# ylsung/vl-merging

Measured on AMD Instinct MI355X. Metric: VL samples/sec (fwd+bwd) base_vl 384^2 at 1/2/4/8 GPUs; merge GB/s vs HBM peak, higher is better.
Workload: dtype bf16

## Files before the change

include/vlm_hip.h:

```cpp
#ifndef VLM_HIP_H
#define VLM_HIP_H
#include <stddef.h>
#include <stdint.h>

#ifdef __cplusplus
extern "C" {
#endif

#define VLM_OK 0
#define VLM_ERR_ARG (-1)
#define VLM_ERR_LAUNCH (-2)
#define VLM_ERR_WORKSPACE (-3)
#define VLM_ERR_UNSUPPORTED (-4)

#define VLM_ABI_VERSION 10
int vlm_abi_version(void);
int vlm_device_cus(void);
int vlm_set_cu_budget(int cus);
int vlm_debug_occupy(int workgroups, int threads, int lds_bytes, int microseconds, void* stream);

#define VLM_MERGE_LERP 0
#define VLM_MERGE_TASKVEC 1
#define VLM_MERGE_MEAN 2
#define VLM_MERGE_MAX_SRC 4

typedef struct {
  void* dst;
  const void* base;
  const void* src[VLM_MERGE_MAX_SRC];
  float ratio[VLM_MERGE_MAX_SRC];
  int32_t n_src;
  int32_t mode;
  uint64_t n_elem;
} vlm_merge_job_t;

size_t vlm_merge_plan_bytes(int n_jobs, uint64_t total_elems);
int vlm_merge_plan_upload(const vlm_merge_job_t* jobs_host, int n_jobs, void* workspace, size_t workspace_bytes,
                          void* stream);
int vlm_merge_run(const void* workspace, void* stream);

typedef struct {
  void* dst;
  const void* base;
  const void* src[VLM_MERGE_MAX_SRC];
  uint64_t k[VLM_MERGE_MAX_SRC];
  uint64_t n_elem;
  int32_t n_src;
  float lam;
} vlm_ties_job_t;

typedef struct {
  uint64_t n_jobs, n_units, n_chunks;
  uint64_t jobs_off;
  uint64_t chunks_off;
  uint64_t unit0_off;
  uint64_t units_off;
  uint64_t state_off;
  uint64_t counters_off;
  uint64_t hist_off;
} vlm_ties_header_t;
typedef struct {
  uint32_t key;
  uint32_t reserved;
  uint64_t rank;
} vlm_ties_state_t;
#define VLM_TIES_COUNTERS (VLM_MERGE_MAX_SRC + 2)

size_t vlm_ties_plan_bytes(int n_jobs, uint64_t total_elems);
int vlm_ties_plan_upload(const vlm_ties_job_t* jobs_host, int n_jobs, void* workspace, size_t workspace_bytes, void* stream);
int vlm_ties_run(void* workspace, void* stream);

#define VLM_ACT_NONE 0
#define VLM_ACT_GELU 1
#define VLM_ACT_GELU_BWD 2
#define VLM_ACT_GELU_DERIV 3
#define VLM_ACT_MUL_AUX 4

typedef struct {
  const float* bias;
  const float* col_scale;
  const float* row_scale;
  const float* residual;
  int64_t ld_res;
  void* aux;
  int64_t ld_aux;
  int32_t act;
  float alpha;
  int32_t accumulate;
  int32_t reserved;
  float* col_sum;
  float* col_sum_ws;
  float* splitk_ws;
  uint64_t splitk_ws_bytes;
} vlm_epilogue_t;

int vlm_gemm_bf16(int ta, int tb, int M, int N, int K, const void* A, int lda, const void* B, int ldb, void* C,
                  int ldc, int c_is_f32, const vlm_epilogue_t* epi, void* stream);
#define VLM_GEMM_MAX_GROUPS 4
typedef struct {
  int32_t row0, rows;
  const void* B;
  int32_t ldb;
  int32_t reserved;
  const float* bias;
  float* col_sum;
  float* col_sum_ws;
} vlm_gemm_group_t;
int vlm_gemm_bf16_grouped(int n_groups, const vlm_gemm_group_t* groups, int N, int K, const void* A, int lda, void* C,
                          int ldc, int c_is_f32, const vlm_epilogue_t* epi, void* stream);
typedef struct {
  int32_t row0, rows;
  float* C;
  int32_t accumulate;
  int32_t reserved;
} vlm_wgrad_group_t;
int vlm_gemm_wgrad_grouped(int n_groups, const vlm_wgrad_group_t* groups, int M, int N, const void* A, int lda,
                           const void* B, int ldb, int ldc, float* splitk_ws, uint64_t splitk_ws_bytes, void* stream);
int vlm_gemm_set_big_tile_mode(int mode);

int vlm_layernorm_fwd(const float* x, int ldx, int M, int D, const float* gamma, const float* beta, float eps,
                      void* y, int ldy, int y_is_f32, float* stats, void* stream);
#define VLM_ROW_WS_BYTES(D) ((size_t)1536 * 2 * (size_t)(D) * sizeof(float))
int vlm_layernorm_bwd(const void* dy, int lddy, int dy_is_f32, const float* x, int ldx, const float* stats,
                      const float* gamma, int M, int D, const float* dres, int lddres, float* dx, int lddx,
                      float* dgamma, float* dbeta, float* workspace, size_t workspace_bytes, int* deferred_blocks,
                      void* stream);
typedef struct {
  const void* y;
  int32_t ldy;
  const float* gamma;
  const float* row_scale;
  void* dy;
  int32_t lddy;
  float* dgamma;
  float* dbias;
  float* workspace;
  size_t workspace_bytes;
} vlm_layerscale_t;
int vlm_layernorm_bwd_scale(const void* dy, int lddy, int dy_is_f32, const float* x, int ldx, const float* stats,
                            const float* gamma, int M, int D, const float* dres, int lddres, float* dx, int lddx,
                            float* dgamma, float* dbeta, float* workspace, size_t workspace_bytes,
                            const vlm_layerscale_t* scale, int* deferred_blocks, void* stream);
#define VLM_MAX_FOLD_JOBS 16
typedef struct {
  const float* partials;
  int32_t nblocks;
  int32_t D;
  float* out0;
  float* out1;
} vlm_fold_job_t;
int vlm_colreduce_batch(const vlm_fold_job_t* jobs_host, int n_jobs, void* stream);
int vlm_layerscale_bwd(const float* dx, int lddx, const void* y_bf16, int ldy, const float* gamma,
                       const float* row_scale, int M, int D, void* dy_bf16, int lddy, float* dgamma, float* dbias,
                       float* workspace, size_t workspace_bytes, int* deferred_blocks, void* stream);
#define VLM_MAX_LAYERSCALE_JOBS 32
typedef struct {
  const float* weight;
  const float* gamma;
  const float* bias;
  void* shadow;
  float* bias_out;
  float* raw_w;
  float* raw_b;
  float* dweight;
  float* dbias;
  float* dgamma;
  int32_t N, K;
} vlm_layerscale_job_t;
int vlm_layerscale_fold(const vlm_layerscale_job_t* jobs_host, int n_jobs, void* stream);
int vlm_layerscale_finish(const vlm_layerscale_job_t* jobs_host, int n_jobs, void* stream);
int vlm_colsum_bf16(const void* a, int lda, int M, int N, float* out, void* stream);

int vlm_cross_entropy_fwd(const void* logits_bf16, int ld, int rows, int V, const int64_t* labels, int64_t ignore_index,
                          float* loss_rows, float* lse, void* stream);
int vlm_cross_entropy_bwd(const void* logits_bf16, int ld, int rows, int V, const int64_t* labels, int64_t ignore_index,
                          const float* lse, const float* scale_dev, void* dlogits_bf16, int ld_d, void* stream);

int vlm_l2norm_fwd(const void* x, int x_is_bf16, int ld, int rows, int D, float* y, float* inv_norm, void* stream);
int vlm_l2norm_bwd(const float* g, const float* y, const float* inv_norm, int rows, int D, void* dx, int dx_is_bf16, int ld, void* stream);
size_t vlm_contrastive_ws_floats(int n);
int vlm_contrastive(const float* all_img, const float* all_txt, int n, int B, int D, const float* log_scale, float* logits, float* out3,
                    float* d_img, float* d_txt, float* ws, void* stream);
int vlm_small_cross_entropy(const void* logits, int is_bf16, int ld, int rows, int V, const int64_t* labels, float* loss, float* dlogits,
                            void* stream);
int vlm_cross_entropy_reduce(const float* loss_rows, const int64_t* labels, int rows, int V, int64_t ignore_index, float* out2, void* stream);
int vlm_scale_by_scalar(const float* const* in, float* const* out, const int* n, int count, const float* scalar_dev, void* stream);

int vlm_text_rows_fwd(const int64_t* ids, int n, const float* word, int ld_word, const float* add0, const float* gamma, const float* beta,
                      float eps, const float* u, float p, float scale, const float* add1, float* out, int ld_out, float* stats, int D,
                      void* stream);
size_t vlm_text_rows_bwd_ws_floats(int D);
int vlm_text_rows_bwd(const float* g, int ld_g, const int64_t* ids, int n, const float* word, int ld_word, const float* add0,
                      const float* gamma, const float* stats, const float* u, float p, float scale, int D, float* d_word,
                      int64_t padding_idx, float* d_add1, float* d_beta, float* d_gamma, float* d_add0, float* ws, void* stream);
int vlm_image_rows_prep(const float* conv_bias, const float* type_row, const float* cls, int D, float* out2, void* stream);
int vlm_image_lead_rows(float* x, int ld_x, int B, int rows, int D, const float* lead, void* stream);
size_t vlm_image_rows_bwd_ws_floats(int D);
int vlm_image_rows_bwd(const float* g, int ld_g, int B, int rows, int D, void* g16, float* d_bias, float* d_type_row, float* d_cls, float* ws,
                       void* stream);
int vlm_tanh_fwd(const void* x_bf16, int ld_x, int M, int N, float* y, void* stream);
int vlm_act_bwd(const void* g, int g_is_f32, int ld_g, const void* saved, int ld_saved, int mode, int M, int N, int Np, void* dy_bf16,
                void* stream);
int vlm_colsum_small(const void* a_bf16, int lda, int M, int N, float* out, void* stream);
int vlm_sample_negatives(const float* sim_a, int a_row_stride, int a_col_stride, const float* sim_b, int b_row_stride, int b_col_stride, int B,
                         int n, const float* u, int64_t* idx, void* stream);
int vlm_weighted_sum(const float* const* terms, const float* weights, int count, float* out, void* stream);

typedef struct {
  const void* g;
  int g_is_f32;
  int ld;
  int first_row, row_step, count;
} vlm_scatter_src_t;
int vlm_scatter_rows(void* dx, int dx_is_f32, int ld_dx, int R, int D, const vlm_scatter_src_t* src, int n_src, void* stream);

int vlm_adamw_step(float* p, float* g, float* m, float* v, void* p_bf16, uint64_t n, float lr, float beta1,
                   float beta2, float eps, float weight_decay, float step_size, float grad_scale, int zero_grad,
                   void* stream);
int vlm_cast_f32_bf16(const float* src, void* dst_bf16, uint64_t n, void* stream);
int vlm_embedding_bwd(const float* gy, int ld, const int64_t* ids, int64_t n, int D, int64_t padding_idx, float* dW, int ld_w,
                      int64_t vocab, void* stream);
typedef struct {
  uint64_t src;
  uint64_t dst;
  int32_t rows, cols;
  int32_t tile_row, tile_col;
} vlm_transpose_tile_t;
int vlm_transpose_bf16_tiles(const vlm_transpose_tile_t* tiles_dev, int n_tiles, void* stream);

int vlm_droppath_rows(const float* u, float keep, int B, int n0, int n1, int base0, int base1, float* out, void* stream);
int vlm_droppath_sites(const float* u0, const float* u1, const float* keep, int n_sites, int B, int n0, int n1, int base0,
                       int base1, int rows, float* out, void* stream);
int vlm_patch_im2col(const float* image, void* patches_bf16, int B, int H, int W, int P, int lead_rows, void* stream);
int vlm_accumulate_f32_f64(const float* src, double* dst_f64, uint64_t n, void* stream);
int vlm_gram_f64(const void* x, int ldx, int M, int D, int x_is_f32, double* gram, void* stream);
int vlm_gemm_f64(int ta, int tb, int M, int N, int K, double alpha, const void* A, int lda, int a_is_f32, const double* B,
                 int ldb, double beta, double* C, int ldc, void* stream);
int vlm_scale_gram_f64(const double* src, double* dst, int n, double alpha, int accumulate, void* stream);
int vlm_potrf_block_f64(double* A, int lda, int j0, int nb, int* status, void* stream);
int vlm_trsm_block_f64(const double* L, int ldl, int l0, int nb, int trans, double* B, int ldb, int rows, int c0, void* stream);
int vlm_cholesky_f64(double* A, int n, int* status, void* stream);
int vlm_solve_spd_right_f64(const double* chol, int n, double* rhs, int ld, int rows, void* stream);
int vlm_gemm_f64_batched(int ta, int tb, int M, int N, int K, double alpha, const void* const* A_list, int lda, int a_is_f32,
                         const double* const* B_list, int ldb, double beta, double* const* C_list, int ldc, int count, void* stream);
int vlm_cholesky_f64_batched(double* const* A_list, int count, int n, int* status, void* stream);
int vlm_solve_spd_right_f64_batched(double* const* chol_list, int n, double* const* rhs_list, int ld, int rows, int count, void* stream);

#define VLM_ATTN_JOINT 0
#define VLM_ATTN_SEPARATE 1

typedef struct {
  const void* qkv;
  int32_t ld_qkv;
  int32_t H;
  int32_t total_rows;
  int32_t R;
  const float* bias_t;
  const int16_t* rel_index;
  const int16_t* rel_index_t;
  int32_t ld_index;
  int32_t index_rows;
  int32_t ld_index_t;
  int32_t index_t_rows;
  int32_t head_row0;
  int32_t mode;
  const uint8_t* keep0;
  const uint8_t* keep1;
  int32_t B, n0, n1, base0, base1, pos1;
  float scale;
  int32_t reserved;
  const void* bias_dense;
  const void* bias_dense_t;
  int32_t dense_tiles;
  int32_t reserved2;
} vlm_attn_desc_t;

size_t vlm_bias_dense_bytes(int n0, int n1, int pos1, int mode);
int vlm_bias_dense(const float* bias_t, int n_cols, int R, const int16_t* index, int ld_index, int n0, int n1, int pos1,
                   int mode, int k_major, void* out_f16, void* stream);

int vlm_attention_fwd(const vlm_attn_desc_t* d, void* out_bf16, int ld_out, float* lse, void* stream);
typedef struct {
  float* dq[2];
  float* dv[2];
} vlm_attn_colsum_t;

size_t vlm_attention_bwd_ws_floats(const vlm_attn_desc_t* d, int with_dbias);
int vlm_attention_bwd(const vlm_attn_desc_t* d, const void* out_bf16, int ld_out, const void* dout_bf16, int ld_dout,
                      const float* lse, float* delta_ws, size_t ws_floats, void* dqkv_bf16, int ld_dqkv, float* dbias_t,
                      const vlm_attn_colsum_t* colsum, void* stream);

#ifdef __cplusplus
}
#endif
#endif
```

vl-merging_amd/_lib.py:

```python
import ctypes
import os

_HERE = os.path.dirname(os.path.abspath(__file__))
LIB_PATH = os.environ.get("VLM_LIB_PATH") or os.path.join(_HERE, "lib", "libvlm_hip.so")
_lib = None

c_void_p = ctypes.c_void_p
c_int = ctypes.c_int
c_float = ctypes.c_float
c_size_t = ctypes.c_size_t
c_u64 = ctypes.c_uint64

MERGE_LERP, MERGE_TASKVEC, MERGE_MEAN = 0, 1, 2
MERGE_MAX_SRC = 4


class MergeJob(ctypes.Structure):
    _fields_ = [
        ("dst", c_void_p),
        ("base", c_void_p),
        ("src", c_void_p * MERGE_MAX_SRC),
        ("ratio", c_float * MERGE_MAX_SRC),
        ("n_src", ctypes.c_int32),
        ("mode", ctypes.c_int32),
        ("n_elem", c_u64),
    ]


TIES_COUNTERS = MERGE_MAX_SRC + 2


class TiesJob(ctypes.Structure):
    _fields_ = [
        ("dst", c_void_p),
        ("base", c_void_p),
        ("src", c_void_p * MERGE_MAX_SRC),
        ("k", c_u64 * MERGE_MAX_SRC),
        ("n_elem", c_u64),
        ("n_src", ctypes.c_int32),
        ("lam", c_float),
    ]


class TiesHeader(ctypes.Structure):
    _fields_ = [(n, c_u64) for n in ("n_jobs", "n_units", "n_chunks", "jobs_off", "chunks_off", "unit0_off", "units_off",
                                     "state_off", "counters_off", "hist_off")]


class TiesState(ctypes.Structure):
    _fields_ = [("key", ctypes.c_uint32), ("reserved", ctypes.c_uint32), ("rank", c_u64)]


class ScatterSrc(ctypes.Structure):
    _fields_ = [("g", c_void_p), ("g_is_f32", ctypes.c_int32), ("ld", ctypes.c_int32), ("first_row", ctypes.c_int32),
                ("row_step", ctypes.c_int32), ("count", ctypes.c_int32)]


class Epilogue(ctypes.Structure):
    _fields_ = [
        ("bias", c_void_p), ("col_scale", c_void_p), ("row_scale", c_void_p), ("residual", c_void_p),
        ("ld_res", ctypes.c_int64), ("aux", c_void_p), ("ld_aux", ctypes.c_int64), ("act", ctypes.c_int32),
        ("alpha", c_float), ("accumulate", ctypes.c_int32), ("reserved", ctypes.c_int32), ("col_sum", c_void_p),
        ("col_sum_ws", c_void_p), ("splitk_ws", c_void_p), ("splitk_ws_bytes", ctypes.c_uint64),
    ]


GEMM_MAX_GROUPS = 4


class GemmGroup(ctypes.Structure):
    _fields_ = [("row0", ctypes.c_int32), ("rows", ctypes.c_int32), ("B", c_void_p), ("ldb", ctypes.c_int32),
                ("reserved", ctypes.c_int32), ("bias", c_void_p), ("col_sum", c_void_p), ("col_sum_ws", c_void_p)]


class WgradGroup(ctypes.Structure):
    _fields_ = [("row0", ctypes.c_int32), ("rows", ctypes.c_int32), ("C", c_void_p), ("accumulate", ctypes.c_int32),
                ("reserved", ctypes.c_int32)]


class FoldJob(ctypes.Structure):
    _fields_ = [("partials", c_void_p), ("nblocks", ctypes.c_int32), ("D", ctypes.c_int32), ("out0", c_void_p),
                ("out1", c_void_p)]


class LayerScale(ctypes.Structure):
    _fields_ = [("y", c_void_p), ("ldy", ctypes.c_int32), ("gamma", c_void_p), ("row_scale", c_void_p), ("dy", c_void_p),
                ("lddy", ctypes.c_int32), ("dgamma", c_void_p), ("dbias", c_void_p), ("workspace", c_void_p),
                ("workspace_bytes", c_size_t)]


class AttnColsum(ctypes.Structure):
    _fields_ = [("dq", c_void_p * 2), ("dv", c_void_p * 2)]


ACT_NONE, ACT_GELU, ACT_GELU_BWD, ACT_GELU_DERIV, ACT_MUL_AUX = 0, 1, 2, 3, 4
ATTN_JOINT, ATTN_SEPARATE = 0, 1


class AttnDesc(ctypes.Structure):
    _fields_ = [
        ("qkv", c_void_p), ("ld_qkv", ctypes.c_int32), ("H", ctypes.c_int32), ("total_rows", ctypes.c_int32),
        ("R", ctypes.c_int32), ("bias_t", c_void_p), ("rel_index", c_void_p), ("rel_index_t", c_void_p),
        ("ld_index", ctypes.c_int32), ("index_rows", ctypes.c_int32), ("ld_index_t", ctypes.c_int32),
        ("index_t_rows", ctypes.c_int32), ("head_row0", ctypes.c_int32), ("mode", ctypes.c_int32),
        ("keep0", c_void_p), ("keep1", c_void_p),
        ("B", ctypes.c_int32), ("n0", ctypes.c_int32), ("n1", ctypes.c_int32), ("base0", ctypes.c_int32),
        ("base1", ctypes.c_int32), ("pos1", ctypes.c_int32), ("scale", c_float), ("reserved", ctypes.c_int32),
        ("bias_dense", c_void_p), ("bias_dense_t", c_void_p), ("dense_tiles", ctypes.c_int32), ("reserved2", ctypes.c_int32),
    ]


class LayerScaleJob(ctypes.Structure):
    _fields_ = [("weight", c_void_p), ("gamma", c_void_p), ("bias", c_void_p), ("shadow", c_void_p), ("bias_out", c_void_p),
                ("raw_w", c_void_p), ("raw_b", c_void_p), ("dweight", c_void_p), ("dbias", c_void_p), ("dgamma", c_void_p),
                ("N", ctypes.c_int32), ("K", ctypes.c_int32)]


MAX_LAYERSCALE_JOBS = 32


class VlmError(RuntimeError):
    pass


_ERR = {-1: "VLM_ERR_ARG", -2: "VLM_ERR_LAUNCH", -3: "VLM_ERR_WORKSPACE", -4: "VLM_ERR_UNSUPPORTED"}

SIGNATURES = {
    "vlm_abi_version": (c_int, []),
    "vlm_device_cus": (c_int, []),
    "vlm_set_cu_budget": (c_int, [c_int]),
    "vlm_debug_occupy": (c_int, [c_int, c_int, c_int, c_int, c_void_p]),
    "vlm_layerscale_fold": (c_int, [ctypes.POINTER(LayerScaleJob), c_int, c_void_p]),
    "vlm_layerscale_finish": (c_int, [ctypes.POINTER(LayerScaleJob), c_int, c_void_p]),
    "vlm_merge_plan_bytes": (c_size_t, [c_int, c_u64]),
    "vlm_merge_plan_upload": (c_int, [ctypes.POINTER(MergeJob), c_int, c_void_p, c_size_t, c_void_p]),
    "vlm_merge_run": (c_int, [c_void_p, c_void_p]),
    "vlm_ties_plan_bytes": (c_size_t, [c_int, c_u64]),
    "vlm_ties_plan_upload": (c_int, [ctypes.POINTER(TiesJob), c_int, c_void_p, c_size_t, c_void_p]),
    "vlm_ties_run": (c_int, [c_void_p, c_void_p]),
    "vlm_gemm_bf16": (c_int, [c_int, c_int, c_int, c_int, c_int, c_void_p, c_int, c_void_p, c_int, c_void_p, c_int,
                              c_int, ctypes.POINTER(Epilogue), c_void_p]),
    "vlm_gemm_bf16_grouped": (c_int, [c_int, ctypes.POINTER(GemmGroup), c_int, c_int, c_void_p, c_int, c_void_p, c_int, c_int,
                                      ctypes.POINTER(Epilogue), c_void_p]),
    "vlm_gemm_wgrad_grouped": (c_int, [c_int, ctypes.POINTER(WgradGroup), c_int, c_int, c_void_p, c_int, c_void_p, c_int, c_int,
                                       c_void_p, c_u64, c_void_p]),
    "vlm_attention_fwd": (c_int, [ctypes.POINTER(AttnDesc), c_void_p, c_int, c_void_p, c_void_p]),
    "vlm_attention_bwd_ws_floats": (c_size_t, [ctypes.POINTER(AttnDesc), c_int]),
    "vlm_attention_bwd": (c_int, [ctypes.POINTER(AttnDesc), c_void_p, c_int, c_void_p, c_int, c_void_p, c_void_p, c_size_t,
                                  c_void_p, c_int, c_void_p, c_void_p, c_void_p]),
    "vlm_layernorm_fwd": (c_int, [c_void_p, c_int, c_int, c_int, c_void_p, c_void_p, c_float, c_void_p, c_int, c_int,
                                  c_void_p, c_void_p]),
    "vlm_layernorm_bwd": (c_int, [c_void_p, c_int, c_int, c_void_p, c_int, c_void_p, c_void_p, c_int, c_int, c_void_p,
                                  c_int, c_void_p, c_int, c_void_p, c_void_p, c_void_p, c_size_t,
                                  ctypes.POINTER(c_int), c_void_p]),
    "vlm_layernorm_bwd_scale": (c_int, [c_void_p, c_int, c_int, c_void_p, c_int, c_void_p, c_void_p, c_int, c_int, c_void_p,
                                        c_int, c_void_p, c_int, c_void_p, c_void_p, c_void_p, c_size_t,
                                        ctypes.POINTER(LayerScale), ctypes.POINTER(c_int), c_void_p]),
    "vlm_layerscale_bwd": (c_int, [c_void_p, c_int, c_void_p, c_int, c_void_p, c_void_p, c_int, c_int, c_void_p, c_int,
                                   c_void_p, c_void_p, c_void_p, c_size_t, ctypes.POINTER(c_int), c_void_p]),
    "vlm_colreduce_batch": (c_int, [ctypes.POINTER(FoldJob), c_int, c_void_p]),
    "vlm_gemm_set_big_tile_mode": (c_int, [c_int]),
    "vlm_colsum_bf16": (c_int, [c_void_p, c_int, c_int, c_int, c_void_p, c_void_p]),
    "vlm_adamw_step": (c_int, [c_void_p, c_void_p, c_void_p, c_void_p, c_void_p, c_u64, c_float, c_float, c_float,
                               c_float, c_float, c_float, c_float, c_int, c_void_p]),
    "vlm_accumulate_f32_f64": (c_int, [c_void_p, c_void_p, c_u64, c_void_p]),
    "vlm_gram_f64": (c_int, [c_void_p, c_int, c_int, c_int, c_int, c_void_p, c_void_p]),
    "vlm_gemm_f64": (c_int, [c_int, c_int, c_int, c_int, c_int, ctypes.c_double, c_void_p, c_int, c_int, c_void_p, c_int,
                             ctypes.c_double, c_void_p, c_int, c_void_p]),
    "vlm_scale_gram_f64": (c_int, [c_void_p, c_void_p, c_int, ctypes.c_double, c_int, c_void_p]),
    "vlm_potrf_block_f64": (c_int, [c_void_p, c_int, c_int, c_int, c_void_p, c_void_p]),
    "vlm_trsm_block_f64": (c_int, [c_void_p, c_int, c_int, c_int, c_int, c_void_p, c_int, c_int, c_int, c_void_p]),
    "vlm_cholesky_f64": (c_int, [c_void_p, c_int, c_void_p, c_void_p]),
    "vlm_solve_spd_right_f64": (c_int, [c_void_p, c_int, c_void_p, c_int, c_int, c_void_p]),
    "vlm_gemm_f64_batched": (c_int, [c_int, c_int, c_int, c_int, c_int, ctypes.c_double, ctypes.POINTER(c_void_p), c_int, c_int,
                                     ctypes.POINTER(c_void_p), c_int, ctypes.c_double, ctypes.POINTER(c_void_p), c_int, c_int, c_void_p]),
    "vlm_cholesky_f64_batched": (c_int, [ctypes.POINTER(c_void_p), c_int, c_int, c_void_p, c_void_p]),
    "vlm_solve_spd_right_f64_batched": (c_int, [ctypes.POINTER(c_void_p), c_int, ctypes.POINTER(c_void_p), c_int, c_int, c_int, c_void_p]),
    "vlm_cross_entropy_fwd": (c_int, [c_void_p, c_int, c_int, c_int, c_void_p, ctypes.c_int64, c_void_p, c_void_p, c_void_p]),
    "vlm_cross_entropy_bwd": (c_int, [c_void_p, c_int, c_int, c_int, c_void_p, ctypes.c_int64, c_void_p, c_void_p, c_void_p, c_int,
                                      c_void_p]),
    "vlm_l2norm_fwd": (c_int, [c_void_p, c_int, c_int, c_int, c_int, c_void_p, c_void_p, c_void_p]),
    "vlm_l2norm_bwd": (c_int, [c_void_p, c_void_p, c_void_p, c_int, c_int, c_void_p, c_int, c_int, c_void_p]),
    "vlm_contrastive_ws_floats": (c_size_t, [c_int]),
    "vlm_contrastive": (c_int, [c_void_p, c_void_p, c_int, c_int, c_int, c_void_p, c_void_p, c_void_p, c_void_p, c_void_p, c_void_p,
                                c_void_p]),
    "vlm_small_cross_entropy": (c_int, [c_void_p, c_int, c_int, c_int, c_int, c_void_p, c_void_p, c_void_p, c_void_p]),
    "vlm_cross_entropy_reduce": (c_int, [c_void_p, c_void_p, c_int, c_int, ctypes.c_int64, c_void_p, c_void_p]),
    "vlm_scale_by_scalar": (c_int, [ctypes.POINTER(c_void_p), ctypes.POINTER(c_void_p), ctypes.POINTER(c_int), c_int, c_void_p, c_void_p]),
    "vlm_text_rows_fwd": (c_int, [c_void_p, c_int, c_void_p, c_int, c_void_p, c_void_p, c_void_p, c_float, c_void_p, c_float, c_float,
                                  c_void_p, c_void_p, c_int, c_void_p, c_int, c_void_p]),
    "vlm_text_rows_bwd_ws_floats": (c_size_t, [c_int]),
    "vlm_text_rows_bwd": (c_int, [c_void_p, c_int, c_void_p, c_int, c_void_p, c_int, c_void_p, c_void_p, c_void_p, c_void_p, c_float, c_float,
                                  c_int, c_void_p, ctypes.c_int64, c_void_p, c_void_p, c_void_p, c_void_p, c_void_p, c_void_p]),
    "vlm_image_rows_prep": (c_int, [c_void_p, c_void_p, c_void_p, c_int, c_void_p, c_void_p]),
    "vlm_image_lead_rows": (c_int, [c_void_p, c_int, c_int, c_int, c_int, c_void_p, c_void_p]),
    "vlm_image_rows_bwd_ws_floats": (c_size_t, [c_int]),
    "vlm_image_rows_bwd": (c_int, [c_void_p, c_int, c_int, c_int, c_int, c_void_p, c_void_p, c_void_p, c_void_p, c_void_p, c_void_p]),
    "vlm_tanh_fwd": (c_int, [c_void_p, c_int, c_int, c_int, c_void_p, c_void_p]),
    "vlm_act_bwd": (c_int, [c_void_p, c_int, c_int, c_void_p, c_int, c_int, c_int, c_int, c_int, c_void_p, c_void_p]),
    "vlm_colsum_small": (c_int, [c_void_p, c_int, c_int, c_int, c_void_p, c_void_p]),
    "vlm_sample_negatives": (c_int, [c_void_p, c_int, c_int, c_void_p, c_int, c_int, c_int, c_int, c_void_p, c_void_p, c_void_p]),
    "vlm_weighted_sum": (c_int, [ctypes.POINTER(c_void_p), ctypes.POINTER(c_float), c_int, c_void_p, c_void_p]),
    "vlm_scatter_rows": (c_int, [c_void_p, c_int, c_int, c_int, c_int, c_void_p, c_int, c_void_p]),
    "vlm_cast_f32_bf16": (c_int, [c_void_p, c_void_p, c_u64, c_void_p]),
    "vlm_embedding_bwd": (c_int, [c_void_p, c_int, c_void_p, ctypes.c_int64, c_int, ctypes.c_int64, c_void_p, c_int,
                                  ctypes.c_int64, c_void_p]),
    "vlm_bias_dense_bytes": (c_size_t, [c_int, c_int, c_int, c_int]),
    "vlm_bias_dense": (c_int, [c_void_p, c_int, c_int, c_void_p, c_int, c_int, c_int, c_int, c_int, c_int, c_void_p,
                               c_void_p]),
    "vlm_transpose_bf16_tiles": (c_int, [c_void_p, c_int, c_void_p]),
    "vlm_droppath_sites": (c_int, [c_void_p, c_void_p, c_void_p, c_int, c_int, c_int, c_int, c_int, c_int, c_int, c_void_p,
                                   c_void_p]),
    "vlm_droppath_rows": (c_int, [c_void_p, c_float, c_int, c_int, c_int, c_int, c_int, c_void_p, c_void_p]),
    "vlm_patch_im2col": (c_int, [c_void_p, c_void_p, c_int, c_int, c_int, c_int, c_int, c_void_p]),
}


def get_lib():
    global _lib
    if _lib is None:
        if not os.path.exists(LIB_PATH):
            raise VlmError(
                f"{LIB_PATH} is missing: build it with `python -c 'import __graft_entry__ as g; g.build()'` "
                "(hipcc --offload-arch=gfx950).  There is no CPU fallback for the hot path.")
        import torch
        lib = ctypes.CDLL(LIB_PATH)
        for name, (res, args) in SIGNATURES.items():
            fn = getattr(lib, name)
            fn.restype = res
            fn.argtypes = args
        _lib = lib
    return _lib


def check(rc, what):
    if rc != 0:
        raise VlmError(f"{what} failed: {_ERR.get(rc, rc)}")


def stream_ptr():
    import torch
    return c_void_p(torch.cuda.current_stream().cuda_stream)


def ptr(t):
    return c_void_p(t.data_ptr()) if t is not None else c_void_p(0)


def require_cuda(*tensors):
    for t in tensors:
        if t is not None and not t.is_cuda:
            raise VlmError("vl_merging_amd ops run on the GPU only (tensor on %s); there is no CPU path" % t.device)
```

vl-merging_amd/csrc/gemm.hip:

```cpp
#include "vlm_common.h"
#include "vlm_diag.h"
#include <atomic>

#define GEMM_BM 128
#define GEMM_BN 128
#define GEMM_BK 64
#define GEMM_THREADS 256
#define GEMM_TILE_BYTES (GEMM_BM * GEMM_BK * 2)

typedef __attribute__((address_space(3))) s16x4 lds_s16x4;

__device__ __forceinline__ float gelu_cdf(float x, float& ez2) {
  const float t = __builtin_amdgcn_rcpf(fmaf(0.3275911f * 0.70710678118654752440f, fabsf(x), 1.0f));
  ez2 = __builtin_amdgcn_exp2f((x * x) * (-0.5f * 1.4426950408889634f));
  float poly = fmaf(t, 0.5f * 1.061405429f, 0.5f * -1.453152027f);
  poly = fmaf(t, poly, 0.5f * 1.421413741f);
  poly = fmaf(t, poly, 0.5f * -0.284496736f);
  poly = fmaf(t, poly, 0.5f * 0.254829592f);
  const float e = fmaf(-(poly * t), ez2, 0.5f);
  return 0.5f + copysignf(e, x);
}
__device__ __forceinline__ float gelu_erf(float x) {
  float ez2;
  return x * gelu_cdf(x, ez2);
}
__device__ __forceinline__ float gelu_erf_grad(float x) {
  float ez2;
  const float cdf = gelu_cdf(x, ez2);
  return fmaf(x * 0.39894228040143267794f, ez2, cdf);
}
__device__ __forceinline__ float gelu_erf_both(float x, float& deriv) {
  float ez2;
  const float cdf = gelu_cdf(x, ez2);
  deriv = fmaf(x * 0.39894228040143267794f, ez2, cdf);
  return x * cdf;
}
__device__ __forceinline__ float act_bwd_factor(int act, float saved) {
  return act == VLM_ACT_MUL_AUX ? saved : gelu_erf_grad(saved);
}

template <bool KSTRIDED>
__device__ __forceinline__ void stage_load(u32x4 (&r)[4], __amdgpu_buffer_rsrc_t rsrc, uint32_t row0, uint32_t k0,
                                           uint32_t ld, int tid) {
#pragma unroll
  for (int u = 0; u < 4; ++u) {
    const uint32_t p = tid + 256 * u;
    uint32_t off;
    if (!KSTRIDED) {
      const uint32_t row = p >> 3, chunk = p & 7;
      off = ((row0 + row) * ld + k0 + chunk * 8) * 2;
    } else {
      const uint32_t krow = p >> 4, c16 = p & 15;
      off = ((k0 + krow) * ld + row0 + c16 * 8) * 2;
    }
    r[u] = __builtin_amdgcn_raw_buffer_load_b128(rsrc, off, 0, 0);
  }
}

template <bool KSTRIDED>
__device__ __forceinline__ void stage_store(const u32x4 (&r)[4], unsigned char* lds, int tid) {
#pragma unroll
  for (int u = 0; u < 4; ++u) {
    const uint32_t p = tid + 256 * u;
    uint32_t byte;
    if (!KSTRIDED) {
      const uint32_t row = p >> 3, chunk = p & 7;
      byte = row * 128 + ((chunk ^ (row & 7)) << 4);
    } else {
      const uint32_t krow = p >> 4, c16 = p & 15;
      const uint32_t c32 = (c16 >> 1) ^ (krow & 3) ^ (((krow >> 3) & 1) << 2);
      byte = krow * 256 + c32 * 32 + (c16 & 1) * 16;
    }
    *reinterpret_cast<u32x4*>(lds + byte) = r[u];
  }
}

typedef __attribute__((address_space(3))) void lds_void;
__device__ __forceinline__ void stage_dma(__amdgpu_buffer_rsrc_t rsrc, unsigned char* tile, uint32_t row0, uint32_t k0,
                                          uint32_t ld, int wave, int lane) {
#pragma unroll
  for (int u = 0; u < 4; ++u) {
    const int j = wave + 4 * u;
    const uint32_t row = j * 8 + (lane >> 3), chunk = (lane & 7) ^ (row & 7);
    const uint32_t off = ((row0 + row) * ld + k0 + chunk * 8) * 2;
    __builtin_amdgcn_raw_ptr_buffer_load_lds(rsrc, (lds_void*)(tile + j * 1024), 16, off, 0, 0, 0);
  }
}

template <bool KSTRIDED>
__device__ __forceinline__ bf16x8 frag_load(const unsigned char* lds, int xblk , int ksub,
                                            int lane) {
  if (!KSTRIDED) {
    const uint32_t row = xblk * 16 + (lane & 15);
    const uint32_t chunk = ksub * 4 + (lane >> 4);
    const uint32_t byte = row * 128 + ((chunk ^ (row & 7)) << 4);
    return *reinterpret_cast<const bf16x8*>(lds + byte);
  } else {
    const uint32_t g = lane >> 4, q = (lane & 15) >> 2, p = lane & 3;
    const uint32_t row = ksub * 32 + 8 * g + q;
    const uint32_t c32 = ((uint32_t)xblk ^ q ^ ((g & 1) << 2));
    const uint32_t byte = row * 256 + c32 * 32 + 8 * p;
    s16x4 lo = __builtin_amdgcn_ds_read_tr16_b64_v4i16((lds_s16x4*)(lds + byte));
    s16x4 hi = __builtin_amdgcn_ds_read_tr16_b64_v4i16((lds_s16x4*)(lds + byte + 4 * 256));
    s16x8 v = {lo[0], lo[1], lo[2], lo[3], hi[0], hi[1], hi[2], hi[3]};
    return __builtin_bit_cast(bf16x8, v);
  }
}

struct gemm_group_t {
  const void* B;
  const float* bias;
  float* col_sum;
  float* col_sum_ws;
  int ldb, row0, row_end, tile0;
};

struct gemmT_group_t {
  int row0, row_end, item0, kps, slice0;
};

struct gemm_params_t {
  const void* A;
  const void* B;
  void* C;
  int M, N, K;
  int lda, ldb, ldc;
  vlm_epilogue_t epi;
  int tiles_m, tiles_n;
  int group_m;
  int splits, ksteps_per_split;
  int n_groups;
  gemm_group_t grp[VLM_GEMM_MAX_GROUPS];
  gemmT_group_t grpT[VLM_GEMM_MAX_GROUPS];
  VLM_DIAG_GEMM_FIELD
};

__device__ __forceinline__ void lane16_swap(float& x, float& y) {
  asm volatile("s_nop 1\n\tv_permlane16_swap_b32 %0, %1" : "+v"(x), "+v"(y));
}

template <bool OUT_F32, bool LEAN = false>
__device__ __forceinline__ int gemm_epilogue(const gemm_params_t& p, const f32x4 (&acc)[4][4], int mw0, int nw0, int lane,
                                             float* red = nullptr, int red_off = 0) {
  const vlm_epilogue_t& e = p.epi;
  const bool vec_ok = ((p.ldc & 3) == 0) && (!e.aux || (e.ld_aux & 3) == 0) && (!e.residual || (e.ld_res & 3) == 0);
  const bool vec8_ok = vec_ok && (OUT_F32 || (p.ldc & 7) == 0) && (!e.aux || ((e.ld_aux & 7) == 0 && ((uintptr_t)e.aux & 15) == 0)) &&
                       (!e.residual || ((uintptr_t)e.residual & 15) == 0) && (!e.bias || ((uintptr_t)e.bias & 15) == 0) &&
                       (!e.col_scale || ((uintptr_t)e.col_scale & 15) == 0);
  if (vec8_ok && mw0 + 64 <= p.M && nw0 + 64 <= p.N) {
    const bool has_res = e.residual != nullptr, bwd = e.act == VLM_ACT_GELU_BWD || e.act == VLM_ACT_MUL_AUX, accum = OUT_F32 && e.accumulate;
    const int g = lane >> 4;
    const int nl = nw0 + (g & 1) * 16 + (g >> 1) * 8;
    float bia[2][8], gam[2][8], csum[2][8];
#pragma unroll
    for (int jp = 0; jp < 2; ++jp)
#pragma unroll
      for (int r = 0; r < 8; ++r) csum[jp][r] = 0.f;
#define EPI_LOAD_COL_VECTORS()                                                                                          \
  _Pragma("unroll") for (int jp = 0; jp < 2; ++jp) _Pragma("unroll") for (int q = 0; q < 2; ++q) {                    \
    const f32x4 b4 = e.bias ? *reinterpret_cast<const f32x4*>(e.bias + nl + jp * 32 + q * 4) : (f32x4){0.f, 0.f, 0.f, 0.f}; \
    const f32x4 g4 =                                                                                                    \
        e.col_scale ? *reinterpret_cast<const f32x4*>(e.col_scale + nl + jp * 32 + q * 4) : (f32x4){1.f, 1.f, 1.f, 1.f}; \
    _Pragma("unroll") for (int r = 0; r < 4; ++r) {                                                                     \
      bia[jp][q * 4 + r] = b4[r];                                                                                       \
      gam[jp][q * 4 + r] = g4[r];                                                                                       \
    }                                                                                                                   \
  }
    if (!LEAN) { EPI_LOAD_COL_VECTORS() }
#pragma unroll
    for (int hf = 0; hf < 4; ++hf) {
      f32x4 rsd[1][2][2], old[1][2][2];
      bf16x8 hx[1][2];
      float rs[1];
      if (LEAN) { EPI_LOAD_COL_VECTORS() }
#pragma unroll
      for (int ii = 0; ii < 1; ++ii) {
        const size_t m = mw0 + (hf + ii) * 16 + (lane & 15);
        rs[ii] = e.row_scale ? e.row_scale[m] : 1.0f;
#pragma unroll
        for (int jp = 0; jp < 2; ++jp) {
          const int n = nl + jp * 32;
          if (has_res) {
            rsd[ii][jp][0] = *reinterpret_cast<const f32x4*>(e.residual + m * e.ld_res + n);
            rsd[ii][jp][1] = *reinterpret_cast<const f32x4*>(e.residual + m * e.ld_res + n + 4);
          }
          if (bwd) hx[ii][jp] = *reinterpret_cast<const bf16x8*>(reinterpret_cast<const bf16_t*>(e.aux) + m * e.ld_aux + n);
          if (accum) {
            old[ii][jp][0] = *reinterpret_cast<const f32x4*>(reinterpret_cast<const float*>(p.C) + m * p.ldc + n);
            old[ii][jp][1] = *reinterpret_cast<const f32x4*>(reinterpret_cast<const float*>(p.C) + m * p.ldc + n + 4);
          }
        }
      }
#pragma unroll
      for (int ii = 0; ii < 1; ++ii) {
        const size_t m = mw0 + (hf + ii) * 16 + (lane & 15);
#pragma unroll
        for (int jp = 0; jp < 2; ++jp) {
          const int n = nl + jp * 32;
          float v[8];
#pragma unroll
          for (int r = 0; r < 4; ++r) {
            float x = acc[hf + ii][2 * jp][r] * e.alpha, y = acc[hf + ii][2 * jp + 1][r] * e.alpha;
            lane16_swap(x, y);
            v[r] = x;
            v[4 + r] = y;
          }
#pragma unroll
          for (int r = 0; r < 8; ++r) v[r] += bia[jp][r];
          if (bwd) {
#pragma unroll
            for (int r = 0; r < 8; ++r) v[r] *= act_bwd_factor(e.act, (float)hx[ii][jp][r]);
          } else if (e.act == VLM_ACT_GELU_DERIV) {
            bf16x8 h;
#pragma unroll
            for (int r = 0; r < 8; ++r) {
              float dg;
              v[r] = gelu_erf_both(v[r], dg);
              h[r] = (bf16_t)dg;
            }
            *reinterpret_cast<bf16x8*>(reinterpret_cast<bf16_t*>(e.aux) + m * e.ld_aux + n) = h;
          } else {
            if (e.aux) {
              bf16x8 h;
#pragma unroll
              for (int r = 0; r < 8; ++r) h[r] = (bf16_t)v[r];
              *reinterpret_cast<bf16x8*>(reinterpret_cast<bf16_t*>(e.aux) + m * e.ld_aux + n) = h;
            }
            if (e.act == VLM_ACT_GELU) {
#pragma unroll
              for (int r = 0; r < 8; ++r) v[r] = gelu_erf(v[r]);
            }
          }
          if (e.col_scale) {
#pragma unroll
            for (int r = 0; r < 8; ++r) v[r] *= gam[jp][r];
          }
          if (e.row_scale) {
#pragma unroll
            for (int r = 0; r < 8; ++r) v[r] *= rs[ii];
          }
          if (has_res) {
#pragma unroll
            for (int r = 0; r < 8; ++r) v[r] += rsd[ii][jp][r >> 2][r & 3];
          }
          if (OUT_F32 && accum) {
#pragma unroll
            for (int r = 0; r < 8; ++r) v[r] += old[ii][jp][r >> 2][r & 3];
          }
          if (!LEAN && e.col_sum) {
#pragma unroll
            for (int r = 0; r < 8; ++r) csum[jp][r] += v[r];
          }
          if (OUT_F32) {
            float* c = reinterpret_cast<float*>(p.C) + m * p.ldc + n;
            *reinterpret_cast<f32x4*>(c) = (f32x4){v[0], v[1], v[2], v[3]};
            *reinterpret_cast<f32x4*>(c + 4) = (f32x4){v[4], v[5], v[6], v[7]};
          } else {
            bf16x8 o;
#pragma unroll
            for (int r = 0; r < 8; ++r) o[r] = (bf16_t)v[r];
            *reinterpret_cast<bf16x8*>(reinterpret_cast<bf16_t*>(p.C) + m * p.ldc + n) = o;
          }
        }
      }
    }
    if (!LEAN && e.col_sum) {
#pragma unroll
      for (int jp = 0; jp < 2; ++jp)
#pragma unroll
        for (int r = 0; r < 8; ++r) {
          float t = csum[jp][r];
          t += dpp_f32<0x128>(t);
          t += dpp_f32<0x124>(t);
          t += dpp_f32<0x122>(t);
          t += dpp_f32<0x121>(t);
          if ((lane & 15) == 0) {
            if (red) red[red_off + (g & 1) * 16 + (g >> 1) * 8 + jp * 32 + r] = t;
            else atomicAdd(e.col_sum + nl + jp * 32 + r, t);
          }
        }
      return -1;
    }
    return 8 * (OUT_F32 ? 2 : 1) + ((e.aux && !bwd) ? 8 : 0);
  }
#pragma unroll
  for (int i = 0; i < 4; ++i) {
    const int m = mw0 + i * 16 + (lane & 15);
    if (m >= p.M) continue;
    const float rs = e.row_scale ? e.row_scale[m] : 1.0f;
#pragma unroll
    for (int j = 0; j < 4; ++j) {
      const int n = nw0 + j * 16 + (lane >> 4) * 4;
      if (n >= p.N) continue;
      const bool full = vec_ok && (n + 3 < p.N);
      float v[4];
#pragma unroll
      for (int r = 0; r < 4; ++r) v[r] = acc[i][j][r] * e.alpha;
      if (full) {
        if (e.bias) {
          const f32x4 b = *reinterpret_cast<const f32x4*>(e.bias + n);
#pragma unroll
          for (int r = 0; r < 4; ++r) v[r] += b[r];
        }
        if (e.act == VLM_ACT_GELU_BWD || e.act == VLM_ACT_MUL_AUX) {
          const bf16x4 h = *reinterpret_cast<const bf16x4*>(reinterpret_cast<const bf16_t*>(e.aux) + (size_t)m * e.ld_aux + n);
#pragma unroll
          for (int r = 0; r < 4; ++r) v[r] *= act_bwd_factor(e.act, (float)h[r]);
        } else if (e.act == VLM_ACT_GELU_DERIV) {
          bf16x4 h;
#pragma unroll
          for (int r = 0; r < 4; ++r) {
            float dg;
            v[r] = gelu_erf_both(v[r], dg);
            h[r] = (bf16_t)dg;
          }
          *reinterpret_cast<bf16x4*>(reinterpret_cast<bf16_t*>(e.aux) + (size_t)m * e.ld_aux + n) = h;
        } else {
          if (e.aux) {
            bf16x4 h;
#pragma unroll
            for (int r = 0; r < 4; ++r) h[r] = (bf16_t)v[r];
            *reinterpret_cast<bf16x4*>(reinterpret_cast<bf16_t*>(e.aux) + (size_t)m * e.ld_aux + n) = h;
          }
          if (e.act == VLM_ACT_GELU) {
#pragma unroll
            for (int r = 0; r < 4; ++r) v[r] = gelu_erf(v[r]);
          }
        }
        if (e.col_scale) {
          const f32x4 g = *reinterpret_cast<const f32x4*>(e.col_scale + n);
#pragma unroll
          for (int r = 0; r < 4; ++r) v[r] *= g[r];
        }
        if (e.row_scale) {
#pragma unroll
          for (int r = 0; r < 4; ++r) v[r] *= rs;
        }
        if (e.residual) {
          const f32x4 x = *reinterpret_cast<const f32x4*>(e.residual + (size_t)m * e.ld_res + n);
#pragma unroll
          for (int r = 0; r < 4; ++r) v[r] += x[r];
        }
        if (OUT_F32) {
          float* c = reinterpret_cast<float*>(p.C) + (size_t)m * p.ldc + n;
          f32x4 o = {v[0], v[1], v[2], v[3]};
          if (e.accumulate) {
            const f32x4 old = *reinterpret_cast<const f32x4*>(c);
            o += old;
          }
          if (e.col_sum) {
#pragma unroll
            for (int r = 0; r < 4; ++r) atomicAdd(e.col_sum + n + r, o[r]);
          }
          *reinterpret_cast<f32x4*>(c) = o;
        } else {
          if (e.col_sum) {
#pragma unroll
            for (int r = 0; r < 4; ++r) atomicAdd(e.col_sum + n + r, v[r]);
          }
          bf16x4 o;
#pragma unroll
          for (int r = 0; r < 4; ++r) o[r] = (bf16_t)v[r];
          *reinterpret_cast<bf16x4*>(reinterpret_cast<bf16_t*>(p.C) + (size_t)m * p.ldc + n) = o;
        }
      } else {
        for (int r = 0; r < 4 && n + r < p.N; ++r) {
          float x = v[r];
          if (e.bias) x += e.bias[n + r];
          if (e.act == VLM_ACT_GELU_BWD || e.act == VLM_ACT_MUL_AUX) {
            x *= act_bwd_factor(e.act, (float)reinterpret_cast<const bf16_t*>(e.aux)[(size_t)m * e.ld_aux + n + r]);
          } else if (e.act == VLM_ACT_GELU_DERIV) {
            float dg;
            x = gelu_erf_both(x, dg);
            reinterpret_cast<bf16_t*>(e.aux)[(size_t)m * e.ld_aux + n + r] = (bf16_t)dg;
          } else {
            if (e.aux) reinterpret_cast<bf16_t*>(e.aux)[(size_t)m * e.ld_aux + n + r] = (bf16_t)x;
            if (e.act == VLM_ACT_GELU) x = gelu_erf(x);
          }
          if (e.col_scale) x *= e.col_scale[n + r];
          if (e.row_scale) x *= rs;
          if (e.residual) x += e.residual[(size_t)m * e.ld_res + n + r];
          if (OUT_F32 && e.accumulate) x += reinterpret_cast<const float*>(p.C)[(size_t)m * p.ldc + n + r];
          if (e.col_sum) atomicAdd(e.col_sum + n + r, x);
          if (OUT_F32) {
            reinterpret_cast<float*>(p.C)[(size_t)m * p.ldc + n + r] = x;
          } else {
            reinterpret_cast<bf16_t*>(p.C)[(size_t)m * p.ldc + n + r] = (bf16_t)x;
          }
        }
      }
    }
  }
  return -1;
}

template <bool TA, bool TB, bool OUT_F32, bool SPLITK>
__global__ __launch_bounds__(GEMM_THREADS, 2) void vlm_gemm_kernel(const gemm_params_t p) {
  constexpr bool DMA_A = !TA && !SPLITK, DMA_B = !TB && !SPLITK;
  extern __shared__ __attribute__((aligned(16))) unsigned char smem[];
  const int tid = threadIdx.x;
  const int lane = tid & 63;
  const int wave = tid >> 6;
  const int wm = wave >> 1, wn = wave & 1;
  GEMM_STAMP(0)

  const uint32_t ntile = p.tiles_m * p.tiles_n;
  uint32_t tile, split = 0;
  if (SPLITK) {
    tile = blockIdx.x % ntile;
    split = blockIdx.x / ntile;
  } else {
    const uint32_t nblk = gridDim.x;
    const uint32_t bid = blockIdx.x;
    const uint32_t q8 = nblk >> 3, r8 = nblk & 7, xcd = bid & 7;
    tile = (xcd < r8 ? xcd * (q8 + 1) : r8 * (q8 + 1) + (xcd - r8) * q8) + (bid >> 3);
  }
  uint32_t tm, tn;
  {
    const uint32_t gm = (uint32_t)p.group_m, gsz = gm * p.tiles_n, grp = tile / gsz, first = grp * gm;
    const uint32_t rows = min(gm, (uint32_t)p.tiles_m - first), in = tile - grp * gsz;
    tm = first + in % rows;
    tn = in / rows;
  }
  const uint32_t m0 = tm * GEMM_BM, n0 = tn * GEMM_BN;

  const uint64_t a_rows = TA ? (uint64_t)p.K : (uint64_t)p.M;
  const uint64_t b_rows = TB ? (uint64_t)p.K : (uint64_t)p.N;
  const __amdgpu_buffer_rsrc_t ra =
      __builtin_amdgcn_make_buffer_rsrc(const_cast<void*>(p.A), 0, (int)(a_rows * p.lda * 2), 0x00020000);
  const __amdgpu_buffer_rsrc_t rb =
      __builtin_amdgcn_make_buffer_rsrc(const_cast<void*>(p.B), 0, (int)(b_rows * p.ldb * 2), 0x00020000);

#define LDS_A(s) (smem + (s) * 2 * GEMM_TILE_BYTES)
#define LDS_B(s) (smem + (s) * 2 * GEMM_TILE_BYTES + GEMM_TILE_BYTES)

  f32x4 acc[4][4];
// ... 202 lines not shown
#pragma unroll
          for (int r = 0; r < 8; ++r) v[r] *= gelu_erf_grad((float)in.hx[t][r]);
        }
      } else if (AUX == 1 && e.act == VLM_ACT_GELU_DERIV) {
        bf16x8 h;
#pragma unroll
        for (int r = 0; r < 8; ++r) {
          float dg;
          v[r] = gelu_erf_both(v[r], dg);
          h[r] = (bf16_t)dg;
        }
        __builtin_amdgcn_raw_buffer_store_b128(__builtin_bit_cast(u32x4, h), r_aux, (m * (uint32_t)e.ld_aux + n) * 2, 0, EPIL_AUX_STORE_AUX);
      } else {
        if (AUX == 1) {
          bf16x8 h;
#pragma unroll
          for (int r = 0; r < 8; ++r) h[r] = (bf16_t)v[r];
          __builtin_amdgcn_raw_buffer_store_b128(__builtin_bit_cast(u32x4, h), r_aux, (m * (uint32_t)e.ld_aux + n) * 2, 0, EPIL_AUX_STORE_AUX);
        }
        if (e.act == VLM_ACT_GELU) {
#pragma unroll
          for (int r = 0; r < 8; ++r) v[r] = gelu_erf(v[r]);
        }
      }
      if (RES) {
#pragma unroll
        for (int r = 0; r < 8; ++r) v[r] *= gam[r];
        if (e.row_scale) {
#pragma unroll
          for (int r = 0; r < 8; ++r) v[r] *= in.rs[t];
        }
#pragma unroll
        for (int r = 0; r < 8; ++r) v[r] += in.rsd[t][r >> 2][r & 3];
      }
      if (AUX == 2) {
        if (m < (uint32_t)p.M) {
#pragma unroll
          for (int r = 0; r < 8; ++r) csum[r] += v[r];
        }
      }
      if (OUT_F32) {
        const uint32_t co = (m * (uint32_t)p.ldc + n) * 4;
        __builtin_amdgcn_raw_buffer_store_b128(__builtin_bit_cast(u32x4, (f32x4){v[0], v[1], v[2], v[3]}), r_c, co, 0, STORE_AUX);
        __builtin_amdgcn_raw_buffer_store_b128(__builtin_bit_cast(u32x4, (f32x4){v[4], v[5], v[6], v[7]}), r_c, co + 16, 0, STORE_AUX);
      } else {
        bf16x8 o;
#pragma unroll
        for (int r = 0; r < 8; ++r) o[r] = (bf16_t)v[r];
        __builtin_amdgcn_raw_buffer_store_b128(__builtin_bit_cast(u32x4, o), r_c, (m * (uint32_t)p.ldc + n) * 2, 0, STORE_AUX);
      }
    }
  }

  __device__ __forceinline__ void finish(int lane, float* ws_row) {
    const vlm_epilogue_t& e = p.epi;
    if (AUX != 2 || !e.col_sum) return;
#pragma unroll
    for (int r = 0; r < 8; ++r) {
      if (LPR == 8) csum[r] += __shfl_xor(csum[r], 8);
      csum[r] += __shfl_xor(csum[r], 16);
      csum[r] += __shfl_xor(csum[r], 32);
    }
    if (lane < LPR) {
      if (ws_row) {
        *reinterpret_cast<f32x4*>(ws_row + n) = (f32x4){csum[0], csum[1], csum[2], csum[3]};
        *reinterpret_cast<f32x4*>(ws_row + n + 4) = (f32x4){csum[4], csum[5], csum[6], csum[7]};
      } else {
#pragma unroll
        for (int r = 0; r < 8; ++r) atomicAdd(e.col_sum + n + r, csum[r]);
      }
    }
  }
};

#define EPIL_DUMP_ROW(A0, A1, II, OFF)                                                           \
  _Pragma("unroll") for (int j = 0; j < 4; ++j) {                                                \
    *reinterpret_cast<f32x4*>(wr + (OFF) + 64 * j) = A0[II][j];                                  \
    *reinterpret_cast<f32x4*>(wr + (OFF) + 64 * (4 + j)) = A1[II][j];                            \
  }
#define BIG_EPILOGUE_LOOP_DEEP(AHEAD)                                                                             \
  unsigned char* wr = wl + (lane & 15) * EPIL_PITCH + (lane >> 4) * 16;                                            \
  epil_in_t in8[8];                                                                                                \
  _Pragma("unroll") for (int b8 = 0; b8 < (AHEAD); ++b8) ep.load_inputs(in8[b8], b8);                              \
  _Pragma("unroll") for (int q = 0; q < 4; ++q) {                                                                  \
    switch (q) {                                                                                                   \
      case 0: EPIL_DUMP_ROW(acc00, acc01, 0, 0) EPIL_DUMP_ROW(acc00, acc01, 1, 16 * EPIL_PITCH) break;             \
      case 1: EPIL_DUMP_ROW(acc00, acc01, 2, 0) EPIL_DUMP_ROW(acc00, acc01, 3, 16 * EPIL_PITCH) break;             \
      case 2: EPIL_DUMP_ROW(acc10, acc11, 0, 0) EPIL_DUMP_ROW(acc10, acc11, 1, 16 * EPIL_PITCH) break;             \
      default: EPIL_DUMP_ROW(acc10, acc11, 2, 0) EPIL_DUMP_ROW(acc10, acc11, 3, 16 * EPIL_PITCH) break;            \
    }                                                                                                              \
    ep.process(in8[2 * q], 2 * q, 0);                                                                              \
    if (2 * q + (AHEAD) < 8) ep.load_inputs(in8[2 * q + (AHEAD)], 2 * q + (AHEAD));                                \
    ep.process(in8[2 * q + 1], 2 * q + 1, 16 * EPIL_PITCH);                                                        \
    if (2 * q + 1 + (AHEAD) < 8) ep.load_inputs(in8[2 * q + 1 + (AHEAD)], 2 * q + 1 + (AHEAD));                    \
  }
#define BIG_EPILOGUE_LOOP()                                                                                       \
  unsigned char* wr = wl + (lane & 15) * EPIL_PITCH + (lane >> 4) * 16;                                            \
  ep.load_inputs(inB, 1);                                                                                          \
  _Pragma("unroll 1") for (int q = 0; q < 4; ++q) {                                                                \
    switch (q) {                                                                                                   \
      case 0: EPIL_DUMP_ROW(acc00, acc01, 0, 0) EPIL_DUMP_ROW(acc00, acc01, 1, 16 * EPIL_PITCH) break;             \
      case 1: EPIL_DUMP_ROW(acc00, acc01, 2, 0) EPIL_DUMP_ROW(acc00, acc01, 3, 16 * EPIL_PITCH) break;             \
      case 2: EPIL_DUMP_ROW(acc10, acc11, 0, 0) EPIL_DUMP_ROW(acc10, acc11, 1, 16 * EPIL_PITCH) break;             \
      default: EPIL_DUMP_ROW(acc10, acc11, 2, 0) EPIL_DUMP_ROW(acc10, acc11, 3, 16 * EPIL_PITCH) break;            \
    }                                                                                                              \
    ep.process(inA, 2 * q, 0);                                                                                     \
    ep.load_inputs(inA, q < 3 ? 2 * q + 2 : 7);                                                                    \
    ep.process(inB, 2 * q + 1, 16 * EPIL_PITCH);                                                                   \
    ep.load_inputs(inB, q < 3 ? 2 * q + 3 : 7);                                                                    \
  }

template <bool OUT_F32, bool RES, int AUX, bool GROUPED = false>
__global__ __launch_bounds__(GEMM_THREADS, 1) void vlm_gemm_big_kernel(const gemm_params_t p_in) {
  __shared__ __attribute__((aligned(1024))) unsigned char sA0[BIG_OP_BYTES], sA1[BIG_OP_BYTES], sB0[BIG_OP_BYTES], sB1[BIG_OP_BYTES];
  __shared__ __attribute__((aligned(16))) unsigned char epl[4 * EPIL_WAVE_BYTES];
  const int tid = threadIdx.x;
  const int lane = tid & 63;
  const int wave = __builtin_amdgcn_readfirstlane(tid >> 6);
  const int wm = wave >> 1, wn = wave & 1;

  const uint32_t nblk = gridDim.x, bid = blockIdx.x;
  const uint32_t q8 = nblk >> 3, r8 = nblk & 7, xcd = bid & 7;
  const uint32_t tile = (xcd < r8 ? xcd * (q8 + 1) : r8 * (q8 + 1) + (xcd - r8) * q8) + (bid >> 3);
  uint32_t tm, tn;
  {
    const uint32_t gm = (uint32_t)p_in.group_m, gsz = gm * p_in.tiles_n, grp = tile / gsz, first = grp * gm;
    const uint32_t rows = min(gm, (uint32_t)p_in.tiles_m - first), in = tile - grp * gsz;
    tm = first + in % rows;
    tn = in / rows;
  }
  gemm_params_t p_grp;
  uint32_t m0 = tm * BIG_BM, tm_ws = tm;
  if constexpr (GROUPED) {
    p_grp = p_in;
    int g = 0;
#pragma unroll
    for (int i = 1; i < VLM_GEMM_MAX_GROUPS; ++i)
      if (i < p_in.n_groups && tm >= (uint32_t)p_in.grp[i].tile0) g = i;
    const gemm_group_t G = p_in.grp[g];
    tm_ws = tm - (uint32_t)G.tile0;
    m0 = (uint32_t)G.row0 + tm_ws * BIG_BM;
    p_grp.M = G.row_end;
    p_grp.B = G.B;
    p_grp.ldb = G.ldb;
    p_grp.epi.bias = G.bias;
    p_grp.epi.col_sum = G.col_sum;
    p_grp.epi.col_sum_ws = G.col_sum_ws;
  }
  const gemm_params_t& p = GROUPED ? p_grp : p_in;
  GEMM_STAMP(0)
  const uint32_t n0 = tn * BIG_BN;
  const __amdgpu_buffer_rsrc_t ra =
      __builtin_amdgcn_make_buffer_rsrc(const_cast<void*>(p.A), 0, (int)((uint64_t)p.M * p.lda * 2), 0x00020000);
  const __amdgpu_buffer_rsrc_t rb =
      __builtin_amdgcn_make_buffer_rsrc(const_cast<void*>(p.B), 0, (int)((uint64_t)p.N * p.ldb * 2), 0x00020000);

  uint32_t offa[4], offb[4];
  {
    const uint32_t chunk = (lane & 3) ^ big_swz(lane >> 4);
#pragma unroll
    for (int u = 0; u < 4; ++u) {
      const uint32_t row = (wave + 4 * u) * 16 + (lane >> 2);
      offa[u] = ((m0 + row) * (uint32_t)p.lda + chunk * 8) * 2;
      offb[u] = ((n0 + row) * (uint32_t)p.ldb + chunk * 8) * 2;
    }
  }
  const uint32_t rd_slot = ((uint32_t)(lane >> 4) ^ big_swz((lane & 15) >> 2)) * 16 + (lane & 15) * 64;
  const uint32_t rda = wm * 128 * 64 + rd_slot, rdb = wn * 128 * 64 + rd_slot;

  f32x4 acc00[4][4], acc01[4][4], acc10[4][4], acc11[4][4];
#pragma unroll
  for (int i = 0; i < 4; ++i)
#pragma unroll
    for (int j = 0; j < 4; ++j) {
      acc00[i][j] = (f32x4){0.f, 0.f, 0.f, 0.f};
      acc01[i][j] = (f32x4){0.f, 0.f, 0.f, 0.f};
      acc10[i][j] = (f32x4){0.f, 0.f, 0.f, 0.f};
      acc11[i][j] = (f32x4){0.f, 0.f, 0.f, 0.f};
    }

#define BIG_PIN_ACC()                                                                                   \
  _Pragma("unroll") for (int i = 0; i < 4; ++i) _Pragma("unroll") for (int j = 0; j < 4; ++j) {         \
    asm volatile("" : "+a"(acc00[i][j]), "+a"(acc01[i][j]), "+a"(acc10[i][j]), "+a"(acc11[i][j]));      \
  }
  constexpr bool DEEP = AUX == 2 && !RES;
  constexpr int AHEAD = 6;
  if constexpr (DEEP) { BIG_PIN_ACC() }

  const int nk = p.K / BIG_BK;
  const uint32_t mw0 = m0 + wm * 128, nw0 = n0 + wn * 128;
  unsigned char* const wl = epl + wave * EPIL_WAVE_BYTES;
#define EPIL_SETUP()                                       \
  big_epilogue_t<OUT_F32, RES, AUX> ep(p, wl, mw0, nw0, lane); \
  epil_in_t inA, inB;                                      \
  ep.load_inputs(inA, 0);
  bf16x8 fa0[8], fb0[8], fa1[8], fb1[8];

#define BIG_READ(FA, FB, SA, SB)                                                         \
  _Pragma("unroll") for (int i = 0; i < 8; ++i) {                                        \
    FA[i] = *reinterpret_cast<const bf16x8*>((SA) + rda + i * 1024);                     \
    FB[i] = *reinterpret_cast<const bf16x8*>((SB) + rdb + i * 1024);                     \
  }
#define BIG_MFMA_Q(ACC, FA, FB, I0, J0)                                                                                \
  _Pragma("unroll") for (int i = 0; i < 4; ++i) _Pragma("unroll") for (int j = 0; j < 4; ++j)                         \
      ACC[i][j] = __builtin_amdgcn_mfma_f32_16x16x32_bf16(FB[(J0) + j], FA[(I0) + i], ACC[i][j], 0, 0, 0);
#define BIG_MFMA(FA, FB)        \
  BIG_MFMA_Q(acc00, FA, FB, 0, 0) \
  BIG_MFMA_Q(acc01, FA, FB, 0, 4) \
  BIG_MFMA_Q(acc11, FA, FB, 4, 4) \
  BIG_MFMA_Q(acc10, FA, FB, 4, 0)
  uint32_t wr_off[4];
  {
    const uint32_t slot = (lane & 3) ^ big_swz(lane >> 4);
#pragma unroll
    for (int u = 0; u < 4; ++u) wr_off[u] = ((wave + 4 * u) * 16 + (lane >> 2)) * 64 + slot * 16;
  }
  {
    const uint32_t unswz = (((lane & 3) ^ big_swz(lane >> 4)) - (lane & 3)) * 16;
#pragma unroll
    for (int u = 0; u < 4; ++u) { offa[u] -= unswz; offb[u] -= unswz; }
  }
  u32x4 ra0[4], rb0[4], ra1[4], rb1[4];
#define BIG_GLOAD(RA_, RB_, S)                                                                        \
  _Pragma("unroll") for (int u = 0; u < 4; ++u) {                                                     \
    RA_[u] = __builtin_amdgcn_raw_buffer_load_b128(ra, offa[u], (S) * (BIG_BK * 2), 0);               \
    RB_[u] = __builtin_amdgcn_raw_buffer_load_b128(rb, offb[u], (S) * (BIG_BK * 2), 0);               \
  }
#define BIG_LWRITE(RA_, RB_, SA, SB)                                                                  \
  _Pragma("unroll") for (int u = 0; u < 4; ++u) {                                                     \
    *reinterpret_cast<u32x4*>((SA) + wr_off[u]) = RA_[u];                                             \
    *reinterpret_cast<u32x4*>((SB) + wr_off[u]) = RB_[u];                                             \
  }
#define BIG_STEP(K, GL, WR, RD, FCA, FCB, FNA, FNB, RSA, RSB, BUFA_W, BUFB_W, BUFA_R, BUFB_R)   \
  {                                                                                      \
    if (RD) {                                                                            \
      asm volatile("s_waitcnt lgkmcnt(0)" ::: "memory");                                 \
      __builtin_amdgcn_s_barrier();                                                      \
    }                                                                                    \
    __builtin_amdgcn_sched_barrier(0);                                                   \
    if (WR) { BIG_LWRITE(RSA, RSB, BUFA_W, BUFB_W) }                                     \
    if (GL) { BIG_GLOAD(RSA, RSB, (K) + 4) }                                             \
    if (RD) { BIG_READ(FNA, FNB, BUFA_R, BUFB_R) }                                       \
    BIG_MFMA(FCA, FCB)                                                                   \
    _Pragma("unroll") for (int g = 0; g < 16; ++g) {                                     \
      __builtin_amdgcn_sched_group_barrier(0x008, 2, 0);                                 \
      __builtin_amdgcn_sched_group_barrier(0x100, 1, 0);                                 \
    }                                                                                    \
    _Pragma("unroll") for (int g = 0; g < 8; ++g) {                                      \
      __builtin_amdgcn_sched_group_barrier(0x008, 2, 0);                                 \
      __builtin_amdgcn_sched_group_barrier(0x200, 1, 0);                                 \
      __builtin_amdgcn_sched_group_barrier(0x008, 2, 0);                                 \
      __builtin_amdgcn_sched_group_barrier(0x020, 1, 0);                                 \
    }                                                                                    \
    __builtin_amdgcn_sched_barrier(0);                                                   \
  }

  BIG_GLOAD(ra0, rb0, 0)
  BIG_GLOAD(ra1, rb1, 1)
  BIG_LWRITE(ra0, rb0, sA0, sB0)
  BIG_GLOAD(ra0, rb0, 2)
  BIG_LWRITE(ra1, rb1, sA1, sB1)
  BIG_GLOAD(ra1, rb1, 3)
  asm volatile("s_waitcnt lgkmcnt(0)" ::: "memory");
  __builtin_amdgcn_s_barrier();
  BIG_READ(fa0, fb0, sA0, sB0)
  GEMM_STAMP(1)

  int kt = 0;
  for (; kt < nk - 4; kt += 2) {
    BIG_STEP(kt + 0, 1, 1, 1, fa0, fb0, fa1, fb1, ra0, rb0, sA0, sB0, sA1, sB1)
    BIG_STEP(kt + 1, 1, 1, 1, fa1, fb1, fa0, fb0, ra1, rb1, sA1, sB1, sA0, sB0)
  }
#define BIG_TAIL_STEPS()                                                               \
  BIG_STEP(kt + 0, 0, 1, 1, fa0, fb0, fa1, fb1, ra0, rb0, sA0, sB0, sA1, sB1)          \
  BIG_STEP(kt + 1, 0, 1, 1, fa1, fb1, fa0, fb0, ra1, rb1, sA1, sB1, sA0, sB0)          \
  BIG_STEP(kt + 2, 0, 0, 1, fa0, fb0, fa1, fb1, ra0, rb0, sA0, sB0, sA1, sB1)          \
  BIG_STEP(kt + 3, 0, 0, 0, fa1, fb1, fa0, fb0, ra1, rb1, sA1, sB1, sA0, sB0)
  if constexpr (DEEP) {
    BIG_TAIL_STEPS()
    GEMM_STAMP(2)
    big_epilogue_t<OUT_F32, RES, AUX> ep(p, wl, mw0, nw0, lane);
    float* ws_row = (p.epi.col_sum_ws && mw0 + 128 <= (uint32_t)p.M) ? p.epi.col_sum_ws + ((size_t)(tm_ws * 2 + wm) * 2) * p.N : nullptr;
    BIG_EPILOGUE_LOOP_DEEP(AHEAD)
    ep.finish(lane, ws_row);
  } else {
    EPIL_SETUP()
    BIG_TAIL_STEPS()
    GEMM_STAMP(2)
    float* ws_row = (p.epi.col_sum_ws && mw0 + 128 <= (uint32_t)p.M) ? p.epi.col_sum_ws + ((size_t)(tm_ws * 2 + wm) * 2) * p.N : nullptr;
    BIG_EPILOGUE_LOOP()
    ep.finish(lane, ws_row);
  }
  GEMM_STAMP_END()
}

template <bool GROUPED = false>
__global__ __launch_bounds__(GEMM_THREADS, 1) void vlm_gemm_bigT_kernel(const gemm_params_t p) {
  __shared__ __attribute__((aligned(1024))) unsigned char sA0[BIG_OP_BYTES], sA1[BIG_OP_BYTES], sB0[BIG_OP_BYTES], sB1[BIG_OP_BYTES];
  __shared__ __attribute__((aligned(16))) unsigned char epl[4 * EPIL_WAVE_BYTES];
  const int tid = threadIdx.x;
  const int lane = tid & 63;
  const int wave = __builtin_amdgcn_readfirstlane(tid >> 6);
  const int wm = wave >> 1, wn = wave & 1;
  const uint32_t ntile = p.tiles_m * p.tiles_n;
  const uint32_t q8 = gridDim.x >> 3, r8 = gridDim.x & 7, xcd = blockIdx.x & 7;
  uint32_t item = (xcd < r8 ? xcd * (q8 + 1) : r8 * (q8 + 1) + (xcd - r8) * q8) + (blockIdx.x >> 3);
  uint32_t k_base = 0, k_end = (uint32_t)p.K, slice0 = 0;
  int nk = p.ksteps_per_split;
  if constexpr (GROUPED) {
    int g = 0;
#pragma unroll
    for (int i = 1; i < VLM_GEMM_MAX_GROUPS; ++i)
      if (i < p.n_groups && item >= (uint32_t)p.grpT[i].item0) g = i;
    const gemmT_group_t G = p.grpT[g];
    item -= (uint32_t)G.item0;
    k_base = (uint32_t)G.row0;
    k_end = (uint32_t)G.row_end;
    nk = G.kps;
    slice0 = (uint32_t)G.slice0;
  }
  const uint32_t split = item / ntile, tile = item - split * ntile;
  const uint32_t tm = tile / p.tiles_n, tn = tile - tm * p.tiles_n;
  const uint32_t m0 = tm * BIG_BM, n0 = tn * BIG_BN;
  const uint32_t k_first = k_base + split * (uint32_t)nk * BIG_BK;
  const __amdgpu_buffer_rsrc_t ra =
      __builtin_amdgcn_make_buffer_rsrc(const_cast<void*>(p.A), 0, (int)((uint64_t)k_end * p.lda * 2), 0x00020000);
  const __amdgpu_buffer_rsrc_t rb =
      __builtin_amdgcn_make_buffer_rsrc(const_cast<void*>(p.B), 0, (int)((uint64_t)k_end * p.ldb * 2), 0x00020000);

  uint32_t offa[4], offb[4], wr_off[4];
#pragma unroll
  for (int u = 0; u < 4; ++u) {
    const uint32_t row = 2 * (wave + 4 * u) + (lane >> 5), c16 = lane & 31;
    offa[u] = ((k_first + row) * (uint32_t)p.lda + m0 + c16 * 8) * 2;
    offb[u] = ((k_first + row) * (uint32_t)p.ldb + n0 + c16 * 8) * 2;
    wr_off[u] = row * 512 + (((c16 >> 1) ^ ((row & 3) | (((row >> 3) & 1) << 2))) << 5) + (c16 & 1) * 16;
  }
  uint32_t rda[8], rdb[8];
  {
    const uint32_t g = lane >> 4, q = (lane & 15) >> 2, pp = lane & 3, sw = q | ((g & 1) << 2);
#pragma unroll
    for (int i = 0; i < 8; ++i) {
      rda[i] = (8 * g + q) * 512 + wm * 256 + ((i ^ sw) << 5) + 8 * pp;
      rdb[i] = (8 * g + q) * 512 + wn * 256 + ((i ^ sw) << 5) + 8 * pp;
    }
  }
  f32x4 acc00[4][4], acc01[4][4], acc10[4][4], acc11[4][4];
#pragma unroll
  for (int i = 0; i < 4; ++i)
#pragma unroll
    for (int j = 0; j < 4; ++j) {
      acc00[i][j] = (f32x4){0.f, 0.f, 0.f, 0.f};
      acc01[i][j] = (f32x4){0.f, 0.f, 0.f, 0.f};
      acc10[i][j] = (f32x4){0.f, 0.f, 0.f, 0.f};
      acc11[i][j] = (f32x4){0.f, 0.f, 0.f, 0.f};
    }
  const uint32_t stepa = BIG_BK * (uint32_t)p.lda * 2, stepb = BIG_BK * (uint32_t)p.ldb * 2;
  bf16x8 fa0[8], fb0[8], fa1[8], fb1[8];
  u32x4 ra0[4], rb0[4], ra1[4], rb1[4];
#define BIGT_TR(PTR) __builtin_amdgcn_ds_read_tr16_b64_v4i16((lds_s16x4*)(PTR))
#define BIGT_READ(FA, FB, SA, SB)                                                                    \
  _Pragma("unroll") for (int i = 0; i < 8; ++i) {                                                    \
    const s16x4 al = BIGT_TR((SA) + rda[i]), ah = BIGT_TR((SA) + rda[i] + 4 * 512);                  \
    const s16x4 bl = BIGT_TR((SB) + rdb[i]), bh = BIGT_TR((SB) + rdb[i] + 4 * 512);                  \
    FA[i] = __builtin_bit_cast(bf16x8, (s16x8){al[0], al[1], al[2], al[3], ah[0], ah[1], ah[2], ah[3]}); \
    FB[i] = __builtin_bit_cast(bf16x8, (s16x8){bl[0], bl[1], bl[2], bl[3], bh[0], bh[1], bh[2], bh[3]}); \
  }
#define BIGT_GLOAD(RA_, RB_, S)                                                                      \
  _Pragma("unroll") for (int u = 0; u < 4; ++u) {                                                    \
    RA_[u] = __builtin_amdgcn_raw_buffer_load_b128(ra, offa[u], (S) * stepa, 0);                     \
    RB_[u] = __builtin_amdgcn_raw_buffer_load_b128(rb, offb[u], (S) * stepb, 0);                     \
  }
#define BIGT_LWRITE(RA_, RB_, SA, SB)                                                                \
  _Pragma("unroll") for (int u = 0; u < 4; ++u) {                                                    \
    *reinterpret_cast<u32x4*>((SA) + wr_off[u]) = RA_[u];                                            \
    *reinterpret_cast<u32x4*>((SB) + wr_off[u]) = RB_[u];                                            \
  }
#define BIGT_STEP(K, GL, WR, RD, FCA, FCB, FNA, FNB, RSA, RSB, BUFA_W, BUFB_W, BUFA_R, BUFB_R)      \
  {                                                                                      \
    if (RD) {                                                                            \
      asm volatile("s_waitcnt lgkmcnt(0)" ::: "memory");                                 \
      __builtin_amdgcn_s_barrier();                                                      \
    }                                                                                    \
    __builtin_amdgcn_sched_barrier(0);                                                   \
    if (WR) { BIGT_LWRITE(RSA, RSB, BUFA_W, BUFB_W) }                                    \
    if (GL) { BIGT_GLOAD(RSA, RSB, (K) + 4) }                                            \
    if (RD) { BIGT_READ(FNA, FNB, BUFA_R, BUFB_R) }                                      \
    BIG_MFMA(FCA, FCB)                                                                   \
    _Pragma("unroll") for (int g = 0; g < 32; ++g) {                                     \
      __builtin_amdgcn_sched_group_barrier(0x008, 1, 0);                                 \
      __builtin_amdgcn_sched_group_barrier(0x100, 1, 0);                                 \
    }                                                                                    \
    _Pragma("unroll") for (int g = 0; g < 8; ++g) {                                      \
      __builtin_amdgcn_sched_group_barrier(0x008, 2, 0);                                 \
      __builtin_amdgcn_sched_group_barrier(0x200, 1, 0);                                 \
      __builtin_amdgcn_sched_group_barrier(0x008, 2, 0);                                 \
      __builtin_amdgcn_sched_group_barrier(0x020, 1, 0);                                 \
    }                                                                                    \
    __builtin_amdgcn_sched_barrier(0);                                                   \
  }
  BIGT_GLOAD(ra0, rb0, 0)
  BIGT_GLOAD(ra1, rb1, 1)
  BIGT_LWRITE(ra0, rb0, sA0, sB0)
  BIGT_GLOAD(ra0, rb0, 2)
  BIGT_LWRITE(ra1, rb1, sA1, sB1)
  BIGT_GLOAD(ra1, rb1, 3)
  asm volatile("s_waitcnt lgkmcnt(0)" ::: "memory");
  __builtin_amdgcn_s_barrier();
  BIGT_READ(fa0, fb0, sA0, sB0)
  int kt = 0;
  for (; kt < nk - 4; kt += 2) {
    BIGT_STEP(kt + 0, 1, 1, 1, fa0, fb0, fa1, fb1, ra0, rb0, sA0, sB0, sA1, sB1)
    BIGT_STEP(kt + 1, 1, 1, 1, fa1, fb1, fa0, fb0, ra1, rb1, sA1, sB1, sA0, sB0)
  }
  BIGT_STEP(kt + 0, 0, 1, 1, fa0, fb0, fa1, fb1, ra0, rb0, sA0, sB0, sA1, sB1)
  BIGT_STEP(kt + 1, 0, 1, 1, fa1, fb1, fa0, fb0, ra1, rb1, sA1, sB1, sA0, sB0)
  BIGT_STEP(kt + 2, 0, 0, 1, fa0, fb0, fa1, fb1, ra0, rb0, sA0, sB0, sA1, sB1)
  BIGT_STEP(kt + 3, 0, 0, 0, fa1, fb1, fa0, fb0, ra1, rb1, sA1, sB1, sA0, sB0)

  gemm_params_t pl = p;
  pl.C = reinterpret_cast<float*>(p.C) + (size_t)(slice0 + split) * p.M * p.N;
  pl.ldc = p.N;
  const uint32_t mw0 = m0 + wm * 128, nw0 = n0 + wn * 128;
  unsigned char* const wl = epl + wave * EPIL_WAVE_BYTES;
  big_epilogue_t<true, false, 0, 128, 0, true> ep(pl, wl, mw0, nw0, lane);
  epil_in_t inA, inB;
  ep.load_inputs(inA, 0);
  BIG_EPILOGUE_LOOP()
}

__global__ __launch_bounds__(256) void splitk_reduce_kernel(const float* __restrict__ ws, int splits, int M, int N, float* __restrict__ C,
                                                            int ldc, int accumulate) {
  const size_t i = (size_t)blockIdx.x * 256 + threadIdx.x, per = (size_t)M * N / 4;
  if (i >= per) return;
  const size_t e = i * 4, m = e / N, n = e - m * N;
  f32x4 t = accumulate ? *reinterpret_cast<const f32x4*>(C + m * ldc + n) : (f32x4){0.f, 0.f, 0.f, 0.f};
  for (int s = 0; s < splits; ++s) t += *reinterpret_cast<const f32x4*>(ws + (size_t)s * M * N + e);
  *reinterpret_cast<f32x4*>(C + m * ldc + n) = t;
}

struct splitk_groups_t {
  float* C[VLM_GEMM_MAX_GROUPS];
  int slice0[VLM_GEMM_MAX_GROUPS], splits[VLM_GEMM_MAX_GROUPS], accumulate[VLM_GEMM_MAX_GROUPS];
};
__global__ __launch_bounds__(256) void splitk_reduce_grouped_kernel(const float* __restrict__ ws, const splitk_groups_t g, int M, int N, int ldc) {
  const size_t i = (size_t)blockIdx.x * 256 + threadIdx.x, per = (size_t)M * N / 4;
  if (i >= per) return;
  const int gi = blockIdx.y;
  float* const C = g.C[gi];
  const size_t e = i * 4, m = e / N, n = e - m * N;
  f32x4 t = g.accumulate[gi] ? *reinterpret_cast<const f32x4*>(C + m * ldc + n) : (f32x4){0.f, 0.f, 0.f, 0.f};
  for (int s = 0; s < g.splits[gi]; ++s) t += *reinterpret_cast<const f32x4*>(ws + (size_t)(g.slice0[gi] + s) * M * N + e);
  *reinterpret_cast<f32x4*>(C + m * ldc + n) = t;
}

static int plan_cus() {
  const int cus = vlm_device_cus();
  return cus > 0 ? cus : 256;
}

static bool epi_vec8(const vlm_epilogue_t* e, int ldc, int c_is_f32) {
  const bool v4 = ((ldc & 3) == 0) && (!e->aux || (e->ld_aux & 3) == 0) && (!e->residual || (e->ld_res & 3) == 0);
  return v4 && (c_is_f32 || (ldc & 7) == 0) && (!e->aux || ((e->ld_aux & 7) == 0 && ((uintptr_t)e->aux & 15) == 0)) &&
         (!e->residual || ((uintptr_t)e->residual & 15) == 0) && (!e->bias || ((uintptr_t)e->bias & 15) == 0) &&
         (!e->col_scale || ((uintptr_t)e->col_scale & 15) == 0);
}

static bool epi_off32(const vlm_epilogue_t* e, int M, int lda, int ldc) {
  return (uint64_t)M * ldc * 4 < (1ull << 31) && (!e->residual || (uint64_t)M * e->ld_res * 4 < (1ull << 31)) &&
         (!e->aux || (uint64_t)M * e->ld_aux * 2 < (1ull << 31)) && (uint64_t)M * lda * 2 < (1ull << 31);
}

static int launch_gemm_bigT(gemm_params_t p, const vlm_epilogue_t* epi, hipStream_t stream) {
  if (!epi->splitk_ws || (p.N % BIG_BN) || (p.ldc % 4)) return 1;
  if ((uint64_t)p.M * p.N * 4 >= (1ull << 31)) return 1;
  p.tiles_m = (p.M + BIG_BM - 1) / BIG_BM;
  p.tiles_n = (p.N + BIG_BN - 1) / BIG_BN;
  const int ntile = p.tiles_m * p.tiles_n, nk = (p.K + BIG_BK - 1) / BIG_BK;
  int splits = plan_cus() / ntile;
  if (splits < 1) splits = 1;
  if (splits > nk / 16) splits = nk / 16;
  if (splits < 1) return 1;
  int kps = (nk + splits - 1) / splits;
  kps += kps & 1;
  if (kps < 4) kps = 4;
  splits = (nk + kps - 1) / kps;
  if ((size_t)splits * p.M * p.N * 4 > (size_t)epi->splitk_ws_bytes) return 1;
  p.ksteps_per_split = kps;
  p.splits = splits;
  float* const out = reinterpret_cast<float*>(p.C);
  const int ldc = p.ldc;
  p.C = epi->splitk_ws;
  hipLaunchKernelGGL(vlm_gemm_bigT_kernel<false>, dim3(ntile * splits), dim3(GEMM_THREADS), 0, stream, p);
  VLM_CHECK_LAUNCH();
  const size_t per = (size_t)p.M * p.N / 4;
  hipLaunchKernelGGL(splitk_reduce_kernel, dim3((unsigned)((per + 255) / 256)), dim3(256), 0, stream,
                     reinterpret_cast<const float*>(epi->splitk_ws), splits, p.M, p.N, out, ldc, epi->accumulate);
  VLM_CHECK_LAUNCH();
  return VLM_OK;
}

template <bool OUT_F32, bool RES, int AUX, bool GROUPED = false>
static int launch_gemm_big(gemm_params_t p, hipStream_t stream) {
  if (!GROUPED) p.tiles_m = (p.M + BIG_BM - 1) / BIG_BM;
  p.tiles_n = (p.N + BIG_BN - 1) / BIG_BN;
  p.group_m = p.tiles_n >= 6 ? 4 : 1;
  GEMM_STAMP_ARM(p)
  hipLaunchKernelGGL((vlm_gemm_big_kernel<OUT_F32, RES, AUX, GROUPED>), dim3(p.tiles_m * p.tiles_n), dim3(GEMM_THREADS), 0, stream, p);
  VLM_CHECK_LAUNCH();
  return VLM_OK;
}

template <bool GROUPED = false>
static int launch_gemm_big_variant(const gemm_params_t& p, bool c_is_f32, hipStream_t s) {
  const vlm_epilogue_t& e = p.epi;
  const bool res = e.residual != nullptr;
  const int aux = e.aux ? ((e.act == VLM_ACT_GELU_BWD || e.act == VLM_ACT_MUL_AUX) ? 2 : 1) : 0;
  if (e.row_scale && !res) return 1;
  {
    bool any_cs = e.col_sum != nullptr;
    if (GROUPED)
      for (int g = 0; g < p.n_groups; ++g) any_cs = any_cs || p.grp[g].col_sum != nullptr;
    if (e.alpha != 1.0f || (e.col_scale && !res) || (any_cs && aux != 2)) return 1;
  }
  if (!c_is_f32 && !res) {
    if (aux == 0) return launch_gemm_big<false, false, 0, GROUPED>(p, s);
    if (aux == 1) return launch_gemm_big<false, false, 1, GROUPED>(p, s);
    return launch_gemm_big<false, false, 2, GROUPED>(p, s);
  }
  if (c_is_f32 && aux != 2) {
    if (res && aux) return launch_gemm_big<true, true, 1, GROUPED>(p, s);
    if (res) return launch_gemm_big<true, true, 0, GROUPED>(p, s);
    if (GROUPED) return 1;
    if (aux == 0) return launch_gemm_big<true, false, 0>(p, s);
  }
  return 1;
}

static std::atomic<int> g_big_mode{1};
static int gemm_big_mode() { return g_big_mode.load(std::memory_order_relaxed); }
extern "C" int vlm_gemm_set_big_tile_mode(int mode) {
  if (mode < -1 || mode > 2) return VLM_ERR_ARG;
  g_big_mode.store(mode < 0 ? 1 : mode, std::memory_order_relaxed);
  return VLM_OK;
}


extern "C" int vlm_gemm_bf16(int ta, int tb, int M, int N, int K, const void* A, int lda, const void* B, int ldb,
                             void* C, int ldc, int c_is_f32, const vlm_epilogue_t* epi, void* stream) {
  if (M < 0 || N < 0 || K < 0 || !C) return VLM_ERR_ARG;
  if (M == 0 || N == 0) return VLM_OK;
  if (!A || !B || !epi) return VLM_ERR_ARG;
  if ((lda & 7) || (ldb & 7) || ((uintptr_t)A & 15) || ((uintptr_t)B & 15)) return VLM_ERR_ARG;
  if ((!ta || !tb) && (K % GEMM_BK)) return VLM_ERR_UNSUPPORTED;
  if (((ldc & 3) == 0) && ((uintptr_t)C & 15)) return VLM_ERR_ARG;
  if (epi->accumulate && !c_is_f32) return VLM_ERR_ARG;
  if ((epi->act == VLM_ACT_GELU_BWD || epi->act == VLM_ACT_MUL_AUX || epi->act == VLM_ACT_GELU_DERIV) && !epi->aux) return VLM_ERR_ARG;
  if (epi->act < VLM_ACT_NONE || epi->act > VLM_ACT_MUL_AUX) return VLM_ERR_ARG;
  if (epi->col_sum_ws && (!epi->col_sum || (N % GEMM_BN) != 0 || ta)) return VLM_ERR_ARG;
  const uint64_t a_bytes = (uint64_t)(ta ? K : M) * lda * 2, b_bytes = (uint64_t)(tb ? K : N) * ldb * 2;
  if (a_bytes >= (1ull << 31) || b_bytes >= (1ull << 31)) return VLM_ERR_UNSUPPORTED;
  gemm_params_t p;
  p.A = A; p.B = B; p.C = C;
  p.M = M; p.N = N; p.K = K;
  p.lda = lda; p.ldb = ldb; p.ldc = ldc;
  p.epi = *epi;
  p.epi.reserved = epi_vec8(epi, ldc, c_is_f32) ? 1 : 0;
  if (epi->col_sum_ws && !p.epi.reserved) return VLM_ERR_ARG;
  p.tiles_m = (M + GEMM_BM - 1) / GEMM_BM;
  p.tiles_n = (N + GEMM_BN - 1) / GEMM_BN;
  p.splits = 1;
  p.ksteps_per_split = 0;
  p.n_groups = 0;
  p.group_m = p.tiles_n >= 12 ? 8 : 1;
  GEMM_STAMP_ARM(p)
  hipStream_t s = (hipStream_t)stream;
  const int ntile = p.tiles_m * p.tiles_n, nk = (K + GEMM_BK - 1) / GEMM_BK;
  const bool plain_acc = epi->accumulate && c_is_f32 && !epi->bias && !epi->col_scale && !epi->row_scale &&
                         !epi->residual && !epi->aux && !epi->col_sum && epi->act == VLM_ACT_NONE;
  if (gemm_big_mode() > 0 && ta && tb && c_is_f32 && !epi->bias && !epi->col_scale && !epi->row_scale && !epi->residual &&
      !epi->aux && !epi->col_sum && epi->act == VLM_ACT_NONE && K >= 2048) {
    const int rc = launch_gemm_bigT(p, epi, s);
    if (rc <= 0) return rc;
  }
  if (tb && plain_acc && ntile < 512 && nk >= 32) {
    int splits = 2 * plan_cus() / ntile;
    if (splits < 1) splits = 1;
    if (splits > nk / 8) splits = nk / 8;
    if (splits > 1) {
      p.ksteps_per_split = (nk + splits - 1) / splits;
      p.splits = (nk + p.ksteps_per_split - 1) / p.ksteps_per_split;
      p.group_m = p.tiles_n >= 12 ? 1 : 4;
      if (ta) return launch_gemm<true, true, true, true>(p, s);
      return launch_gemm<false, true, true, true>(p, s);
    }
  }
  if (!ta && !tb && (K % (4 * BIG_BK)) == 0 && gemm_big_mode() > 0) {
    const long big_tiles = (long)((M + BIG_BM - 1) / BIG_BM) * ((N + BIG_BN - 1) / BIG_BN);
    const bool ws_ok = (N % BIG_BN) == 0 && p.epi.reserved == 1 && epi_off32(epi, M, lda, ldc) && !epi->accumulate;
    if (ws_ok && (gemm_big_mode() >= 2 || 2 * big_tiles >= plan_cus())) {
      const int rc = launch_gemm_big_variant<>(p, c_is_f32 != 0, s);
      if (rc <= 0) return rc;
    }
  }
#ifdef GEMM_ONLY_BIG
  return VLM_ERR_UNSUPPORTED;
#endif
  const int key = (ta ? 4 : 0) | (tb ? 2 : 0) | (c_is_f32 ? 1 : 0);
  switch (key) {
    case 0: return launch_gemm<false, false, false, false>(p, s);
    case 1: return launch_gemm<false, false, true, false>(p, s);
    case 2: return launch_gemm<false, true, false, false>(p, s);
    case 3: return launch_gemm<false, true, true, false>(p, s);
    case 4: return launch_gemm<true, false, false, false>(p, s);
    case 5: return launch_gemm<true, false, true, false>(p, s);
    case 6: return launch_gemm<true, true, false, false>(p, s);
    default: return launch_gemm<true, true, true, false>(p, s);
  }
}

extern "C" int vlm_gemm_bf16_grouped(int n_groups, const vlm_gemm_group_t* groups, int N, int K, const void* A, int lda, void* C,
                                     int ldc, int c_is_f32, const vlm_epilogue_t* epi, void* stream) {
  if (n_groups < 1 || n_groups > VLM_GEMM_MAX_GROUPS || !groups || N < 0 || K < 0 || !C || !epi) return VLM_ERR_ARG;
  if (epi->bias || epi->col_sum || epi->col_sum_ws || epi->splitk_ws) return VLM_ERR_ARG;
  int prev_end = 0;
  for (int g = 0; g < n_groups; ++g) {
    const vlm_gemm_group_t& G = groups[g];
    if (G.row0 < prev_end || G.rows < 0 || !G.B || (G.col_sum_ws && !G.col_sum)) return VLM_ERR_ARG;
    prev_end = G.row0 + G.rows;
  }
  const int M_total = prev_end;
  if (M_total == 0 || N == 0) return VLM_OK;
  if (!A) return VLM_ERR_ARG;
  hipStream_t s = (hipStream_t)stream;
  bool big = gemm_big_mode() > 0 && (K % (4 * BIG_BK)) == 0 && (N % BIG_BN) == 0 && !epi->accumulate && (lda & 7) == 0 &&
             ((uintptr_t)A & 15) == 0 && ((uintptr_t)C & 15) == 0 && epi_vec8(epi, ldc, c_is_f32) && epi_off32(epi, M_total, lda, ldc);
  gemm_params_t p;
  p.A = A; p.B = nullptr; p.C = C;
  p.M = M_total; p.N = N; p.K = K;
  p.lda = lda; p.ldb = 0; p.ldc = ldc;
  p.epi = *epi;
  p.epi.reserved = 1;
  p.splits = 1;
  p.ksteps_per_split = 0;
  p.n_groups = 0;
  int tiles = 0;
  for (int g = 0; g < n_groups && big; ++g) {
    const vlm_gemm_group_t& G = groups[g];
    if (G.rows == 0) continue;
    if ((G.ldb & 7) || ((uintptr_t)G.B & 15) || (uint64_t)N * G.ldb * 2 >= (1ull << 31) || (G.bias && ((uintptr_t)G.bias & 15))) big = false;
    gemm_group_t& D = p.grp[p.n_groups++];
    D.B = G.B; D.bias = G.bias; D.col_sum = G.col_sum; D.col_sum_ws = G.col_sum_ws;
    D.ldb = G.ldb; D.row0 = G.row0; D.row_end = G.row0 + G.rows; D.tile0 = tiles;
    tiles += (G.rows + BIG_BM - 1) / BIG_BM;
  }
  if (big && p.n_groups >= 1) {
    p.tiles_m = tiles;
    if (gemm_big_mode() >= 2 || 2l * tiles * (N / BIG_BN) >= plan_cus()) {
      const int rc = launch_gemm_big_variant<true>(p, c_is_f32 != 0, s);
      if (rc <= 0) return rc;
    }
  }
  for (int g = 0; g < n_groups; ++g) {
    const vlm_gemm_group_t& G = groups[g];
    if (G.rows == 0) continue;
    vlm_epilogue_t e = *epi;
    const size_t r0 = (size_t)G.row0;
    e.bias = G.bias; e.col_sum = G.col_sum; e.col_sum_ws = G.col_sum_ws;
    if (e.residual) e.residual += r0 * e.ld_res;
    if (e.aux) e.aux = reinterpret_cast<unsigned char*>(e.aux) + r0 * e.ld_aux * 2;
    if (e.row_scale) e.row_scale += r0;
    const int rc = vlm_gemm_bf16(0, 0, G.rows, N, K, reinterpret_cast<const unsigned char*>(A) + r0 * lda * 2, lda, G.B, G.ldb,
                                 reinterpret_cast<unsigned char*>(C) + r0 * ldc * (c_is_f32 ? 4 : 2), ldc, c_is_f32, &e, stream);
    if (rc) return rc;
  }
  return VLM_OK;
}

extern "C" int vlm_gemm_wgrad_grouped(int n_groups, const vlm_wgrad_group_t* groups, int M, int N, const void* A, int lda,
                                      const void* B, int ldb, int ldc, float* splitk_ws, uint64_t splitk_ws_bytes, void* stream) {
  if (n_groups < 1 || n_groups > VLM_GEMM_MAX_GROUPS || !groups || M < 0 || N < 0) return VLM_ERR_ARG;
  int prev_end = 0;
  for (int g = 0; g < n_groups; ++g) {
    if (groups[g].row0 < prev_end || groups[g].rows < 0 || !groups[g].C) return VLM_ERR_ARG;
    prev_end = groups[g].row0 + groups[g].rows;
  }
  if (M == 0 || N == 0) return VLM_OK;
  if (!A || !B || (lda & 7) || (ldb & 7) || ((uintptr_t)A & 15) || ((uintptr_t)B & 15)) return VLM_ERR_ARG;
  hipStream_t s = (hipStream_t)stream;
  for (int g = 0; g < n_groups; ++g)
    if (groups[g].rows == 0 && !groups[g].accumulate &&
        hipMemset2DAsync(groups[g].C, (size_t)ldc * 4, 0, (size_t)N * 4, M, s) != hipSuccess)
      return VLM_ERR_LAUNCH;
  const int K_total = prev_end;
  bool big = gemm_big_mode() > 0 && splitk_ws && (N % BIG_BN) == 0 && (ldc % 4) == 0 && (uint64_t)M * N * 4 < (1ull << 31) &&
             (uint64_t)K_total * lda * 2 < (1ull << 31) && (uint64_t)K_total * ldb * 2 < (1ull << 31);
  gemm_params_t p;
  p.A = A; p.B = B; p.C = splitk_ws;
  p.M = M; p.N = N; p.K = K_total;
  p.lda = lda; p.ldb = ldb; p.ldc = N;
  p.epi = vlm_epilogue_t{};
  p.epi.alpha = 1.0f;
  p.epi.reserved = 1;
  p.tiles_m = (M + BIG_BM - 1) / BIG_BM;
  p.tiles_n = (N + BIG_BN - 1) / BIG_BN;
  p.group_m = 1;
  p.splits = 1;
  p.ksteps_per_split = 0;
  p.n_groups = 0;
  splitk_groups_t rg{};
  if (big) {
    const int ntile = p.tiles_m * p.tiles_n;
    const int cus = plan_cus();
    long total_steps = 0;
    int live = 0;
    for (int g = 0; g < n_groups; ++g)
      if (groups[g].rows > 0) { total_steps += (groups[g].rows + BIG_BK - 1) / BIG_BK; ++live; }
    if (live == 0) return VLM_OK;
    if ((long)live * ntile > cus) big = false;
    long target = (total_steps * ntile + cus - 1) / cus;
    if (target < 16) target = 16;
    for (; big; target += 2) {
      long items = 0;
      for (int g = 0; g < n_groups; ++g)
        if (groups[g].rows > 0) items += (((groups[g].rows + BIG_BK - 1) / BIG_BK + target - 1) / target) * ntile;
      if (items <= cus) break;
    }
    int item0 = 0, slice0 = 0;
    for (int g = 0; g < n_groups && big; ++g) {
      const vlm_wgrad_group_t& G = groups[g];
      if (G.rows == 0) continue;
      if ((uintptr_t)G.C & 15) { big = false; break; }
      const int nk = (G.rows + BIG_BK - 1) / BIG_BK;
      int splits = (int)((nk + target - 1) / target);
      int kps = (nk + splits - 1) / splits;
      kps += kps & 1;
      if (kps < 4) kps = 4;
      splits = (nk + kps - 1) / kps;
      const int i = p.n_groups++;
      p.grpT[i] = gemmT_group_t{G.row0, G.row0 + G.rows, item0, kps, slice0};
      rg.C[i] = G.C; rg.slice0[i] = slice0; rg.splits[i] = splits; rg.accumulate[i] = G.accumulate;
      item0 += splits * ntile;
      slice0 += splits;
    }
    if (big && (size_t)slice0 * M * N * 4 > (size_t)splitk_ws_bytes) big = false;
    if (big) {
      hipLaunchKernelGGL(vlm_gemm_bigT_kernel<true>, dim3(item0), dim3(GEMM_THREADS), 0, s, p);
      VLM_CHECK_LAUNCH();
      const size_t per = (size_t)M * N / 4;
      hipLaunchKernelGGL(splitk_reduce_grouped_kernel, dim3((unsigned)((per + 255) / 256), p.n_groups), dim3(256), 0, s,
                         reinterpret_cast<const float*>(splitk_ws), rg, M, N, ldc);
      VLM_CHECK_LAUNCH();
      return VLM_OK;
    }
  }
  for (int g = 0; g < n_groups; ++g) {
    const vlm_wgrad_group_t& G = groups[g];
    if (G.rows == 0) continue;
    vlm_epilogue_t e{};
    e.alpha = 1.0f;
    e.accumulate = G.accumulate;
    e.splitk_ws = splitk_ws;
    e.splitk_ws_bytes = splitk_ws_bytes;
    const size_t r0 = (size_t)G.row0;
    const int rc = vlm_gemm_bf16(1, 1, M, N, G.rows, reinterpret_cast<const unsigned char*>(A) + r0 * lda * 2, lda,
                                 reinterpret_cast<const unsigned char*>(B) + r0 * ldb * 2, ldb, G.C, ldc, 1, &e, stream);
    if (rc) return rc;
  }
  return VLM_OK;
}
```

vl-merging_amd/engine.py:

```python
import itertools
import math
import os
import weakref
from typing import List, Optional

import torch

from . import _lib as L
from . import ops

BF16, F32 = torch.bfloat16, torch.float32
ALIGN = 64


def _touch_hook(p):
    p._vlm_flat.touched.add(p._vlm_name)


def touch(*params):
    for p in params:
        if p is not None:
            f = getattr(p, "_vlm_flat", None)
            if f is not None:
                f.touched.add(p._vlm_name)


def _touch_expert(e):
    touch(e.n1w, e.n1b, e.qkvw, e.qb, e.vb, e.projw, e.projb, e.n2w, e.n2b, e.fc1w, e.fc1b, e.fc2w, e.fc2b)


_FLAT_SERIAL = itertools.count()


class FlatParams:

    def __init__(self, module: torch.nn.Module, order_key=None):
        named = [(n, p) for n, p in module.named_parameters()]
        if order_key is not None:
            named.sort(key=lambda np_: order_key(np_[0]))
        self.names = [n for n, _ in named]
        self.params = [p for _, p in named]
        self.offsets = {}
        self.extent = {}
        off = 0
        for i, (n, p) in enumerate(named):
            self.offsets[n] = (off, p.numel())
            ext = (p.numel() + ALIGN - 1) // ALIGN * ALIGN
            nxt = named[i + 1] if i + 1 < len(named) else None
            if (n.endswith(".q_bias") and nxt is not None and nxt[0] == n[:-len("q_bias")] + "v_bias"
                    and p.numel() % ALIGN == 0 and nxt[1].numel() == p.numel()):
                ext = 2 * p.numel()
                p._vlm_qkv_bias_span = 3 * p.numel()
            self.extent[n] = ext
            off += ext
        self.numel = off
        self.touched = set()
        self.serial = next(_FLAT_SERIAL)
        self.dense_cache = {}
        dev = self.params[0].device
        pad = 64 * 4096
        self.flat_p = torch.zeros(off + pad, device=dev, dtype=F32)
        self.flat_g = torch.zeros(off + pad, device=dev, dtype=F32)
        self.flat_b = torch.zeros(off + pad, device=dev, dtype=BF16) if dev.type == "cuda" else None
        for n, p in named:
            o, k = self.offsets[n]
            self.flat_p[o:o + k].view_as(p).copy_(p.data)
            p.data = self.flat_p[o:o + k].view_as(p)
            p.grad = self.flat_g[o:o + k].view_as(p)
            p._vlm_name = n
            p._vlm_flat = self
            p.register_post_accumulate_grad_hook(_touch_hook)
            p._vlm_bf16 = self.flat_b[o:o + k].view_as(p) if self.flat_b is not None else None
            span = getattr(p, "_vlm_qkv_bias_span", 0)
            p._vlm_qkv_bias = self.flat_p[o:o + span] if span else None
        self.dirty = True
        self.version = 0

    def refresh_shadow(self):
        if self.flat_b is None:
            raise L.VlmError("the bf16 shadow lives on the GPU; move the model to cuda before flattening")
        ops.cast_bf16(self.flat_p[:self.numel], self.flat_b[:self.numel])
        self.refresh_transposed()
        self.dirty = False
        self.version += 1

    def enable_transposed(self, predicate):
        if self.flat_b is None:
            return
        self.flat_bt = torch.zeros_like(self.flat_b)
        pairs = []
        for n, p in zip(self.names, self.params):
            if p.dim() == 2 and predicate(n):
                o, k = self.offsets[n]
                p._vlm_bf16_t = self.flat_bt[o:o + k].view(p.shape[1], p.shape[0])
                pairs.append((p._vlm_bf16, p._vlm_bf16_t))
        self._tr_table, self._tr_tiles = ops.transpose_table(pairs) if pairs else (None, 0)

    def refresh_transposed(self):
        self.refresh_folded()
        if getattr(self, "_tr_tiles", 0):
            ops.transpose_tiles(self._tr_table, self._tr_tiles)

    def enable_layerscale_fold(self, entries):
        if self.flat_b is None or not entries:
            return
        seen, total = set(), 0
        uniq = []
        for layer, w, b, g in entries:
            if id(w) in seen:
                continue
            seen.add(id(w))
            uniq.append((layer, w, b, g))
            total += (w.numel() + ALIGN - 1) // ALIGN * ALIGN + 2 * ((w.shape[0] + ALIGN - 1) // ALIGN * ALIGN)
        buf = torch.zeros(total, device=self.flat_p.device, dtype=F32)
        off = 0
        self._ls_jobs = {}

        def take(n, shape):
            nonlocal off
            t = buf[off:off + n].view(shape)
            off += (n + ALIGN - 1) // ALIGN * ALIGN
            return t

        for layer, w, b, g in uniq:
            w._vlm_raw = take(w.numel(), w.shape)
            raw_b = take(w.shape[0], (w.shape[0],))
            folded_b = take(w.shape[0], (w.shape[0],))
            if b is not None:
                b._vlm_raw, b._vlm_folded = raw_b, folded_b
            w._vlm_ls_gamma = g
            self._ls_jobs.setdefault(layer, []).append(dict(
                weight=w.data, gamma=g.data, bias=b.data if b is not None else None, shadow=w._vlm_bf16,
                bias_out=folded_b if b is not None else None, raw_w=w._vlm_raw, raw_b=raw_b if b is not None else None,
                dweight=w.grad, dbias=b.grad if b is not None else None, dgamma=g.grad))
        self._ls_buf = buf
        self.ls_pending = set()

    def shadow_reference(self):
        ref = self.flat_p[:self.numel].to(BF16)
        for jobs in getattr(self, "_ls_jobs", {}).values():
            for j in jobs:
                w = j["weight"]
                o = (w.data_ptr() - self.flat_p.data_ptr()) // 4
                ref[o:o + w.numel()] = (j["gamma"][:, None] * w).to(BF16).reshape(-1)
        return ref

    def refresh_folded(self):
        jobs = getattr(self, "_ls_jobs", None)
        if jobs:
            ops.layerscale_fold([j for layer in sorted(jobs) for j in jobs[layer]])

    def finish_layerscale(self, layer=None):
        pend = getattr(self, "ls_pending", None)
        if not pend:
            return
        layers = sorted(pend) if layer is None else ([layer] if layer in pend else [])
        if not layers:
            return
        jobs = [j for i in layers for j in self._ls_jobs.get(i, ())]
        side = wgrad_stream()
        if side is None:
            ops.layerscale_finish(jobs)
        else:
            side.wait_stream(torch.cuda.current_stream())
            with torch.cuda.stream(side):
                ops.layerscale_finish(jobs)
            if not _WGRAD["pending"]:
                torch.cuda.current_stream().wait_stream(side)
        for i in layers:
            pend.discard(i)

    def zero_grad(self):
        self.flat_g.zero_()
        if getattr(self, "ls_pending", None) or getattr(self, "_ls_armed", False):
            for jobs in getattr(self, "_ls_jobs", {}).values():
                for j in jobs:
                    j["raw_w"].zero_()
                    if j["raw_b"] is not None:
                        j["raw_b"].zero_()
            self.ls_pending.clear()
            self._ls_armed = False

    def slice_of(self, names):
        lo = min(self.offsets[n][0] for n in names)
        hi = max(self.offsets[n][0] + self.extent[n] for n in names)
        return lo, hi


_WGRAD = {"stream": None, "enabled": os.environ.get("VLM_WGRAD_STREAM", "1") != "0", "pending": False}


def wgrad_stream():
    if not _WGRAD["enabled"]:
        return None
    if _WGRAD["stream"] is None:
        _WGRAD["stream"] = torch.cuda.Stream()
    return _WGRAD["stream"]


def sync_wgrad():
    if _WGRAD["stream"] is not None:
        torch.cuda.current_stream().wait_stream(_WGRAD["stream"])
    _WGRAD["pending"] = False


def _arm_wgrad_join():
    if not _WGRAD["pending"]:
        _WGRAD["pending"] = True
        torch.autograd.Variable._execution_engine.queue_callback(sync_wgrad)


class _Side:

    def __init__(self, *tensors):
        self.s = wgrad_stream()
        self.tensors = tensors
        self.ctx = None

    def __enter__(self):
        if self.s is None:
            return self
        self.s.wait_stream(torch.cuda.current_stream())
        for t in self.tensors:
            t.record_stream(self.s)
        _arm_wgrad_join()
        self.ctx = torch.cuda.stream(self.s)
        self.ctx.__enter__()
        return self

    def __exit__(self, *a):
        if self.ctx is not None:
            self.ctx.__exit__(*a)
        return False


def wT16(p):
    s = getattr(p, "_vlm_bf16_t", None)
    if s is None:
        raise L.VlmError("weight has no transposed bf16 shadow: call model.setup_engine() on a CUDA model first")
    return s


def _gemm_rows(a, groups, out, *, act=L.ACT_NONE, aux=None, col_scale=None, row_scale=None, residual=None, col_sum_fold=None):
    if len(groups) > 1:
        return ops.gemm_grouped(a, groups, out, act=act, aux=aux, col_scale=col_scale, row_scale=row_scale,
                                residual=residual, col_sum_fold=col_sum_fold)
    (r0, r1, w, bias, col_sum), = groups

    def rows(t):
        return t[r0:r1] if t is not None else None

    return ops.gemm(a[r0:r1], w, out[r0:r1], bias=bias, act=act, aux=rows(aux), col_scale=col_scale,
                    row_scale=rows(row_scale), residual=rows(residual), col_sum=col_sum, col_sum_fold=col_sum_fold)


def _wgrad_rows(dy, x, groups):
    if len(groups) > 1:
        return ops.gemm_wgrad_grouped(dy, x, groups)
    (r0, r1, dw), = groups
    return ops.gemm(dy[r0:r1], x[r0:r1], dw, ta=True, tb=True, accumulate=True)


def w16(p):
    s = getattr(p, "_vlm_bf16", None)
    if s is None:
        raise L.VlmError("parameter has no bf16 shadow: call model.setup_engine() on a CUDA model first")
    return s


class RelPos:

    def __init__(self, bias_t, index16, index16_t, holder, cache_tag=None, cache=None):
        self.bias_t = bias_t
        self.index = index16
        self.index_t = index16_t
        self.holder = holder
        self._dense = {}
        self.cache_tag = cache_tag
        self.cache = cache

    def dense_for(self, seq, mode):
        key = (seq.n0, seq.n1, seq.pos1, mode)
        d = self._dense.get(key)
        if d is None:
            ck = self.cache_tag + key if self.cache_tag is not None and self.cache is not None else None
            cache = self.cache
            d = cache.get(ck) if ck is not None else None
            if d is None:
                with torch.no_grad():
                    d = ops.bias_dense(self.bias_t.detach(), self.index, seq, mode)
                _DENSE_STATS["built"] += 1
                if ck is not None:
                    for k in [k for k in cache if k[:2] != ck[:2]]:
                        del cache[k]
                    while len(cache) >= 8:
                        del cache[next(iter(cache))]
                    cache[ck] = d
            else:
                _DENSE_STATS["hits"] += 1
            self._dense[key] = d
        return d

    @property
    def dbias_t(self):
        return self.holder["dbias_t"]


_ZERO = {}


def _zero_scalar(dev):
    z = _ZERO.get(str(dev))
    if z is None:
        z = _ZERO[str(dev)] = torch.zeros((), device=dev, dtype=F32)
    return z


class _TableT(torch.autograd.Function):

    @staticmethod
    def forward(ctx, table, holder):
        ctx.holder, ctx.table = holder, table
        flat = getattr(table, "_vlm_flat", None)
        if flat is None or flat.dirty:
            return table.detach().t().contiguous()
        key = (flat.version, table._version, table.data_ptr())
        ent = getattr(flat, "table_t", None)
        if ent is None or ent[0] != key:
            ent = flat.table_t = (key, table.detach().t().contiguous())
        return ent[1].view_as(ent[1])

    @staticmethod
    def backward(ctx, g):
        acc = ctx.holder.pop("dbias_t", None)
        ctx.holder.pop("routed", None)
        table = ctx.table
        z = _ZERO.get(str(g.device))
        placeholder = z is not None and g.data_ptr() == z.data_ptr()
        if acc is None:
            return (None if placeholder else g.t()), None
        if getattr(table, "_vlm_flat", None) is not None and table.requires_grad and table.grad is not None:
            touch(table)
            table.grad.add_(acc.t() if placeholder else (acc + g).t())
            return None, None
        return (acc if placeholder else acc + g).t(), None


_DENSE_STATS = {"built": 0, "hits": 0}


def make_relpos(table, index16, index16_t, index_tag=None):
    holder = {}
    bias_t = _TableT.apply(table, holder)
    if torch.is_grad_enabled() and table.requires_grad:
        holder["dbias_t"] = torch.zeros_like(bias_t)
    flat = getattr(table, "_vlm_flat", None)
    ok = flat is not None and not flat.dirty and index_tag is not None
    tag = (flat.version, table._version, index_tag) if ok else None
    return RelPos(bias_t, index16, index16_t, holder, tag, flat.dense_cache if ok else None)


_KEEPS_CACHE = {}


class PassCtx:

    def __init__(self, seq: ops.Seq, num_heads: int, relpos: Optional[RelPos], keep0=None, keep1=None):
        self.seq = seq
        self.H = num_heads
        self.relpos = relpos
        self.keep0 = keep0
        self.keep1 = keep1
        self.gram = None
        self._row2sample = None
        self._dp_pool, self._dp_next = None, 0
        self._dp_sites, self._dp_all, self._dp_call = None, None, 0
        self.independent_segments = False
        self.uniform_source = None

    def row2sample(self, device):
        if self._row2sample is None:
            s = self.seq
            a = torch.arange(s.B, device=device).repeat_interleave(s.n0)
            b = torch.arange(s.B, device=device).repeat_interleave(s.n1)
            self._row2sample = torch.cat([a, b])
        return self._row2sample

    def plan_drop_path(self, probs):
        self._dp_sites = [float(p) for p in probs]

    def drop_path_rows(self, prob, training, device):
        if not training or prob <= 0.0:
            self._dp_call += 1
            return None
        s = self.seq
        rows = max(s.base0 + s.B * s.n0, s.base1 + s.B * s.n1)
        i = self._dp_call
        self._dp_call += 1
        if self._dp_sites is not None and i < len(self._dp_sites) and abs(self._dp_sites[i] - prob) < 1e-12:
            if self._dp_all is None:
                S = len(self._dp_sites)
                key = (tuple(self._dp_sites), str(device))
                keeps = _KEEPS_CACHE.get(key)
                if keeps is None:
                    keeps = _KEEPS_CACHE[key] = torch.tensor([1.0 - p if p > 0.0 else 1.0 for p in self._dp_sites],
                                                             dtype=F32).to(device)
                streams = 2 if (self.independent_segments and s.n0 and s.n1) else 1
                if self.uniform_source is not None:
                    u = self.uniform_source(self, S, streams).to(device=device, dtype=F32).contiguous()
                    assert u.shape == (streams, S, s.B), (u.shape, streams, S, s.B)
                else:
                    u = torch.rand(streams, S, s.B, device=device, dtype=F32)
                self._dp_all = ops.droppath_sites(u[0], u[1] if u.shape[0] == 2 else None, keeps, s,
                                                  torch.empty(S, rows, device=device, dtype=F32))
            return self._dp_all[i]
        if self._dp_pool is None or self._dp_next + 2 > self._dp_pool.shape[0]:
            self._dp_pool = torch.rand(64, s.B, device=device, dtype=F32)
            self._dp_next = 0
        u = self._dp_pool[self._dp_next]
        self._dp_next += 1
        out = torch.empty(rows, device=device, dtype=F32)
        if self.independent_segments and s.n0 and s.n1:
            u1 = self._dp_pool[self._dp_next]
            self._dp_next += 1
            ops.droppath_rows(u, 1.0 - prob, ops.Seq(s.B, s.n0, 0, base0=s.base0, base1=s.base1), out)
            return ops.droppath_rows(u1, 1.0 - prob, ops.Seq(s.B, 0, s.n1, base0=s.base0, base1=s.base1), out)
        return ops.droppath_rows(u, 1.0 - prob, s, out)


class ExpertWeights:

    __slots__ = ("n1w", "n1b", "qkvw", "qb", "vb", "projw", "projb", "n2w", "n2b", "fc1w", "fc1b", "fc2w", "fc2b",
                 "gram_names")


class GramCapture:

    def __init__(self):
        self.grams = {}

    def add(self, name, x):
        if name is None or x.shape[0] == 0:
            return
        D = x.shape[1]
        g = self.grams.get(name)
        if g is None:
            g = self.grams[name] = torch.zeros(D, D, device=x.device, dtype=torch.float64)
        ops.gram_accumulate(x if x.stride(1) == 1 else x.contiguous(), g)

    def all_reduce(self, group=None):
        import torch.distributed as dist
        if not (dist.is_available() and dist.is_initialized()) or dist.get_world_size(group) == 1:
            return self
        mine = {k: int(v.shape[0]) for k, v in self.grams.items()}
        every = [None] * dist.get_world_size(group)
        dist.all_gather_object(every, mine, group=group)
        dev = next(iter(self.grams.values())).device if self.grams else torch.device("cuda", torch.cuda.current_device())
        for d in every:
            for k, D in d.items():
                if k not in self.grams:
                    self.grams[k] = torch.zeros(D, D, device=dev, dtype=torch.float64)
        for k in sorted(self.grams):
            dist.all_reduce(self.grams[k], group=group)
        return self

    def state_dict(self):
        return {k: v.cpu() for k, v in self.grams.items()}


_DENSE_BIAS = True


def _segment_bias_grads(ranges, seq):
    qb, vb = [None, None], [None, None]
    for sgm, (base, n) in enumerate(((seq.base0, seq.n0), (seq.base1, seq.n1))):
        if n == 0:
            continue
        lo, hi = base, base + seq.B * n
        owner = [e for r0, r1, e in ranges if r0 <= lo and hi <= r1]
        if len(owner) != 1:
            return None, None, False
        if owner[0].qb is not None:
            qb[sgm], vb[sgm] = owner[0].qb.grad, owner[0].vb.grad
    return qb, vb, True


class BlockPlan:

    def __init__(self, ranges, mode, gamma1, gamma2, layer, drop_prob, eps):
        self.ranges = ranges
        self.mode = mode
        self.gamma1, self.gamma2 = gamma1, gamma2
        self.layer = layer
        self.drop_prob = drop_prob
        self.eps = eps


def _qkv_bias(e):
    if e.qb is None:
        return None
    view = getattr(e.qb, "_vlm_qkv_bias", None)
    if view is not None:
        return view
    return torch.cat((e.qb.detach(), torch.zeros_like(e.vb), e.vb.detach()))


_FOLD_LS = os.environ.get("VLM_FOLD_LAYERSCALE", "1") != "0"


def _folded(ranges):
    return _FOLD_LS and all(getattr(e.projw, "_vlm_raw", None) is not None and getattr(e.fc2w, "_vlm_raw", None) is not None
                            for _, _, e in ranges)


def _fb(b):
    return b._vlm_folded if b is not None else None


def _rb(b):
    return b._vlm_raw if b is not None else None


def _arm_layerscale_finish(flat):
    if getattr(flat, "_ls_armed", False):
        return
    flat._ls_armed = True

    def done():
        flat._ls_armed = False
        flat.finish_layerscale()
        sync_wgrad()

    torch.autograd.Variable._execution_engine.queue_callback(done)


def _ln2_bwd_scale1(dln, x1, st2, e, dx1, dx2, y1, g1, rs1, dy1, fold):
    sgamma, dsgamma, dsbias = (None, None, _rb(e.projb)) if y1 is None else (g1, g1.grad, e.projb.grad)
    if x1.shape[1] <= 768:
        ops.layernorm_bwd_scale(dln, x1, st2, e.n2w, dx1, dx2, e.n2w.grad, e.n2b.grad, y=y1, sgamma=sgamma, row_scale=rs1,
                                sdy=dy1, dsgamma=dsgamma, dsbias=dsbias, fold=fold)
    else:
        ops.layernorm_bwd(dln, x1, st2, e.n2w, dx1, dres=dx2, dgamma=e.n2w.grad, dbeta=e.n2b.grad, fold=fold)
        ops.layerscale_bwd(dx1, y1, sgamma, rs1, dy1, dsgamma, dsbias, fold=fold)


class _BlockFn(torch.autograd.Function):

    @staticmethod
    def forward(ctx, x, bias_t, plan: BlockPlan, pc: PassCtx, training: bool, hook):
        M, D = x.shape
        dev = x.device
        H = pc.H
        Fdim = plan.ranges[0][2].fc1w.shape[0]
        x = x.contiguous()
        ln1 = torch.empty(M, D, device=dev, dtype=BF16)
        st1 = torch.empty(M, 2, device=dev, dtype=F32)
        qkv = torch.empty(M, 3 * D, device=dev, dtype=BF16)
        rs1 = pc.drop_path_rows(plan.drop_prob, training, dev)
        rs2 = pc.drop_path_rows(plan.drop_prob, training, dev)
        rg = plan.ranges
        for r0, r1, e in rg:
            ops.layernorm_fwd(x[r0:r1], e.n1w, e.n1b, plan.eps, ln1[r0:r1], st1[r0:r1])
        _gemm_rows(ln1, [(r0, r1, w16(e.qkvw), _qkv_bias(e), None) for r0, r1, e in rg], qkv)
        o = torch.empty(M, D, device=dev, dtype=BF16)
        lse = torch.empty(H, M, device=dev, dtype=F32)
        rp = pc.relpos
        ops.attention_fwd(qkv, o, lse, pc.seq, H, bias_t=bias_t, head_row0=plan.layer * H,
                          rel_index=rp.index if rp is not None else None,
                          rel_index_t=rp.index_t if rp is not None else None, keep0=pc.keep0, keep1=pc.keep1,
                          mode=plan.mode, bias_dense=rp.dense_for(pc.seq, plan.mode) if rp is not None else None)
        x1 = torch.empty(M, D, device=dev, dtype=F32)
        folded = _folded(plan.ranges)
        y1 = torch.empty(M, D, device=dev, dtype=BF16) if not folded else None
        ln2 = torch.empty(M, D, device=dev, dtype=BF16)
        st2 = torch.empty(M, 2, device=dev, dtype=F32)
        h = torch.empty(M, Fdim, device=dev, dtype=BF16)
        a = torch.empty(M, Fdim, device=dev, dtype=BF16)
        x2 = torch.empty(M, D, device=dev, dtype=F32)
        y2 = torch.empty(M, D, device=dev, dtype=BF16) if not folded else None
        cs1, cs2 = (None, None) if folded else (plan.gamma1, plan.gamma2)
        pb = (lambda e: _fb(e.projb)) if folded else (lambda e: e.projb)
        fb2 = (lambda e: _fb(e.fc2b)) if folded else (lambda e: e.fc2b)
        _gemm_rows(o, [(r0, r1, w16(e.projw), pb(e), None) for r0, r1, e in rg], x1, col_scale=cs1, row_scale=rs1,
                   residual=x, aux=y1)
        for r0, r1, e in rg:
            ops.layernorm_fwd(x1[r0:r1], e.n2w, e.n2b, plan.eps, ln2[r0:r1], st2[r0:r1])
        _gemm_rows(ln2, [(r0, r1, w16(e.fc1w), e.fc1b, None) for r0, r1, e in rg], a, act=L.ACT_GELU_DERIV, aux=h)
        _gemm_rows(a, [(r0, r1, w16(e.fc2w), fb2(e), None) for r0, r1, e in rg], x2, col_scale=cs2, row_scale=rs2,
                   residual=x1, aux=y2)
        if pc.gram is not None:
            for r0, r1, e in plan.ranges:
                gn = e.gram_names
                if gn.get("qkv") or gn.get("fc1"):
                    t32 = torch.empty(r1 - r0, D, device=dev, dtype=F32)
                    st = torch.empty(r1 - r0, 2, device=dev, dtype=F32)
                    if gn.get("qkv"):
                        ops.layernorm_fwd(x[r0:r1], e.n1w, e.n1b, plan.eps, t32, st)
                        pc.gram.add(gn.get("qkv"), t32)
                    if gn.get("fc1"):
                        ops.layernorm_fwd(x1[r0:r1], e.n2w, e.n2b, plan.eps, t32, st)
                        pc.gram.add(gn.get("fc1"), t32)
                pc.gram.add(gn.get("proj"), o[r0:r1])
                pc.gram.add(gn.get("fc2"), a[r0:r1])
        ctx.plan, ctx.pc, ctx.hook = plan, pc, hook
        ctx.has_bias = bias_t is not None
        ctx.folded = folded
        ctx.save_for_backward(x, st1, ln1, qkv, o, lse, y1 if y1 is not None else x.new_empty(0), x1, st2, ln2, h, a,
                              y2 if y2 is not None else x.new_empty(0),
                              rs1 if rs1 is not None else x.new_empty(0), rs2 if rs2 is not None else x.new_empty(0),
                              bias_t if bias_t is not None else x.new_empty(0))
        return x2

    @staticmethod
    def backward(ctx, dx2):
        plan, pc = ctx.plan, ctx.pc
        x, st1, ln1, qkv, o, lse, y1, x1, st2, ln2, h, a, y2, rs1, rs2, bias_t = ctx.saved_tensors
        rs1 = rs1 if rs1.numel() else None
        rs2 = rs2 if rs2.numel() else None
        bias_t = bias_t if ctx.has_bias else None
        M, D = x.shape
        dev = x.device
        H = pc.H
        Fdim = h.shape[1]
        dx2 = dx2.contiguous()
        g1, g2 = plan.gamma1, plan.gamma2
        folded = ctx.folded
        if folded:
            y1 = y2 = None
            flat = plan.ranges[0][2].projw._vlm_flat
            _arm_layerscale_finish(flat)
        wg = (lambda w: w._vlm_raw) if folded else (lambda w: w.grad)
        touch(g1, g2)
        for _, _, e in plan.ranges:
            _touch_expert(e)
        dy2 = torch.empty(M, D, device=dev, dtype=BF16)
        dy1 = torch.empty(M, D, device=dev, dtype=BF16)
        dh = torch.empty(M, Fdim, device=dev, dtype=BF16)
        dln = torch.empty(M, D, device=dev, dtype=BF16)
        dx1 = torch.empty(M, D, device=dev, dtype=F32)
        fold = ops.FoldBatch(dev, D)
        rg = plan.ranges
        do = torch.empty(M, D, device=dev, dtype=BF16)
        for r0, r1, e in rg:
            rr = slice(r0, r1)
            if folded:
                ops.layerscale_bwd(dx2[rr], None, None, rs2[rr] if rs2 is not None else None, dy2[rr], None, _rb(e.fc2b), fold=fold)
            else:
                ops.layerscale_bwd(dx2[rr], y2[rr], g2, rs2[rr] if rs2 is not None else None, dy2[rr], g2.grad, e.fc2b.grad,
                                   fold=fold)
        _gemm_rows(dy2, [(r0, r1, wT16(e.fc2w), None, e.fc1b.grad) for r0, r1, e in rg], dh, act=L.ACT_MUL_AUX, aux=h,
                   col_sum_fold=fold)
        with _Side(dy2, a, dh, ln2):
            _wgrad_rows(dy2, a, [(r0, r1, wg(e.fc2w)) for r0, r1, e in rg])
            _wgrad_rows(dh, ln2, [(r0, r1, e.fc1w.grad) for r0, r1, e in rg])
        _gemm_rows(dh, [(r0, r1, wT16(e.fc1w), None, None) for r0, r1, e in rg], dln)
        for r0, r1, e in rg:
            rr = slice(r0, r1)
            _ln2_bwd_scale1(dln[rr], x1[rr], st2[rr], e, dx1[rr], dx2[rr], y1[rr] if y1 is not None else None, g1,
                            rs1[rr] if rs1 is not None else None, dy1[rr], fold)
        _gemm_rows(dy1, [(r0, r1, wT16(e.projw), None, None) for r0, r1, e in rg], do)
        with _Side(dy1, o):
            _wgrad_rows(dy1, o, [(r0, r1, wg(e.projw)) for r0, r1, e in rg])
        dqkv = torch.empty(M, 3 * D, device=dev, dtype=BF16)
        dln1 = torch.empty(M, D, device=dev, dtype=BF16)
        rp = pc.relpos
        qb_grads, vb_grads, fused_qv = _segment_bias_grads(rg, pc.seq)
        ops.attention_bwd(qkv, o, do, lse, dqkv, pc.seq, H, bias_t=bias_t, head_row0=plan.layer * H,
                          rel_index=rp.index if rp is not None else None,
                          rel_index_t=rp.index_t if rp is not None else None, keep0=pc.keep0, keep1=pc.keep1,
                          mode=plan.mode, dbias_t=rp.holder.get("dbias_t") if rp is not None else None,
                          dq_colsum=qb_grads, dv_colsum=vb_grads,
                          bias_dense=rp.dense_for(pc.seq, plan.mode) if rp is not None else None)
        dx = torch.empty(M, D, device=dev, dtype=F32)
        for r0, r1, e in rg:
            if e.qb is not None and not fused_qv:
                ops.colsum(dqkv[r0:r1, :D], e.qb.grad)
                ops.colsum(dqkv[r0:r1, 2 * D:], e.vb.grad)
        with _Side(dqkv, ln1):
            _wgrad_rows(dqkv, ln1, [(r0, r1, e.qkvw.grad) for r0, r1, e in rg])
        _gemm_rows(dqkv, [(r0, r1, wT16(e.qkvw), None, None) for r0, r1, e in rg], dln1)
        for r0, r1, e in rg:
            rr = slice(r0, r1)
            ops.layernorm_bwd(dln1[rr], x[rr], st1[rr], e.n1w, dx[rr], dres=dx1[rr], dgamma=e.n1w.grad, dbeta=e.n1b.grad,
                              fold=fold)
        fold.flush()
        if folded:
            flat.ls_pending.add(plan.layer)
        if ctx.hook is not None:
            ctx.hook(plan.layer)
        dbias = None
        if bias_t is not None and ctx.needs_input_grad[1] and rp is not None and not rp.holder.get("routed"):
            rp.holder["routed"] = True
            dbias = _zero_scalar(dev).expand_as(bias_t)
        return dx, dbias, None, None, None, None


def run_block(x, plan: BlockPlan, pc: PassCtx, training: bool, hook=None):
    bias_t = pc.relpos.bias_t if pc.relpos is not None else None
    return _BlockFn.apply(x, bias_t, plan, pc, training, hook)


class _LinearFn(torch.autograd.Function):

    @staticmethod
    def forward(ctx, x, weight, bias, act):
        x2 = x.reshape(-1, x.shape[-1])
        if x2.dtype != BF16:
            x2 = x2.to(BF16)
        if x2.stride(1) != 1 or (x2.shape[0] > 1 and x2.stride(0) < x2.shape[1]):
            x2 = x2.contiguous()
        M, K = x2.shape
        N = weight.shape[0]
        Np = (N + 63) // 64 * 64
        gelu = act == "gelu"
        buf = torch.empty(M, Np, device=x.device, dtype=BF16)
        pre = torch.empty(M, Np, device=x.device, dtype=BF16) if gelu else None
        ops.gemm(x2, w16(weight), buf[:, :N], bias=bias, act=L.ACT_GELU if gelu else L.ACT_NONE,
                 aux=pre[:, :N] if gelu else None)
        y = ops.tanh_fwd(buf[:, :N]) if act == "tanh" else None
        ctx.save_for_backward(x2, pre if gelu else (y if y is not None else x2.new_empty(0)))
        ctx.weight, ctx.bias, ctx.act, ctx.shape, ctx.N, ctx.Np = weight, bias, act, x.shape, N, Np
        return (y if y is not None else buf[:, :N]).view(*x.shape[:-1], N)

    @staticmethod
    def backward(ctx, gy):
        x2, saved = ctx.saved_tensors
        weight, bias, N, Np, act = ctx.weight, ctx.bias, ctx.N, ctx.Np, ctx.act
        M, K = x2.shape
        gy2 = gy.reshape(M, N)
        if gy2.dtype not in (BF16, F32):
            gy2 = gy2.float()
        if gy2.stride(1) != 1:
            gy2 = gy2.contiguous()
        if (act is None and gy2.dtype == BF16 and gy2.stride() == (Np, 1) and gy2.storage_offset() == 0
                and _is_padded_grad(gy2, M, Np)):
            dy = torch.as_strided(gy2, (M, Np), (Np, 1))
        elif act is None and Np == N and gy2.dtype == BF16:
            dy = gy2
        else:
            mode = {"gelu": ops.ACT_BWD_GELU, "tanh": ops.ACT_BWD_TANH, None: ops.ACT_BWD_NONE}[act]
            dy = ops.act_bwd(gy2, saved[:, :N] if act is not None else None, mode, Np)
        touch(weight if weight.requires_grad else None, bias if bias is not None and bias.requires_grad else None)
        if bias is not None and bias.requires_grad:
            if N % 8 == 0:
                ops.colsum(dy[:, :N], bias.grad)
            elif N <= 64:
                ops.colsum_small(dy[:, :N], bias.grad)
            elif bias.grad.is_contiguous():
                N8 = N // 8 * 8
                ops.colsum(dy[:, :N8], bias.grad[:N8])
                ops.colsum_small(dy[:, N8:N], bias.grad[N8:])
            else:
                bias.grad.add_(dy[:, :N].float().sum(0))
        if weight.requires_grad:
            ops.gemm(dy[:, :N], x2, weight.grad, ta=True, tb=True, accumulate=True)
        dx = None
        if ctx.needs_input_grad[0]:
            wpad = w16(weight) if Np == N else torch.as_strided(w16(weight), (Np, K), (K, 1))
            if Np >= 8192 and ((M + 127) // 128) * ((K + 127) // 128) <= 128:
                dx32 = torch.zeros(M, K, device=x2.device, dtype=F32)
                ops.gemm(dy, wpad, dx32, tb=True, accumulate=True)
                dx = dx32.to(BF16)
            else:
                dx = torch.empty(M, K, device=x2.device, dtype=BF16)
                ops.gemm(dy, wpad, dx, tb=True)
            dx = dx.view(ctx.shape)
        return dx, None, None, None


def linear(x, weight, bias=None, gelu=False, act=None):
    return _LinearFn.apply(x, weight, bias, "gelu" if gelu else act)


class _L2NormFn(torch.autograd.Function):

    @staticmethod
    def forward(ctx, x):
        x2 = x.reshape(-1, x.shape[-1])
        if x2.stride(-1) != 1:
            x2 = x2.contiguous()
        y, inv = ops.l2norm_fwd(x2)
        ctx.save_for_backward(y, inv)
        ctx.dtype, ctx.shape = x.dtype, x.shape
        return y.view(x.shape)

    @staticmethod
    def backward(ctx, g):
        y, inv = ctx.saved_tensors
        g2 = g.reshape(y.shape)
        if g2.dtype != F32 or not g2.is_contiguous():
            g2 = g2.float().contiguous()
        return ops.l2norm_bwd(g2, y, inv, ctx.dtype).view(ctx.shape)


_FUSED_LOSS = os.environ.get("VLM_FUSED_LOSS", "1") != "0"


def l2_normalize(x):
    if not _FUSED_LOSS or not x.is_cuda or x.dtype not in (BF16, F32):
        x = x.float()
        return x / x.norm(dim=-1, keepdim=True)
    return _L2NormFn.apply(x)


class _ContrastiveFn(torch.autograd.Function):

    @staticmethod
    def forward(ctx, img, txt, log_scale, others_img, others_txt):
        B = img.shape[0]
        all_img = img if others_img is None else torch.cat([img, others_img])
        all_txt = txt if others_txt is None else torch.cat([txt, others_txt])
        ls = log_scale.detach().reshape(1).float()
        out3, logits, d_img, d_txt = ops.contrastive(all_img.contiguous(), all_txt.contiguous(), B, ls)
        ctx.save_for_backward(out3, d_img, d_txt)
        ctx.ls_shape = log_scale.shape
        ctx.mark_non_differentiable(logits)
        ctx.set_materialize_grads(False)
        return out3[0], logits, out3[2]

    @staticmethod
    def backward(ctx, g_loss, _g_logits, g_scale):
        out3, d_img, d_txt = ctx.saved_tensors
        if g_loss is None:
            g_loss = torch.zeros((), device=out3.device, dtype=F32)
        gi, gt, gs = ops.scale_by_scalar([d_img, d_txt, out3[1:2]], g_loss.reshape(1).float())
        gs = gs.view(ctx.ls_shape)
        if g_scale is not None:
            gs = gs + (g_scale * out3[2]).view(ctx.ls_shape)
        return gi, gt, gs, None, None


def contrastive_loss(img, txt, log_scale, others_img=None, others_txt=None):
    return _ContrastiveFn.apply(img, txt, log_scale, others_img, others_txt)


_WVEC = {}


class _WeightedSumFn(torch.autograd.Function):

    @staticmethod
    def forward(ctx, weights, *terms):
        ctx.weights, ctx.dev = weights, terms[0].device
        return ops.weighted_sum([t.detach().reshape(1) for t in terms], weights)

    @staticmethod
    def backward(ctx, g):
        w = ctx.weights
        if all(x == 1.0 for x in w):
            return (None,) + (g,) * len(w)
        key = (w, str(ctx.dev))
        wv = _WVEC.get(key)
        if wv is None:
            if len(_WVEC) > 64:
                _WVEC.clear()
            wv = _WVEC[key] = torch.tensor(w, dtype=F32).to(ctx.dev)
        gw = g * wv
        return (None,) + tuple(gw[k] for k in range(len(w)))


def weighted_sum(terms, weights=None):
    terms = list(terms)
    weights = tuple(float(w) for w in (weights if weights is not None else [1.0] * len(terms)))
    if (_FUSED_LOSS and 1 <= len(terms) <= 8 and all(torch.is_tensor(t) and t.is_cuda and t.dtype == F32 and t.numel() == 1 for t in terms)):
        return _WeightedSumFn.apply(weights, *terms)
    out = 0
    for t, w in zip(terms, weights):
        out = out + (t if w == 1.0 else t * w)
    return out


class _SmallCrossEntropyFn(torch.autograd.Function):

    @staticmethod
    def forward(ctx, logits, labels):
        loss, d = ops.small_cross_entropy(logits, labels)
        ctx.save_for_backward(d)
        ctx.dtype = logits.dtype
        return loss[0]

    @staticmethod
    def backward(ctx, g):
        (d,) = ctx.saved_tensors
        (gd,) = ops.scale_by_scalar([d], g.reshape(1).float())
        return (gd if ctx.dtype == F32 else gd.to(ctx.dtype)), None


def small_cross_entropy(logits, labels):
    if (_FUSED_LOSS and logits.is_cuda and logits.dim() == 2 and logits.dtype in (BF16, F32) and logits.stride(1) == 1
            and logits.shape[1] <= 64 and labels.dtype == torch.int64):
        return _SmallCrossEntropyFn.apply(logits, labels.contiguous())
    return torch.nn.functional.cross_entropy(logits.float(), labels)


_PADDED_GRADS = {}


def _is_padded_grad(g, M, Np):
    ent = _PADDED_GRADS.pop(g.data_ptr(), None)
    return ent is not None and ent[0]() is not None and ent[1:] == (M, Np)


class _CrossEntropyFn(torch.autograd.Function):

    @staticmethod
    def forward(ctx, logits, labels, ignore_index):
        loss_rows, lse = ops.cross_entropy_fwd(logits, labels, ignore_index)
        out2 = ops.cross_entropy_reduce(loss_rows, labels, logits.shape[1], ignore_index)
        ctx.save_for_backward(logits, labels, lse, out2)
        ctx.ignore_index = ignore_index
        return out2[0]

    @staticmethod
    def backward(ctx, g):
        logits, labels, lse, out2 = ctx.saved_tensors
        (scale,) = ops.scale_by_scalar([out2[1:2]], g.reshape(1).float())
        d = ops.cross_entropy_bwd(logits, labels, lse, scale, ctx.ignore_index)
        if len(_PADDED_GRADS) > 64:
            _PADDED_GRADS.clear()
        _PADDED_GRADS[d.data_ptr()] = (weakref.ref(d._base), d.shape[0], d._base.shape[1])
        return d, None, None


def cross_entropy(logits, labels, ignore_index=-100):
    if (_FUSED_LOSS and logits.is_cuda and logits.dtype == BF16 and logits.dim() == 2 and logits.stride(1) == 1 and logits.stride(0) % 8 == 0
            and logits.data_ptr() % 16 == 0 and labels.dtype == torch.int64):
        return _CrossEntropyFn.apply(logits, labels.contiguous(), ignore_index)
    return torch.nn.functional.cross_entropy(logits.float(), labels, ignore_index=ignore_index)


class _LayerNormFn(torch.autograd.Function):

    @staticmethod
    def forward(ctx, x, weight, bias, eps, out_f32):
        shape = x.shape
        x2 = x.reshape(-1, shape[-1]).float().contiguous()
        M, D = x2.shape
        y = torch.empty(M, D, device=x.device, dtype=F32 if out_f32 else BF16)
        st = torch.empty(M, 2, device=x.device, dtype=F32)
        ops.layernorm_fwd(x2, weight, bias, eps, y, st)
        ctx.save_for_backward(x2, st)
        ctx.weight, ctx.bias, ctx.shape, ctx.in_dtype = weight, bias, shape, x.dtype
        return y.view(shape)

    @staticmethod
    def backward(ctx, gy):
        x2, st = ctx.saved_tensors
        M, D = x2.shape
        g2 = gy.reshape(M, D).contiguous()
        if g2.dtype not in (BF16, F32):
            g2 = g2.float()
        dx = torch.empty(M, D, device=x2.device, dtype=F32)
        touch(ctx.weight if ctx.weight.requires_grad else None, ctx.bias if ctx.bias.requires_grad else None)
        ops.layernorm_bwd(g2, x2, st, ctx.weight, dx, dgamma=ctx.weight.grad if ctx.weight.requires_grad else None,
                          dbeta=ctx.bias.grad if ctx.bias.requires_grad else None)
        return dx.view(ctx.shape).to(ctx.in_dtype), None, None, None, None


def layer_norm(x, weight, bias, eps, out_f32=False):
    return _LayerNormFn.apply(x, weight, bias, eps, out_f32)


def _rows2d(g, D):
    g2 = g.reshape(-1, D)
    if g2.dtype not in (BF16, F32):
        g2 = g2.float()
    return g2 if g2.stride(1) == 1 else g2.contiguous()


class _FeatureViewsFn(torch.autograd.Function):

    @staticmethod
    def forward(ctx, x, B, T, I):
        ctx.set_materialize_grads(False)
        D = x.shape[1]
        nt = B * T
        ctx.geom = (x.shape[0], D, B, T, I, x.dtype)
        text = x[:nt].view(B, T, D)
        image = x[nt:].view(B, I, D)
        tcls = torch.as_strided(x, (B, D), (T * D, 1), x.storage_offset()) if T else x[:0]
        icls = torch.as_strided(x, (B, D), (I * D, 1), x.storage_offset() + nt * D) if I else x[:0]
        return text, image, tcls, icls
# ... 192 lines not shown
```

vl-merging_amd/ops.py:

```python
import ctypes

import torch

from . import _lib as L

BF16 = torch.bfloat16
F32 = torch.float32


def _ld(t):
    if t.dim() != 2 or t.stride(1) != 1:
        raise L.VlmError("expected a 2-D tensor with unit inner stride, got shape %s strides %s"
                         % (tuple(t.shape), t.stride()))
    return t.stride(0) if t.shape[0] > 1 else max(t.stride(0), t.shape[1])


def gemm(a, b, out, ta=False, tb=False, *, bias=None, act=L.ACT_NONE, aux=None, col_scale=None, row_scale=None,
         residual=None, alpha=1.0, accumulate=False, col_sum=None, col_sum_fold=None):
    L.require_cuda(a, b, out, bias, aux, col_scale, row_scale, residual, col_sum)
    if a.dtype != BF16 or b.dtype != BF16:
        raise L.VlmError("gemm operands must be bfloat16")
    M, N = out.shape
    K = a.shape[0] if ta else a.shape[1]
    if (a.shape[1] if ta else a.shape[0]) != M:
        raise L.VlmError("gemm: A rows %s do not match M=%d" % (tuple(a.shape), M))
    kb, nb = (b.shape[0], b.shape[1]) if tb else (b.shape[1], b.shape[0])
    if nb != N or kb != K:
        raise L.VlmError("gemm: B shape %s incompatible with N=%d K=%d" % (tuple(b.shape), N, K))
    e = L.Epilogue()
    e.bias = bias.data_ptr() if bias is not None else 0
    e.col_scale = col_scale.data_ptr() if col_scale is not None else 0
    e.row_scale = row_scale.data_ptr() if row_scale is not None else 0
    e.residual = residual.data_ptr() if residual is not None else 0
    e.ld_res = _ld(residual) if residual is not None else 0
    e.aux = aux.data_ptr() if aux is not None else 0
    e.ld_aux = _ld(aux) if aux is not None else 0
    e.act = act
    e.alpha = alpha
    e.accumulate = 1 if accumulate else 0
    e.col_sum = col_sum.data_ptr() if col_sum is not None else 0
    region = None
    if col_sum is not None and col_sum_fold is not None and not ta and N % 128 == 0 and M >= 128:
        region = col_sum_fold.next_region()
        if region.numel() >= (M // 128) * 2 * N:
            e.col_sum_ws = region.data_ptr()
        else:
            region = None
    if ta and tb and out.dtype == F32 and K >= 2048 and bias is None and col_sum is None:
        ws = _splitk_workspace(out.device)
        e.splitk_ws = ws.data_ptr()
        e.splitk_ws_bytes = ws.numel() * 4
    if col_sum is not None and (col_sum.numel() < N or not col_sum.is_contiguous()):
        raise L.VlmError("gemm: col_sum must be a contiguous f32 vector of at least N elements")
    for t, dt in ((bias, F32), (col_scale, F32), (row_scale, F32), (residual, F32), (aux, BF16), (col_sum, F32)):
        if t is not None and t.dtype != dt:
            raise L.VlmError("gemm epilogue tensor has dtype %s, expected %s" % (t.dtype, dt))
    if out.dtype not in (BF16, F32):
        raise L.VlmError("gemm output must be bf16 or f32")
    rc = L.get_lib().vlm_gemm_bf16(int(ta), int(tb), M, N, K, L.ptr(a), _ld(a), L.ptr(b), _ld(b), L.ptr(out), _ld(out),
                                   int(out.dtype == F32), ctypes.byref(e), L.stream_ptr())
    L.check(rc, "vlm_gemm_bf16")
    if region is not None:
        col_sum_fold.add(region, M // 128, N, col_sum, None)
    return out


def gemm_grouped(a, groups, out, *, act=L.ACT_NONE, aux=None, col_scale=None, row_scale=None, residual=None, alpha=1.0,
                 col_sum_fold=None):
    L.require_cuda(a, out, aux, col_scale, row_scale, residual)
    if a.dtype != BF16:
        raise L.VlmError("gemm operands must be bfloat16")
    if len(groups) < 1 or len(groups) > L.GEMM_MAX_GROUPS:
        raise L.VlmError("gemm_grouped: 1..%d groups" % L.GEMM_MAX_GROUPS)
    M, N = out.shape
    K = a.shape[1]
    if a.shape[0] != M:
        raise L.VlmError("gemm_grouped: A rows %s do not match M=%d" % (tuple(a.shape), M))
    e = L.Epilogue()
    e.col_scale = col_scale.data_ptr() if col_scale is not None else 0
    e.row_scale = row_scale.data_ptr() if row_scale is not None else 0
    e.residual = residual.data_ptr() if residual is not None else 0
    e.ld_res = _ld(residual) if residual is not None else 0
    e.aux = aux.data_ptr() if aux is not None else 0
    e.ld_aux = _ld(aux) if aux is not None else 0
    e.act = act
    e.alpha = alpha
    for t, dt in ((col_scale, F32), (row_scale, F32), (residual, F32), (aux, BF16)):
        if t is not None and t.dtype != dt:
            raise L.VlmError("gemm epilogue tensor has dtype %s, expected %s" % (t.dtype, dt))
    if out.dtype not in (BF16, F32):
        raise L.VlmError("gemm output must be bf16 or f32")
    arr = (L.GemmGroup * len(groups))()
    folds = []
    prev = 0
    if col_sum_fold is not None and len(col_sum_fold.jobs) + len(groups) > col_sum_fold.MAX:
        col_sum_fold.flush()
    for g, (r0, r1, w, bias, col_sum) in zip(arr, groups):
        L.require_cuda(w, bias, col_sum)
        if w.dtype != BF16 or tuple(w.shape) != (N, K) or r0 < prev or r1 < r0 or r1 > M:
            raise L.VlmError("gemm_grouped: group (%d, %d) weight %s for N=%d K=%d M=%d" % (r0, r1, tuple(w.shape), N, K, M))
        prev = r1
        for t in (bias, col_sum):
            if t is not None and (t.dtype != F32 or t.numel() < N or not t.is_contiguous()):
                raise L.VlmError("gemm_grouped: bias / col_sum must be contiguous f32 vectors of at least N elements")
        g.row0, g.rows, g.B, g.ldb = r0, r1 - r0, w.data_ptr(), _ld(w)
        g.bias = bias.data_ptr() if bias is not None else None
        g.col_sum = col_sum.data_ptr() if col_sum is not None else None
        rows = r1 - r0
        if col_sum is not None and col_sum_fold is not None and N % 128 == 0 and rows >= 128:
            region = col_sum_fold.next_region()
            if region.numel() >= (rows // 128) * 2 * N:
                g.col_sum_ws = region.data_ptr()
                col_sum_fold.add(region, rows // 128, N, col_sum, None)
                folds.append(region)
    rc = L.get_lib().vlm_gemm_bf16_grouped(len(groups), arr, N, K, L.ptr(a), _ld(a), L.ptr(out), _ld(out),
                                           int(out.dtype == F32), ctypes.byref(e), L.stream_ptr())
    L.check(rc, "vlm_gemm_bf16_grouped")
    return out


def gemm_wgrad_grouped(dy, x, groups, accumulate=True):
    L.require_cuda(dy, x)
    if dy.dtype != BF16 or x.dtype != BF16 or dy.shape[0] != x.shape[0]:
        raise L.VlmError("gemm_wgrad_grouped: bf16 dy [tokens, M] and x [tokens, N]")
    M, N = dy.shape[1], x.shape[1]
    arr = (L.WgradGroup * len(groups))()
    prev, ldc = 0, None
    for g, (r0, r1, dW) in zip(arr, groups):
        L.require_cuda(dW)
        if dW.dtype != F32 or tuple(dW.shape) != (M, N) or r0 < prev or r1 < r0 or r1 > dy.shape[0]:
            raise L.VlmError("gemm_wgrad_grouped: group (%d, %d) gradient %s for M=%d N=%d" % (r0, r1, tuple(dW.shape), M, N))
        if ldc is not None and _ld(dW) != ldc:
            raise L.VlmError("gemm_wgrad_grouped: the groups' gradients must share one leading dimension")
        ldc = _ld(dW)
        prev = r1
        g.row0, g.rows, g.C, g.accumulate = r0, r1 - r0, dW.data_ptr(), int(bool(accumulate))
    ws = _splitk_workspace(dy.device)
    rc = L.get_lib().vlm_gemm_wgrad_grouped(len(groups), arr, M, N, L.ptr(dy), _ld(dy), L.ptr(x), _ld(x), ldc, L.ptr(ws),
                                            ws.numel() * 4, L.stream_ptr())
    L.check(rc, "vlm_gemm_wgrad_grouped")


_SPLITK_WS = {}
SPLITK_WS_BYTES = 96 << 20


def _splitk_workspace(device):
    key = (device.index, torch.cuda.current_stream().cuda_stream)
    ws = _SPLITK_WS.get(key)
    if ws is None:
        ws = _SPLITK_WS[key] = torch.empty(SPLITK_WS_BYTES // 4, device=device, dtype=F32)
    return ws


def layernorm_fwd(x, gamma, beta, eps, out, stats=None):
    L.require_cuda(x, gamma, beta, out, stats)
    M, D = x.shape
    rc = L.get_lib().vlm_layernorm_fwd(L.ptr(x), _ld(x), M, D, L.ptr(gamma), L.ptr(beta), eps, L.ptr(out), _ld(out),
                                       int(out.dtype == F32), L.ptr(stats), L.stream_ptr())
    L.check(rc, "vlm_layernorm_fwd")
    return out


_ROW_WS = {}


def _row_workspace(device, D, slot=0):
    key = (device.index, torch.cuda.current_stream().cuda_stream, slot)
    n = 1536 * 2 * max(D, 1024)
    ws = _ROW_WS.get(key)
    if ws is None or ws.numel() < n:
        ws = _ROW_WS[key] = torch.empty(n, device=device, dtype=F32)
    return ws


class FoldBatch:

    MAX = 16

    def __init__(self, device, D=1024):
        self.region = 1536 * 2 * max(D, 1024)
        key = ("fold", device.index, torch.cuda.current_stream().cuda_stream)
        ws = _ROW_WS.get(key)
        if ws is None or ws.numel() < self.MAX * self.region:
            ws = _ROW_WS[key] = torch.empty(self.MAX * self.region, device=device, dtype=F32)
        self.ws = ws
        self.jobs = []
        self.taken = 0

    def next_region(self):
        return self.next_regions(1)[0]

    def next_regions(self, n):
        if self.taken + n > self.MAX:
            self.flush()
        i = self.taken
        self.taken += n
        return [self.ws[(i + k) * self.region:(i + k + 1) * self.region] for k in range(n)]

    def add(self, region, nblocks, D, out0, out1):
        if nblocks > 0:
            self.jobs.append((region, nblocks, D, out0, out1))

    def flush(self):
        self.taken = 0
        if not self.jobs:
            return
        arr = (L.FoldJob * len(self.jobs))()
        for a, (region, nblocks, D, out0, out1) in zip(arr, self.jobs):
            a.partials, a.nblocks, a.D = region.data_ptr(), nblocks, D
            a.out0 = out0.data_ptr() if out0 is not None else None
            a.out1 = out1.data_ptr() if out1 is not None else None
        L.check(L.get_lib().vlm_colreduce_batch(arr, len(self.jobs), L.stream_ptr()), "vlm_colreduce_batch")
        self.jobs = []


def layernorm_bwd(dy, x, stats, gamma, dx, dres=None, dgamma=None, dbeta=None, fold=None):
    L.require_cuda(dy, x, stats, gamma, dx, dres, dgamma, dbeta)
    M, D = x.shape
    ws = fold.next_region() if fold is not None else _row_workspace(x.device, D)
    nb = ctypes.c_int(0)
    rc = L.get_lib().vlm_layernorm_bwd(L.ptr(dy), _ld(dy), int(dy.dtype == F32), L.ptr(x), _ld(x), L.ptr(stats),
                                       L.ptr(gamma), M, D, L.ptr(dres), _ld(dres) if dres is not None else 0,
                                       L.ptr(dx), _ld(dx), L.ptr(dgamma), L.ptr(dbeta), L.ptr(ws), ws.numel() * 4,
                                       ctypes.byref(nb) if fold is not None else None, L.stream_ptr())
    L.check(rc, "vlm_layernorm_bwd")
    if fold is not None:
        fold.add(ws, nb.value, D, dgamma, dbeta)
    return dx


def layernorm_bwd_scale(dy, x, stats, gamma, dx, dres, dgamma, dbeta, *, y, sgamma, row_scale, sdy, dsgamma=None, dsbias=None,
                        fold=None):
    L.require_cuda(dy, x, stats, gamma, dx, dres, dgamma, dbeta, y, sgamma, row_scale, sdy, dsgamma, dsbias)
    M, D = x.shape
    nb = ctypes.c_int(0)
    if fold is not None:
        ws, ws2 = fold.next_regions(2)
    else:
        ws, ws2 = _row_workspace(x.device, D), _row_workspace(x.device, D, slot=1)
    sc = L.LayerScale()
    sc.y, sc.ldy, sc.gamma, sc.row_scale = L.ptr(y), _ld(y) if y is not None else 0, L.ptr(sgamma), L.ptr(row_scale)
    sc.dy, sc.lddy, sc.dgamma, sc.dbias = L.ptr(sdy), _ld(sdy), L.ptr(dsgamma), L.ptr(dsbias)
    sc.workspace, sc.workspace_bytes = L.ptr(ws2), ws2.numel() * 4
    rc = L.get_lib().vlm_layernorm_bwd_scale(L.ptr(dy), _ld(dy), int(dy.dtype == F32), L.ptr(x), _ld(x), L.ptr(stats),
                                             L.ptr(gamma), M, D, L.ptr(dres), _ld(dres) if dres is not None else 0,
                                             L.ptr(dx), _ld(dx), L.ptr(dgamma), L.ptr(dbeta), L.ptr(ws), ws.numel() * 4,
                                             ctypes.byref(sc), ctypes.byref(nb) if fold is not None else None, L.stream_ptr())
    L.check(rc, "vlm_layernorm_bwd_scale")
    if fold is not None:
        fold.add(ws, nb.value if (dgamma is not None or dbeta is not None) else 0, D, dgamma, dbeta)
        fold.add(ws2, nb.value if (dsgamma is not None or dsbias is not None) else 0, D, dsgamma, dsbias)
    return dx


def layerscale_bwd(dx, y, gamma, row_scale, dy, dgamma=None, dbias=None, fold=None):
    L.require_cuda(dx, y, gamma, row_scale, dy, dgamma, dbias)
    M, D = dx.shape
    ws = fold.next_region() if fold is not None else _row_workspace(dx.device, D)
    nb = ctypes.c_int(0)
    rc = L.get_lib().vlm_layerscale_bwd(L.ptr(dx), _ld(dx), L.ptr(y), _ld(y) if y is not None else 0, L.ptr(gamma), L.ptr(row_scale), M, D,
                                        L.ptr(dy), _ld(dy), L.ptr(dgamma), L.ptr(dbias), L.ptr(ws), ws.numel() * 4,
                                        ctypes.byref(nb) if fold is not None else None, L.stream_ptr())
    L.check(rc, "vlm_layerscale_bwd")
    if fold is not None:
        fold.add(ws, nb.value, D, dgamma, dbias)
    return dy


def embedding_bwd(gy, ids, dW, padding_idx=-1):
    L.require_cuda(gy, ids, dW)
    n, D = gy.shape
    assert gy.dtype == F32 and dW.dtype == F32 and ids.dtype == torch.int64 and ids.numel() == n and gy.stride(1) == 1
    L.check(L.get_lib().vlm_embedding_bwd(L.ptr(gy), _ld(gy), L.ptr(ids), n, D, int(padding_idx), L.ptr(dW), _ld(dW),
                                          dW.shape[0], L.stream_ptr()), "vlm_embedding_bwd")
    return dW


def cross_entropy_fwd(logits, labels, ignore_index=-100):
    L.require_cuda(logits, labels)
    rows, V = logits.shape
    if logits.dtype != BF16 or labels.dtype != torch.int64 or labels.numel() != rows or not labels.is_contiguous():
        raise L.VlmError("cross_entropy: bf16 logits [rows, V], contiguous int64 labels [rows]")
    loss_rows = torch.empty(rows, device=logits.device, dtype=F32)
    lse = torch.empty(rows, device=logits.device, dtype=F32)
    L.check(L.get_lib().vlm_cross_entropy_fwd(L.ptr(logits), _ld(logits), rows, V, L.ptr(labels), int(ignore_index), L.ptr(loss_rows),
                                              L.ptr(lse), L.stream_ptr()), "vlm_cross_entropy_fwd")
    return loss_rows, lse


def cross_entropy_bwd(logits, labels, lse, scale, ignore_index=-100):
    L.require_cuda(logits, labels, lse, scale)
    rows, V = logits.shape
    Vp = (V + 63) // 64 * 64
    buf = torch.empty(rows, Vp, device=logits.device, dtype=BF16)
    L.check(L.get_lib().vlm_cross_entropy_bwd(L.ptr(logits), _ld(logits), rows, V, L.ptr(labels), int(ignore_index), L.ptr(lse),
                                              L.ptr(scale), L.ptr(buf), Vp, L.stream_ptr()), "vlm_cross_entropy_bwd")
    return buf[:, :V]


def l2norm_fwd(x):
    L.require_cuda(x)
    rows, D = x.shape
    if x.dtype not in (BF16, F32) or x.stride(1) != 1:
        raise L.VlmError("l2norm: bf16 / fp32 [rows, D] with unit column stride")
    y = torch.empty(rows, D, device=x.device, dtype=F32)
    inv = torch.empty(rows, device=x.device, dtype=F32)
    L.check(L.get_lib().vlm_l2norm_fwd(L.ptr(x), int(x.dtype == BF16), _ld(x), rows, D, L.ptr(y), L.ptr(inv), L.stream_ptr()), "vlm_l2norm_fwd")
    return y, inv


def l2norm_bwd(g, y, inv, dtype):
    L.require_cuda(g, y, inv)
    rows, D = y.shape
    if g.dtype != F32 or not g.is_contiguous() or g.shape != y.shape:
        raise L.VlmError("l2norm_bwd: contiguous fp32 gradient of y's shape")
    dx = torch.empty(rows, D, device=y.device, dtype=dtype)
    L.check(L.get_lib().vlm_l2norm_bwd(L.ptr(g), L.ptr(y), L.ptr(inv), rows, D, L.ptr(dx), int(dtype == BF16), D, L.stream_ptr()), "vlm_l2norm_bwd")
    return dx


def contrastive(all_img, all_txt, B, log_scale):
    L.require_cuda(all_img, all_txt, log_scale)
    n, D = all_img.shape
    for t in (all_img, all_txt):
        if t.dtype != F32 or not t.is_contiguous() or t.shape != (n, D):
            raise L.VlmError("contrastive: contiguous fp32 [n, D] features")
    if log_scale.dtype != F32 or log_scale.numel() != 1:
        raise L.VlmError("contrastive: log_scale is one fp32 number")
    dev = all_img.device
    logits = torch.empty(n, n, device=dev, dtype=F32)
    out3 = torch.empty(3, device=dev, dtype=F32)
    d_img = torch.empty(B, D, device=dev, dtype=F32)
    d_txt = torch.empty(B, D, device=dev, dtype=F32)
    ws = torch.empty(max(1, L.get_lib().vlm_contrastive_ws_floats(n)), device=dev, dtype=F32)
    L.check(L.get_lib().vlm_contrastive(L.ptr(all_img), L.ptr(all_txt), n, B, D, L.ptr(log_scale), L.ptr(logits), L.ptr(out3), L.ptr(d_img),
                                        L.ptr(d_txt), L.ptr(ws), L.stream_ptr()), "vlm_contrastive")
    return out3, logits, d_img, d_txt


def small_cross_entropy(logits, labels):
    L.require_cuda(logits, labels)
    rows, V = logits.shape
    if logits.dtype not in (BF16, F32) or logits.stride(1) != 1 or labels.dtype != torch.int64 or not labels.is_contiguous() or labels.numel() != rows:
        raise L.VlmError("small_cross_entropy: bf16 / fp32 logits [rows, V], contiguous int64 labels [rows]")
    loss = torch.empty(1, device=logits.device, dtype=F32)
    d = torch.empty(rows, V, device=logits.device, dtype=F32)
    L.check(L.get_lib().vlm_small_cross_entropy(L.ptr(logits), int(logits.dtype == BF16), _ld(logits), rows, V, L.ptr(labels), L.ptr(loss),
                                                L.ptr(d), L.stream_ptr()), "vlm_small_cross_entropy")
    return loss, d


def cross_entropy_reduce(loss_rows, labels, V, ignore_index=-100):
    L.require_cuda(loss_rows, labels)
    out2 = torch.empty(2, device=loss_rows.device, dtype=F32)
    L.check(L.get_lib().vlm_cross_entropy_reduce(L.ptr(loss_rows), L.ptr(labels), loss_rows.numel(), int(V), int(ignore_index), L.ptr(out2),
                                                 L.stream_ptr()), "vlm_cross_entropy_reduce")
    return out2


def scale_by_scalar(tensors, scalar):
    L.require_cuda(scalar, *tensors)
    k = len(tensors)
    if k == 0:
        return []
    if k > 4 or any(t.dtype != F32 or not t.is_contiguous() for t in tensors) or scalar.dtype != F32:
        raise L.VlmError("scale_by_scalar: up to four contiguous fp32 tensors and an fp32 device scalar")
    outs = [torch.empty_like(t) for t in tensors]
    P = ctypes.c_void_p * k
    I = ctypes.c_int * k
    L.check(L.get_lib().vlm_scale_by_scalar(P(*[L.ptr(t) for t in tensors]), P(*[L.ptr(o) for o in outs]), I(*[t.numel() for t in tensors]), k,
                                            L.ptr(scalar), L.stream_ptr()), "vlm_scale_by_scalar")
    return outs


_FRONT_WS = {}


def _front_ws(kind, D, device):
    key = (kind, D, str(device))
    ws = _FRONT_WS.get(key)
    if ws is None:
        lib = L.get_lib()
        n = lib.vlm_text_rows_bwd_ws_floats(D) if kind == "text" else lib.vlm_image_rows_bwd_ws_floats(D)
        ws = _FRONT_WS[key] = torch.empty(max(1, n), device=device, dtype=F32)
    return ws


def _rowvec(t, D, what):
    if t is None:
        return 0
    if t.dtype != F32 or t.numel() != D or not t.is_contiguous():
        raise L.VlmError("%s: a contiguous fp32 vector of %d elements" % (what, D))
    return L.ptr(t)


def text_rows_fwd(ids, word, add0, gamma, beta, eps, out, u=None, p=0.0, scale=1.0, add1=None):
    L.require_cuda(ids, word, add0, gamma, beta, out, u, add1)
    n, D = out.shape
    if ids.dtype != torch.int64 or ids.numel() != n or not ids.is_contiguous():
        raise L.VlmError("text_rows: contiguous int64 ids, one per output row")
    if word.dtype != F32 or word.shape[1] != D or word.stride(1) != 1 or out.dtype != F32 or out.stride(1) != 1:
        raise L.VlmError("text_rows: fp32 word table [V, D] and fp32 output rows")
    if u is not None and (u.dtype != F32 or u.numel() != n * D or not u.is_contiguous()):
        raise L.VlmError("text_rows: u is a contiguous fp32 [n, D]")
    stats = torch.empty(n, 2, device=out.device, dtype=F32)
    L.check(L.get_lib().vlm_text_rows_fwd(L.ptr(ids), n, L.ptr(word), _ld(word), _rowvec(add0, D, "add0"), _rowvec(gamma, D, "gamma"),
                                          _rowvec(beta, D, "beta"), float(eps), L.ptr(u) if u is not None else 0, float(p), float(scale),
                                          _rowvec(add1, D, "add1"), L.ptr(out), _ld(out), L.ptr(stats), D, L.stream_ptr()), "vlm_text_rows_fwd")
    return stats


def text_rows_bwd(g, ids, word, add0, gamma, stats, u, p, scale, d_word, padding_idx, d_add1, d_beta, d_gamma, d_add0):
    L.require_cuda(g, ids, word, add0, gamma, stats, u, d_word, d_add1, d_beta, d_gamma, d_add0)
    n, D = g.shape
    if g.dtype != F32 or g.stride(1) != 1:
        raise L.VlmError("text_rows_bwd: fp32 gradient rows with unit column stride")
    if d_word is not None and (d_word.dtype != F32 or d_word.shape != word.shape or d_word.stride() != word.stride()):
        raise L.VlmError("text_rows_bwd: d_word has the word table's layout")
    L.check(L.get_lib().vlm_text_rows_bwd(L.ptr(g), _ld(g), L.ptr(ids), n, L.ptr(word), _ld(word), _rowvec(add0, D, "add0"),
                                          _rowvec(gamma, D, "gamma"), L.ptr(stats), L.ptr(u) if u is not None else 0, float(p), float(scale), D,
                                          L.ptr(d_word) if d_word is not None else 0, -1 if padding_idx is None else int(padding_idx),
                                          _rowvec(d_add1, D, "d_add1"), _rowvec(d_beta, D, "d_beta"), _rowvec(d_gamma, D, "d_gamma"),
                                          _rowvec(d_add0, D, "d_add0"), L.ptr(_front_ws("text", D, g.device)), L.stream_ptr()),
            "vlm_text_rows_bwd")


def image_rows_prep(conv_bias, type_row, cls):
    L.require_cuda(conv_bias, type_row, cls)
    D = cls.numel()
    out2 = torch.empty(2, D, device=cls.device, dtype=F32)
    L.check(L.get_lib().vlm_image_rows_prep(_rowvec(conv_bias, D, "conv_bias"), _rowvec(type_row, D, "type_row"), _rowvec(cls.reshape(-1), D, "cls"),
                                            D, L.ptr(out2), L.stream_ptr()), "vlm_image_rows_prep")
    return out2


def image_lead_rows(x, B, rows, lead):
    L.require_cuda(x, lead)
    D = x.shape[1]
    if x.dtype != F32 or x.stride(1) != 1 or x.shape[0] != B * rows:
        raise L.VlmError("image_lead_rows: fp32 [B * rows, D]")
    L.check(L.get_lib().vlm_image_lead_rows(L.ptr(x), _ld(x), B, rows, D, _rowvec(lead, D, "lead"), L.stream_ptr()), "vlm_image_lead_rows")


def image_rows_bwd(g, B, rows, d_bias, d_type_row, d_cls):
    L.require_cuda(g, d_bias, d_type_row, d_cls)
    n, D = g.shape
    if g.dtype != F32 or g.stride(1) != 1 or n != B * rows:
        raise L.VlmError("image_rows_bwd: fp32 [B * rows, D] gradient rows")
    g16 = torch.empty(n, D, device=g.device, dtype=BF16)
    L.check(L.get_lib().vlm_image_rows_bwd(L.ptr(g), _ld(g), B, rows, D, L.ptr(g16), _rowvec(d_bias, D, "d_bias"),
                                           _rowvec(d_type_row, D, "d_type_row"), _rowvec(d_cls.reshape(-1) if d_cls is not None else None, D, "d_cls"),
                                           L.ptr(_front_ws("image", D, g.device)), L.stream_ptr()), "vlm_image_rows_bwd")
    return g16
# ... 452 lines not shown
```

Before: 336.8.

## Batch all block weight-gradient GEMMs into one planned split-K multi-problem launch

Replaces the per-layer grouped wgrad calls (fc2, fc1, proj, qkv issued separately on a side stream) with one multi-problem wgrad launch per block. A host-side planner breaks every problem into tile groups and K-segments, balances them across CUs and XCDs, and uploads a segment table through a pinned host ring buffer. A per-tile split-K reduce kernel then folds the partials. This is meant to fill the GPU better and cut launch and reduce overhead. In exchange it adds host planning and H2D upload cost on every call and delays all wgrads until after the qkv backward.

```diff
diff --git a/include/vlm_hip.h b/include/vlm_hip.h
--- a/include/vlm_hip.h
+++ b/include/vlm_hip.h
@@ -116,6 +116,26 @@
 } vlm_wgrad_group_t;
 int vlm_gemm_wgrad_grouped(int n_groups, const vlm_wgrad_group_t* groups, int M, int N, const void* A, int lda,
                            const void* B, int ldb, int ldc, float* splitk_ws, uint64_t splitk_ws_bytes, void* stream);
+#define VLM_WGRAD_MAX_PROBLEMS (4 * VLM_GEMM_MAX_GROUPS)
+typedef struct {
+  const void* A;
+  const void* B;
+  float* C;
+  int32_t lda, ldb, ldc;
+  int32_t M, N;
+  int32_t row0, rows;
+  int32_t accumulate;
+  int32_t reserved;
+} vlm_wgrad_problem_t;
+int vlm_gemm_wgrad_multi(int n_problems, const vlm_wgrad_problem_t* problems, float* splitk_ws, uint64_t splitk_ws_bytes,
+                         void* stream);
+typedef struct {
+  int32_t problem, m0, n0;
+  int32_t k0, k1;
+  int32_t slot, part, block;
+} vlm_wgrad_segment_t;
+int vlm_gemm_wgrad_plan(int n_problems, const vlm_wgrad_problem_t* problems, int n_cu, vlm_wgrad_segment_t* segs, int max_segs,
+                        int* n_blocks, uint64_t* ws_bytes);
 int vlm_gemm_set_big_tile_mode(int mode);
 
 int vlm_layernorm_fwd(const float* x, int ldx, int M, int D, const float* gamma, const float* beta, float eps,
diff --git a/vl-merging_amd/_lib.py b/vl-merging_amd/_lib.py
--- a/vl-merging_amd/_lib.py
+++ b/vl-merging_amd/_lib.py
@@ -76,6 +76,20 @@
 class WgradGroup(ctypes.Structure):
     _fields_ = [("row0", ctypes.c_int32), ("rows", ctypes.c_int32), ("C", c_void_p), ("accumulate", ctypes.c_int32),
                 ("reserved", ctypes.c_int32)]
+
+
+WGRAD_MAX_PROBLEMS = 4 * GEMM_MAX_GROUPS
+
+
+class WgradProblem(ctypes.Structure):
+    _fields_ = [("A", c_void_p), ("B", c_void_p), ("C", c_void_p), ("lda", ctypes.c_int32), ("ldb", ctypes.c_int32),
+                ("ldc", ctypes.c_int32), ("M", ctypes.c_int32), ("N", ctypes.c_int32), ("row0", ctypes.c_int32),
+                ("rows", ctypes.c_int32), ("accumulate", ctypes.c_int32), ("reserved", ctypes.c_int32)]
+
+
+class WgradSegment(ctypes.Structure):
+    _fields_ = [("problem", ctypes.c_int32), ("m0", ctypes.c_int32), ("n0", ctypes.c_int32), ("k0", ctypes.c_int32),
+                ("k1", ctypes.c_int32), ("slot", ctypes.c_int32), ("part", ctypes.c_int32), ("block", ctypes.c_int32)]
 
 
 class FoldJob(ctypes.Structure):
@@ -144,6 +158,9 @@
                                       ctypes.POINTER(Epilogue), c_void_p]),
     "vlm_gemm_wgrad_grouped": (c_int, [c_int, ctypes.POINTER(WgradGroup), c_int, c_int, c_void_p, c_int, c_void_p, c_int, c_int,
                                        c_void_p, c_u64, c_void_p]),
+    "vlm_gemm_wgrad_multi": (c_int, [c_int, ctypes.POINTER(WgradProblem), c_void_p, c_u64, c_void_p]),
+    "vlm_gemm_wgrad_plan": (c_int, [c_int, ctypes.POINTER(WgradProblem), c_int, ctypes.POINTER(WgradSegment), c_int,
+                                    ctypes.POINTER(c_int), ctypes.POINTER(c_u64)]),
     "vlm_attention_fwd": (c_int, [ctypes.POINTER(AttnDesc), c_void_p, c_int, c_void_p, c_void_p]),
     "vlm_attention_bwd_ws_floats": (c_size_t, [ctypes.POINTER(AttnDesc), c_int]),
     "vlm_attention_bwd": (c_int, [ctypes.POINTER(AttnDesc), c_void_p, c_int, c_void_p, c_int, c_void_p, c_void_p, c_size_t,
diff --git a/vl-merging_amd/csrc/gemm.hip b/vl-merging_amd/csrc/gemm.hip
--- a/vl-merging_amd/csrc/gemm.hip
+++ b/vl-merging_amd/csrc/gemm.hip
@@ -1,6 +1,10 @@
 #include "vlm_common.h"
 #include "vlm_diag.h"
+#include <algorithm>
 #include <atomic>
+#include <cstring>
+#include <mutex>
+#include <vector>
 
 #define GEMM_BM 128
 #define GEMM_BN 128
@@ -115,8 +119,21 @@
   int ldb, row0, row_end, tile0;
 };
 
-struct gemmT_group_t {
-  int row0, row_end, item0, kps, slice0;
+struct wgrad_seg_t {
+  const void* A;
+  const void* B;
+  int lda, ldb;
+  int m0, n0;
+  int k_first, k_end;
+  int nk;
+  int slot;
+  int m_rows;
+  int pad[3];
+};
+struct wgrad_tile_t {
+  float* C;
+  int ldc, m0, n0, m_rows;
+  int slot0, n_parts, accumulate, pad;
 };
 
 struct gemm_params_t {
@@ -131,7 +148,7 @@
   int splits, ksteps_per_split;
   int n_groups;
   gemm_group_t grp[VLM_GEMM_MAX_GROUPS];
-  gemmT_group_t grpT[VLM_GEMM_MAX_GROUPS];
+  const wgrad_seg_t* segs;
   VLM_DIAG_GEMM_FIELD
 };
 
@@ -940,38 +957,44 @@
   const int lane = tid & 63;
   const int wave = __builtin_amdgcn_readfirstlane(tid >> 6);
   const int wm = wave >> 1, wn = wave & 1;
-  const uint32_t ntile = p.tiles_m * p.tiles_n;
-  const uint32_t q8 = gridDim.x >> 3, r8 = gridDim.x & 7, xcd = blockIdx.x & 7;
-  uint32_t item = (xcd < r8 ? xcd * (q8 + 1) : r8 * (q8 + 1) + (xcd - r8) * q8) + (blockIdx.x >> 3);
-  uint32_t k_base = 0, k_end = (uint32_t)p.K, slice0 = 0;
-  int nk = p.ksteps_per_split;
+  const void* gA = p.A;
+  const void* gB = p.B;
+  uint32_t lda = (uint32_t)p.lda, ldb = (uint32_t)p.ldb;
+  uint32_t m0, n0, k_first, k_end, slot;
+  int nk, m_rows = p.M;
   if constexpr (GROUPED) {
-    int g = 0;
-#pragma unroll
-    for (int i = 1; i < VLM_GEMM_MAX_GROUPS; ++i)
-      if (i < p.n_groups && item >= (uint32_t)p.grpT[i].item0) g = i;
-    const gemmT_group_t G = p.grpT[g];
-    item -= (uint32_t)G.item0;
-    k_base = (uint32_t)G.row0;
-    k_end = (uint32_t)G.row_end;
-    nk = G.kps;
-    slice0 = (uint32_t)G.slice0;
-  }
-  const uint32_t split = item / ntile, tile = item - split * ntile;
-  const uint32_t tm = tile / p.tiles_n, tn = tile - tm * p.tiles_n;
-  const uint32_t m0 = tm * BIG_BM, n0 = tn * BIG_BN;
-  const uint32_t k_first = k_base + split * (uint32_t)nk * BIG_BK;
+    const wgrad_seg_t& S = p.segs[blockIdx.x];
+    nk = S.nk;
+    if (nk == 0) return;
+    gA = S.A; gB = S.B;
+    lda = (uint32_t)S.lda; ldb = (uint32_t)S.ldb;
+    m0 = (uint32_t)S.m0; n0 = (uint32_t)S.n0;
+    k_first = (uint32_t)S.k_first; k_end = (uint32_t)S.k_end;
+    slot = (uint32_t)S.slot;
+    m_rows = S.m_rows;
+  } else {
+    const uint32_t ntile = p.tiles_m * p.tiles_n;
+    const uint32_t q8 = gridDim.x >> 3, r8 = gridDim.x & 7, xcd = blockIdx.x & 7;
+    const uint32_t item = (xcd < r8 ? xcd * (q8 + 1) : r8 * (q8 + 1) + (xcd - r8) * q8) + (blockIdx.x >> 3);
+    nk = p.ksteps_per_split;
+    slot = item / ntile;
+    const uint32_t tile = item - slot * ntile;
+    const uint32_t tm = tile / p.tiles_n, tn = tile - tm * p.tiles_n;
+    m0 = tm * BIG_BM; n0 = tn * BIG_BN;
+    k_first = slot * (uint32_t)nk * BIG_BK;
+    k_end = (uint32_t)p.K;
+  }
   const __amdgpu_buffer_rsrc_t ra =
-      __builtin_amdgcn_make_buffer_rsrc(const_cast<void*>(p.A), 0, (int)((uint64_t)k_end * p.lda * 2), 0x00020000);
+      __builtin_amdgcn_make_buffer_rsrc(const_cast<void*>(gA), 0, (int)((uint64_t)k_end * lda * 2), 0x00020000);
   const __amdgpu_buffer_rsrc_t rb =
-      __builtin_amdgcn_make_buffer_rsrc(const_cast<void*>(p.B), 0, (int)((uint64_t)k_end * p.ldb * 2), 0x00020000);
+      __builtin_amdgcn_make_buffer_rsrc(const_cast<void*>(gB), 0, (int)((uint64_t)k_end * ldb * 2), 0x00020000);
 
   uint32_t offa[4], offb[4], wr_off[4];
 #pragma unroll
   for (int u = 0; u < 4; ++u) {
     const uint32_t row = 2 * (wave + 4 * u) + (lane >> 5), c16 = lane & 31;
-    offa[u] = ((k_first + row) * (uint32_t)p.lda + m0 + c16 * 8) * 2;
-    offb[u] = ((k_first + row) * (uint32_t)p.ldb + n0 + c16 * 8) * 2;
+    offa[u] = ((k_first + row) * lda + m0 + c16 * 8) * 2;
+    offb[u] = ((k_first + row) * ldb + n0 + c16 * 8) * 2;
     wr_off[u] = row * 512 + (((c16 >> 1) ^ ((row & 3) | (((row >> 3) & 1) << 2))) << 5) + (c16 & 1) * 16;
   }
   uint32_t rda[8], rdb[8];
@@ -993,7 +1016,7 @@
       acc10[i][j] = (f32x4){0.f, 0.f, 0.f, 0.f};
       acc11[i][j] = (f32x4){0.f, 0.f, 0.f, 0.f};
     }
-  const uint32_t stepa = BIG_BK * (uint32_t)p.lda * 2, stepb = BIG_BK * (uint32_t)p.ldb * 2;
+  const uint32_t stepa = BIG_BK * lda * 2, stepb = BIG_BK * ldb * 2;
   bf16x8 fa0[8], fb0[8], fa1[8], fb1[8];
   u32x4 ra0[4], rb0[4], ra1[4], rb1[4];
 #define BIGT_TR(PTR) __builtin_amdgcn_ds_read_tr16_b64_v4i16((lds_s16x4*)(PTR))
@@ -1057,9 +1080,10 @@
   BIGT_STEP(kt + 3, 0, 0, 0, fa1, fb1, fa0, fb0, ra1, rb1, sA1, sB1, sA0, sB0)
 
   gemm_params_t pl = p;
-  pl.C = reinterpret_cast<float*>(p.C) + (size_t)(slice0 + split) * p.M * p.N;
-  pl.ldc = p.N;
-  const uint32_t mw0 = m0 + wm * 128, nw0 = n0 + wn * 128;
+  pl.C = reinterpret_cast<float*>(p.C) + (GROUPED ? (size_t)slot * (BIG_BM * BIG_BN) : (size_t)slot * p.M * p.N);
+  pl.M = m_rows;
+  pl.ldc = GROUPED ? BIG_BN : p.N;
+  const uint32_t mw0 = (GROUPED ? 0 : m0) + wm * 128, nw0 = (GROUPED ? 0 : n0) + wn * 128;
   unsigned char* const wl = epl + wave * EPIL_WAVE_BYTES;
   big_epilogue_t<true, false, 0, 128, 0, true> ep(pl, wl, mw0, nw0, lane);
   epil_in_t inA, inB;
@@ -1077,19 +1101,15 @@
   *reinterpret_cast<f32x4*>(C + m * ldc + n) = t;
 }
 
-struct splitk_groups_t {
-  float* C[VLM_GEMM_MAX_GROUPS];
-  int slice0[VLM_GEMM_MAX_GROUPS], splits[VLM_GEMM_MAX_GROUPS], accumulate[VLM_GEMM_MAX_GROUPS];
-};
-__global__ __launch_bounds__(256) void splitk_reduce_grouped_kernel(const float* __restrict__ ws, const splitk_groups_t g, int M, int N, int ldc) {
-  const size_t i = (size_t)blockIdx.x * 256 + threadIdx.x, per = (size_t)M * N / 4;
-  if (i >= per) return;
-  const int gi = blockIdx.y;
-  float* const C = g.C[gi];
-  const size_t e = i * 4, m = e / N, n = e - m * N;
-  f32x4 t = g.accumulate[gi] ? *reinterpret_cast<const f32x4*>(C + m * ldc + n) : (f32x4){0.f, 0.f, 0.f, 0.f};
-  for (int s = 0; s < g.splits[gi]; ++s) t += *reinterpret_cast<const f32x4*>(ws + (size_t)(g.slice0[gi] + s) * M * N + e);
-  *reinterpret_cast<f32x4*>(C + m * ldc + n) = t;
+__global__ __launch_bounds__(256) void splitk_reduce_tiles_kernel(const float* __restrict__ ws, const wgrad_tile_t* __restrict__ tiles) {
+  const wgrad_tile_t T = tiles[blockIdx.y];
+  const int r = blockIdx.x * 4 + (threadIdx.x >> 6), c = (threadIdx.x & 63) * 4;
+  if (r >= T.m_rows) return;
+  float* const dst = T.C + (size_t)(T.m0 + r) * T.ldc + T.n0 + c;
+  f32x4 t = T.accumulate ? *reinterpret_cast<const f32x4*>(dst) : (f32x4){0.f, 0.f, 0.f, 0.f};
+  const float* src = ws + (size_t)T.slot0 * (BIG_BM * BIG_BN) + r * BIG_BN + c;
+  for (int s = 0; s < T.n_parts; ++s) t += *reinterpret_cast<const f32x4*>(src + (size_t)s * (BIG_BM * BIG_BN));
+  *reinterpret_cast<f32x4*>(dst) = t;
 }
 
 static int plan_cus() {
@@ -1315,95 +1335,233 @@
   return VLM_OK;
 }
 
+#define WGRAD_GROUP_EDGE 3
+#define WGRAD_MIN_UNITS 4
+#define WGRAD_XCDS 8
+
+struct wgrad_plan_t {
+  std::vector<vlm_wgrad_segment_t> segs;
+  int n_blocks = 0, n_tiles = 0, n_slots = 0;
+  uint64_t table_bytes = 0, partial_off = 0, ws_bytes = 0;
+};
+
+static uint64_t wgrad_align(uint64_t x, uint64_t a) { return (x + a - 1) / a * a; }
+
+static void wgrad_make_plan(int n, const vlm_wgrad_problem_t* P, int n_cu, wgrad_plan_t& out) {
+  struct grp_t { int prob, tm0, tn0, gm, gn, units, nk, slot0, parts; };
+  struct gseg_t { int g, u0, u1, part; };
+  std::vector<grp_t> groups;
+  int G = 1;
+  long total = 0;
+  for (int i = 0; i < n; ++i) {
+    if (P[i].rows <= 0 || P[i].M <= 0 || P[i].N <= 0) continue;
+    const int tiles_m = (P[i].M + BIG_BM - 1) / BIG_BM, tiles_n = (P[i].N + BIG_BN - 1) / BIG_BN;
+    const int nk = (P[i].rows + BIG_BK - 1) / BIG_BK;
+    for (int tm0 = 0; tm0 < tiles_m; tm0 += WGRAD_GROUP_EDGE)
+      for (int tn0 = 0; tn0 < tiles_n; tn0 += WGRAD_GROUP_EDGE) {
+        const int gm = std::min(WGRAD_GROUP_EDGE, tiles_m - tm0), gn = std::min(WGRAD_GROUP_EDGE, tiles_n - tn0);
+        groups.push_back(grp_t{i, tm0, tn0, gm, gn, (nk + 1) / 2, nk, 0, 0});
+        G = std::max(G, gm * gn);
+        total += (nk + 1) / 2;
+        out.n_tiles += gm * gn;
+      }
+  }
+  if (groups.empty()) return;
+  const long shares = std::max(1, n_cu / G);
+  std::vector<gseg_t> gs;
+  long base = 0, w = 1;
+  for (size_t gi = 0; gi < groups.size(); ++gi) {
+    grp_t& g = groups[gi];
+    int prev = 0, part = 0;
+    for (; w < shares && w * total / shares < base + g.units; ++w) {
+      const int rel = (int)(w * total / shares - base);
+      if (rel - prev >= WGRAD_MIN_UNITS && g.units - rel >= WGRAD_MIN_UNITS) {
+        gs.push_back(gseg_t{(int)gi, prev, rel, part++});
+        prev = rel;
+      }
+    }
+    gs.push_back(gseg_t{(int)gi, prev, g.units, part++});
+    g.parts = part;
+    g.slot0 = out.n_slots;
+    out.n_slots += part * g.gm * g.gn;
+    base += g.units;
+  }
+  std::stable_sort(gs.begin(), gs.end(), [](const gseg_t& a, const gseg_t& b) { return a.u1 - a.u0 > b.u1 - b.u0; });
+  int fill[WGRAD_XCDS] = {};
+  for (size_t j = 0; j < gs.size(); ++j) {
+    const grp_t& g = groups[gs[j].g];
+    const int xcd = (int)(j % WGRAD_XCDS);
+    for (int t = 0; t < g.gm * g.gn; ++t) {
+      vlm_wgrad_segment_t sg;
+      sg.problem = g.prob;
+      sg.m0 = (g.tm0 + t / g.gn) * BIG_BM;
+      sg.n0 = (g.tn0 + t % g.gn) * BIG_BN;
+      sg.k0 = 2 * gs[j].u0;
+      sg.k1 = std::min(2 * gs[j].u1, g.nk);
+      sg.slot = g.slot0 + t * g.parts + gs[j].part;
+      sg.part = gs[j].part;
+      sg.block = WGRAD_XCDS * fill[xcd]++ + xcd;
+      out.segs.push_back(sg);
+    }
+  }
+  out.n_blocks = WGRAD_XCDS * *std::max_element(fill, fill + WGRAD_XCDS);
+  out.table_bytes = (uint64_t)out.n_blocks * sizeof(wgrad_seg_t) + (uint64_t)out.n_tiles * sizeof(wgrad_tile_t);
+  out.partial_off = wgrad_align(out.table_bytes, 4096);
+  out.ws_bytes = out.partial_off + (uint64_t)out.n_slots * (BIG_BM * BIG_BN * 4);
+}
+
+static bool wgrad_problems_ok(int n, const vlm_wgrad_problem_t* P) {
+  if (n < 1 || n > VLM_WGRAD_MAX_PROBLEMS || !P) return false;
+  for (int i = 0; i < n; ++i)
+    if (P[i].M < 0 || P[i].N < 0 || P[i].rows < 0 || P[i].row0 < 0) return false;
+  return true;
+}
+
+extern "C" int vlm_gemm_wgrad_plan(int n_problems, const vlm_wgrad_problem_t* problems, int n_cu, vlm_wgrad_segment_t* segs,
+                                   int max_segs, int* n_blocks, uint64_t* ws_bytes) {
+  if (!wgrad_problems_ok(n_problems, problems) || n_cu < 1) return VLM_ERR_ARG;
+  wgrad_plan_t plan;
+  wgrad_make_plan(n_problems, problems, n_cu, plan);
+  if (n_blocks) *n_blocks = plan.n_blocks;
+  if (ws_bytes) *ws_bytes = plan.ws_bytes;
+  if (segs) {
+    if ((size_t)max_segs < plan.segs.size()) return VLM_ERR_WORKSPACE;
+    std::copy(plan.segs.begin(), plan.segs.end(), segs);
+  }
+  return (int)plan.segs.size();
+}
+
+#define WGRAD_RING 32
+#define WGRAD_IMG_BYTES (64 << 10)
+#define WGRAD_MAX_DEVICES 16
+struct wgrad_ring_t {
+  std::mutex mu;
+  unsigned char* host = nullptr;
+  hipEvent_t ev[WGRAD_RING];
+  bool armed[WGRAD_RING] = {};
+  int next = 0;
+};
+static wgrad_ring_t g_wgrad_ring[WGRAD_MAX_DEVICES];
+
+static int wgrad_upload(const std::vector<unsigned char>& img, void* dst, hipStream_t s) {
+  int dev = 0;
+  if (hipGetDevice(&dev) != hipSuccess || dev < 0 || dev >= WGRAD_MAX_DEVICES) return VLM_ERR_LAUNCH;
+  wgrad_ring_t& R = g_wgrad_ring[dev];
+  std::lock_guard<std::mutex> lock(R.mu);
+  if (!R.host) {
+    if (hipHostMalloc(reinterpret_cast<void**>(&R.host), (size_t)WGRAD_RING * WGRAD_IMG_BYTES, hipHostMallocDefault) != hipSuccess) {
+      R.host = nullptr;
+      return VLM_ERR_LAUNCH;
+    }
+    for (int i = 0; i < WGRAD_RING; ++i)
+      if (hipEventCreateWithFlags(&R.ev[i], hipEventDisableTiming) != hipSuccess) return VLM_ERR_LAUNCH;
+  }
+  const int i = R.next;
+  R.next = (i + 1) % WGRAD_RING;
+  if (R.armed[i] && hipEventSynchronize(R.ev[i]) != hipSuccess) return VLM_ERR_LAUNCH;
+  unsigned char* const src = R.host + (size_t)i * WGRAD_IMG_BYTES;
+  memcpy(src, img.data(), img.size());
+  if (hipMemcpyAsync(dst, src, img.size(), hipMemcpyHostToDevice, s) != hipSuccess) return VLM_ERR_LAUNCH;
+  if (hipEventRecord(R.ev[i], s) != hipSuccess) return VLM_ERR_LAUNCH;
+  R.armed[i] = true;
+  return VLM_OK;
+}
+
+extern "C" int vlm_gemm_wgrad_multi(int n_problems, const vlm_wgrad_problem_t* problems, float* splitk_ws, uint64_t splitk_ws_bytes,
+                                    void* stream) {
+  if (!wgrad_problems_ok(n_problems, problems)) return VLM_ERR_ARG;
+  hipStream_t s = (hipStream_t)stream;
+  const vlm_wgrad_problem_t* P = problems;
+  bool served = gemm_big_mode() > 0 && splitk_ws && ((uintptr_t)splitk_ws & 255) == 0;
+  int live = 0;
+  for (int i = 0; i < n_problems; ++i) {
+    if (P[i].M == 0 || P[i].N == 0) continue;
+    if (!P[i].C) return VLM_ERR_ARG;
+    if (P[i].rows == 0) {
+      if (!P[i].accumulate && hipMemset2DAsync(P[i].C, (size_t)P[i].ldc * 4, 0, (size_t)P[i].N * 4, P[i].M, s) != hipSuccess)
+        return VLM_ERR_LAUNCH;
+      continue;
+    }
+    if (!P[i].A || !P[i].B || (P[i].lda & 7) || (P[i].ldb & 7) || ((uintptr_t)P[i].A & 15) || ((uintptr_t)P[i].B & 15)) return VLM_ERR_ARG;
+    ++live;
+    if ((P[i].N % BIG_BN) || (P[i].ldc % 4) || ((uintptr_t)P[i].C & 15) || (uint64_t)P[i].rows * P[i].lda * 2 >= (1ull << 31) ||
+        (uint64_t)P[i].rows * P[i].ldb * 2 >= (1ull << 31))
+      served = false;
+  }
+  if (live == 0) return VLM_OK;
+  if (served) {
+    wgrad_plan_t plan;
+    wgrad_make_plan(n_problems, P, plan_cus(), plan);
+    if (plan.ws_bytes <= splitk_ws_bytes && plan.table_bytes <= WGRAD_IMG_BYTES) {
+      std::vector<unsigned char> img(plan.table_bytes, 0);
+      wgrad_seg_t* const segs = reinterpret_cast<wgrad_seg_t*>(img.data());
+      wgrad_tile_t* const tiles = reinterpret_cast<wgrad_tile_t*>(img.data() + (size_t)plan.n_blocks * sizeof(wgrad_seg_t));
+      int n_tiles = 0;
+      for (const vlm_wgrad_segment_t& g : plan.segs) {
+        const vlm_wgrad_problem_t& Q = P[g.problem];
+        wgrad_seg_t& S = segs[g.block];
+        S.A = reinterpret_cast<const unsigned char*>(Q.A) + (size_t)Q.row0 * Q.lda * 2;
+        S.B = reinterpret_cast<const unsigned char*>(Q.B) + (size_t)Q.row0 * Q.ldb * 2;
+        S.lda = Q.lda; S.ldb = Q.ldb;
+        S.m0 = g.m0; S.n0 = g.n0;
+        S.k_first = g.k0 * BIG_BK;
+        S.k_end = std::min(Q.rows, g.k1 * BIG_BK);
+        const int len = g.k1 - g.k0;
+        S.nk = std::max(4, len + (len & 1));
+        S.slot = g.slot;
+        S.m_rows = std::min(BIG_BM, Q.M - g.m0);
+        if (g.part == 0) {
+          wgrad_tile_t& T = tiles[n_tiles++];
+          T.C = Q.C; T.ldc = Q.ldc; T.m0 = g.m0; T.n0 = g.n0; T.m_rows = S.m_rows;
+          T.slot0 = g.slot; T.n_parts = 0; T.accumulate = Q.accumulate;
+        }
+      }
+      for (int t = 0; t < n_tiles; ++t)
+        for (const vlm_wgrad_segment_t& g : plan.segs)
+          if (g.slot >= tiles[t].slot0 && g.slot - g.part == tiles[t].slot0) tiles[t].n_parts = std::max(tiles[t].n_parts, g.part + 1);
+      if (n_tiles != plan.n_tiles) return VLM_ERR_LAUNCH;
+      const int rc = wgrad_upload(img, splitk_ws, s);
+      if (rc) return rc;
+      gemm_params_t p{};
+      p.C = reinterpret_cast<unsigned char*>(splitk_ws) + plan.partial_off;
+      p.epi.alpha = 1.0f;
+      p.epi.reserved = 1;
+      p.segs = reinterpret_cast<const wgrad_seg_t*>(splitk_ws);
+      hipLaunchKernelGGL(vlm_gemm_bigT_kernel<true>, dim3(plan.n_blocks), dim3(GEMM_THREADS), 0, s, p);
+      VLM_CHECK_LAUNCH();
+      hipLaunchKernelGGL(splitk_reduce_tiles_kernel, dim3(BIG_BM / 4, n_tiles), dim3(256), 0, s,
+                         reinterpret_cast<const float*>(p.C),
+                         reinterpret_cast<const wgrad_tile_t*>(reinterpret_cast<unsigned char*>(splitk_ws) + (size_t)plan.n_blocks * sizeof(wgrad_seg_t)));
+      VLM_CHECK_LAUNCH();
+      return VLM_OK;
+    }
+  }
+  for (int i = 0; i < n_problems; ++i) {
+    if (P[i].rows == 0 || P[i].M == 0 || P[i].N == 0) continue;
+    vlm_epilogue_t e{};
+    e.alpha = 1.0f;
+    e.accumulate = P[i].accumulate;
+    e.splitk_ws = splitk_ws;
+    e.splitk_ws_bytes = splitk_ws_bytes;
+    const size_t r0 = (size_t)P[i].row0;
+    const int rc = vlm_gemm_bf16(1, 1, P[i].M, P[i].N, P[i].rows, reinterpret_cast<const unsigned char*>(P[i].A) + r0 * P[i].lda * 2, P[i].lda,
+                                 reinterpret_cast<const unsigned char*>(P[i].B) + r0 * P[i].ldb * 2, P[i].ldb, P[i].C, P[i].ldc, 1, &e, stream);
+    if (rc) return rc;
+  }
+  return VLM_OK;
+}
+
 extern "C" int vlm_gemm_wgrad_grouped(int n_groups, const vlm_wgrad_group_t* groups, int M, int N, const void* A, int lda,
                                       const void* B, int ldb, int ldc, float* splitk_ws, uint64_t splitk_ws_bytes, void* stream) {
   if (n_groups < 1 || n_groups > VLM_GEMM_MAX_GROUPS || !groups || M < 0 || N < 0) return VLM_ERR_ARG;
   int prev_end = 0;
+  vlm_wgrad_problem_t P[VLM_GEMM_MAX_GROUPS];
   for (int g = 0; g < n_groups; ++g) {
     if (groups[g].row0 < prev_end || groups[g].rows < 0 || !groups[g].C) return VLM_ERR_ARG;
     prev_end = groups[g].row0 + groups[g].rows;
+    P[g] = vlm_wgrad_problem_t{A, B, groups[g].C, lda, ldb, ldc, M, N, groups[g].row0, groups[g].rows, groups[g].accumulate, 0};
   }
   if (M == 0 || N == 0) return VLM_OK;
   if (!A || !B || (lda & 7) || (ldb & 7) || ((uintptr_t)A & 15) || ((uintptr_t)B & 15)) return VLM_ERR_ARG;
-  hipStream_t s = (hipStream_t)stream;
-  for (int g = 0; g < n_groups; ++g)
-    if (groups[g].rows == 0 && !groups[g].accumulate &&
-        hipMemset2DAsync(groups[g].C, (size_t)ldc * 4, 0, (size_t)N * 4, M, s) != hipSuccess)
-      return VLM_ERR_LAUNCH;
-  const int K_total = prev_end;
-  bool big = gemm_big_mode() > 0 && splitk_ws && (N % BIG_BN) == 0 && (ldc % 4) == 0 && (uint64_t)M * N * 4 < (1ull << 31) &&
-             (uint64_t)K_total * lda * 2 < (1ull << 31) && (uint64_t)K_total * ldb * 2 < (1ull << 31);
-  gemm_params_t p;
-  p.A = A; p.B = B; p.C = splitk_ws;
-  p.M = M; p.N = N; p.K = K_total;
-  p.lda = lda; p.ldb = ldb; p.ldc = N;
-  p.epi = vlm_epilogue_t{};
-  p.epi.alpha = 1.0f;
-  p.epi.reserved = 1;
-  p.tiles_m = (M + BIG_BM - 1) / BIG_BM;
-  p.tiles_n = (N + BIG_BN - 1) / BIG_BN;
-  p.group_m = 1;
-  p.splits = 1;
-  p.ksteps_per_split = 0;
-  p.n_groups = 0;
-  splitk_groups_t rg{};
-  if (big) {
-    const int ntile = p.tiles_m * p.tiles_n;
-    const int cus = plan_cus();
-    long total_steps = 0;
-    int live = 0;
-    for (int g = 0; g < n_groups; ++g)
-      if (groups[g].rows > 0) { total_steps += (groups[g].rows + BIG_BK - 1) / BIG_BK; ++live; }
-    if (live == 0) return VLM_OK;
-    if ((long)live * ntile > cus) big = false;
-    long target = (total_steps * ntile + cus - 1) / cus;
-    if (target < 16) target = 16;
-    for (; big; target += 2) {
-      long items = 0;
-      for (int g = 0; g < n_groups; ++g)
-        if (groups[g].rows > 0) items += (((groups[g].rows + BIG_BK - 1) / BIG_BK + target - 1) / target) * ntile;
-      if (items <= cus) break;
-    }
-    int item0 = 0, slice0 = 0;
-    for (int g = 0; g < n_groups && big; ++g) {
-      const vlm_wgrad_group_t& G = groups[g];
-      if (G.rows == 0) continue;
-      if ((uintptr_t)G.C & 15) { big = false; break; }
-      const int nk = (G.rows + BIG_BK - 1) / BIG_BK;
-      int splits = (int)((nk + target - 1) / target);
-      int kps = (nk + splits - 1) / splits;
-      kps += kps & 1;
-      if (kps < 4) kps = 4;
-      splits = (nk + kps - 1) / kps;
-      const int i = p.n_groups++;
-      p.grpT[i] = gemmT_group_t{G.row0, G.row0 + G.rows, item0, kps, slice0};
-      rg.C[i] = G.C; rg.slice0[i] = slice0; rg.splits[i] = splits; rg.accumulate[i] = G.accumulate;
-      item0 += splits * ntile;
-      slice0 += splits;
-    }
-    if (big && (size_t)slice0 * M * N * 4 > (size_t)splitk_ws_bytes) big = false;
-    if (big) {
-      hipLaunchKernelGGL(vlm_gemm_bigT_kernel<true>, dim3(item0), dim3(GEMM_THREADS), 0, s, p);
-      VLM_CHECK_LAUNCH();
-      const size_t per = (size_t)M * N / 4;
-      hipLaunchKernelGGL(splitk_reduce_grouped_kernel, dim3((unsigned)((per + 255) / 256), p.n_groups), dim3(256), 0, s,
-                         reinterpret_cast<const float*>(splitk_ws), rg, M, N, ldc);
-      VLM_CHECK_LAUNCH();
-      return VLM_OK;
-    }
-  }
-  for (int g = 0; g < n_groups; ++g) {
-    const vlm_wgrad_group_t& G = groups[g];
-    if (G.rows == 0) continue;
-    vlm_epilogue_t e{};
-    e.alpha = 1.0f;
-    e.accumulate = G.accumulate;
-    e.splitk_ws = splitk_ws;
-    e.splitk_ws_bytes = splitk_ws_bytes;
-    const size_t r0 = (size_t)G.row0;
-    const int rc = vlm_gemm_bf16(1, 1, M, N, G.rows, reinterpret_cast<const unsigned char*>(A) + r0 * lda * 2, lda,
-                                 reinterpret_cast<const unsigned char*>(B) + r0 * ldb * 2, ldb, G.C, ldc, 1, &e, stream);
-    if (rc) return rc;
-  }
-  return VLM_OK;
-}
+  return vlm_gemm_wgrad_multi(n_groups, P, splitk_ws, splitk_ws_bytes, stream);
+}
diff --git a/vl-merging_amd/engine.py b/vl-merging_amd/engine.py
--- a/vl-merging_amd/engine.py
+++ b/vl-merging_amd/engine.py
@@ -252,13 +252,6 @@
 
     return ops.gemm(a[r0:r1], w, out[r0:r1], bias=bias, act=act, aux=rows(aux), col_scale=col_scale,
                     row_scale=rows(row_scale), residual=rows(residual), col_sum=col_sum, col_sum_fold=col_sum_fold)
-
-
-def _wgrad_rows(dy, x, groups):
-    if len(groups) > 1:
-        return ops.gemm_wgrad_grouped(dy, x, groups)
-    (r0, r1, dw), = groups
-    return ops.gemm(dy[r0:r1], x[r0:r1], dw, ta=True, tb=True, accumulate=True)
 
 
 def w16(p):
@@ -650,17 +643,12 @@
                                    fold=fold)
         _gemm_rows(dy2, [(r0, r1, wT16(e.fc2w), None, e.fc1b.grad) for r0, r1, e in rg], dh, act=L.ACT_MUL_AUX, aux=h,
                    col_sum_fold=fold)
-        with _Side(dy2, a, dh, ln2):
-            _wgrad_rows(dy2, a, [(r0, r1, wg(e.fc2w)) for r0, r1, e in rg])
-            _wgrad_rows(dh, ln2, [(r0, r1, e.fc1w.grad) for r0, r1, e in rg])
         _gemm_rows(dh, [(r0, r1, wT16(e.fc1w), None, None) for r0, r1, e in rg], dln)
         for r0, r1, e in rg:
             rr = slice(r0, r1)
             _ln2_bwd_scale1(dln[rr], x1[rr], st2[rr], e, dx1[rr], dx2[rr], y1[rr] if y1 is not None else None, g1,
                             rs1[rr] if rs1 is not None else None, dy1[rr], fold)
         _gemm_rows(dy1, [(r0, r1, wT16(e.projw), None, None) for r0, r1, e in rg], do)
-        with _Side(dy1, o):
-            _wgrad_rows(dy1, o, [(r0, r1, wg(e.projw)) for r0, r1, e in rg])
         dqkv = torch.empty(M, 3 * D, device=dev, dtype=BF16)
         dln1 = torch.empty(M, D, device=dev, dtype=BF16)
         rp = pc.relpos
@@ -676,8 +664,9 @@
             if e.qb is not None and not fused_qv:
                 ops.colsum(dqkv[r0:r1, :D], e.qb.grad)
                 ops.colsum(dqkv[r0:r1, 2 * D:], e.vb.grad)
-        with _Side(dqkv, ln1):
-            _wgrad_rows(dqkv, ln1, [(r0, r1, e.qkvw.grad) for r0, r1, e in rg])
+        with _Side(dy2, a, dh, ln2, dy1, o, dqkv, ln1):
+            ops.gemm_wgrad_multi([q for r0, r1, e in rg for q in ((dy2, a, r0, r1, wg(e.fc2w)), (dh, ln2, r0, r1, e.fc1w.grad),
+                                                                   (dy1, o, r0, r1, wg(e.projw)), (dqkv, ln1, r0, r1, e.qkvw.grad))])
         _gemm_rows(dqkv, [(r0, r1, wT16(e.qkvw), None, None) for r0, r1, e in rg], dln1)
         for r0, r1, e in rg:
             rr = slice(r0, r1)
diff --git a/vl-merging_amd/ops.py b/vl-merging_amd/ops.py
--- a/vl-merging_amd/ops.py
+++ b/vl-merging_amd/ops.py
@@ -141,15 +141,40 @@
     L.check(rc, "vlm_gemm_wgrad_grouped")
 
 
+def gemm_wgrad_multi(problems, accumulate=True):
+    if len(problems) < 1 or len(problems) > L.WGRAD_MAX_PROBLEMS:
+        raise L.VlmError("gemm_wgrad_multi: 1..%d problems" % L.WGRAD_MAX_PROBLEMS)
+    arr = (L.WgradProblem * len(problems))()
+    tiles = 0
+    for q, (dy, x, r0, r1, dW) in zip(arr, problems):
+        L.require_cuda(dy, x, dW)
+        if dy.dtype != BF16 or x.dtype != BF16 or dy.shape[0] != x.shape[0] or dy.dim() != 2 or x.dim() != 2:
+            raise L.VlmError("gemm_wgrad_multi: bf16 dy [tokens, M] and x [tokens, N]")
+        M, N = dy.shape[1], x.shape[1]
+        if dW.dtype != F32 or tuple(dW.shape) != (M, N) or r0 < 0 or r1 < r0 or r1 > dy.shape[0]:
+            raise L.VlmError("gemm_wgrad_multi: rows (%d, %d) gradient %s for M=%d N=%d" % (r0, r1, tuple(dW.shape), M, N))
+        q.A, q.B, q.C = dy.data_ptr(), x.data_ptr(), dW.data_ptr()
+        q.lda, q.ldb, q.ldc, q.M, q.N = _ld(dy), _ld(x), _ld(dW), M, N
+        q.row0, q.rows, q.accumulate = r0, r1 - r0, int(bool(accumulate))
+        tiles += ((M + 255) // 256) * ((N + 255) // 256)
+    ws = _splitk_workspace(problems[0][0].device, wgrad_ws_bound(tiles))
+    rc = L.get_lib().vlm_gemm_wgrad_multi(len(problems), arr, L.ptr(ws), ws.numel() * 4, L.stream_ptr())
+    L.check(rc, "vlm_gemm_wgrad_multi")
+
+
 _SPLITK_WS = {}
 SPLITK_WS_BYTES = 96 << 20
 
 
-def _splitk_workspace(device):
+def wgrad_ws_bound(tiles):
+    return (max(L.get_lib().vlm_device_cus(), 1) + 9 + tiles) * (256 << 10) + (64 << 10)
+
+
+def _splitk_workspace(device, need=0):
     key = (device.index, torch.cuda.current_stream().cuda_stream)
     ws = _SPLITK_WS.get(key)
-    if ws is None:
-        ws = _SPLITK_WS[key] = torch.empty(SPLITK_WS_BYTES // 4, device=device, dtype=F32)
+    if ws is None or ws.numel() * 4 < need:
+        ws = _SPLITK_WS[key] = torch.empty(max(SPLITK_WS_BYTES, need) // 4, device=device, dtype=F32)
     return ws
 
 
```

Result: no change. 334.6 (-0.7%).
